# HuttleyLab/DiverseSeq

Measured on AMD Instinct MI355X. Metric: sequences scored/sec (delta-JSD, k=6), higher is better.
Workload: dtype f64 (results and every set update in f64; reject/accept decisions tiered: f32 and f32-log scores decide rows farther from the threshold than their proven error bands, f64 the rest)

## Files before the change

### diverseseq_amd/_lib.py

```python

from __future__ import annotations

import ctypes as C
import os
import pathlib
import threading

import numpy as np

_HERE = pathlib.Path(__file__).resolve().parent
LIB_PATH = pathlib.Path(os.environ["DVS_HIP_LIB"]).resolve() if os.environ.get("DVS_HIP_LIB") else _HERE / "libdvs_hip.so"

OK, ERR_VALUE, ERR_RUNTIME, ERR_NOMEM, ERR_UNSUPPORTED, ERR_ZERODIV = range(6)
CUT_HEIGHT, CUT_NCLUSTERS = 0, 1
MODE_NMOST, MODE_MAX, MODE_SET = 0, 1, 2
STAT_STDEV, STAT_COV = 0, 1
SELECT_NO_ARBITER = 1
SELECT_STEPWISE = 2
ROW_REMOTE = 0xFFFFFFFF

EXPORTS = (
    "dvs_abi_version", "dvs_ctx_create", "dvs_ctx_destroy", "dvs_last_error", "dvs_ctx_sync",
    "dvs_ctx_trim", "dvs_ctx_device_info", "dvs_ctx_set_timing", "dvs_ctx_refresh_knobs", "dvs_matrix_build", "dvs_matrix_from_freqs", "dvs_matrix_from_device_freqs", "dvs_matrix_get_source_rows", "dvs_matrix_count_bytes",
    "dvs_matrix_destroy", "dvs_matrix_nrows", "dvs_matrix_nbins", "dvs_matrix_dev_counts",
    "dvs_matrix_dev_totals", "dvs_matrix_dev_entropy", "dvs_matrix_get_counts",
    "dvs_matrix_get_totals", "dvs_matrix_get_entropy", "dvs_kmer_counts", "dvs_select_run",
    "dvs_select_destroy", "dvs_select_get_summary", "dvs_select_get_members",
    "dvs_select_gather_members",
    "dvs_select_delta_jsd", "dvs_select_step_pack",
    "dvs_select_step_apply", "dvs_select_step_poll", "dvs_select_step_peek", "dvs_select_bench_scan", "dvs_selftest_fast_log2", "dvs_selftest_log2_acc", "dvs_selftest_log2_f32", "dvs_selftest_exact_div", "dvs_selftest_handover", "dvs_mash_sketch", "dvs_mash_distances", "dvs_sketches_build", "dvs_sketches_destroy", "dvs_sketches_get", "dvs_sketches_dev", "dvs_sketches_dev_lens", "dvs_sketches_distances",
    "dvs_sketches_from_device", "dvs_sketches_copy_to_device", "dvs_sketches_distances_device",
    "dvs_default_alphabet_lut", "dvs_seqbatch_from_fasta", "dvs_seqbatch_destroy", "dvs_seqbatch_info",
    "dvs_seqbatch_offsets", "dvs_seqbatch_header_positions", "dvs_seqbatch_dev_codes", "dvs_seqbatch_get_codes",
    "dvs_matrix_build_from_seqbatch",
    "dvs_pack_sequences", "dvs_packed_destroy", "dvs_packed_info", "dvs_packed_dev_codes", "dvs_packed_dev_mask",
    "dvs_packed_get", "dvs_matrix_build_packed", "dvs_sketches_build_packed", "dvs_seqbatch_pack",
    "dvs_seqbatch_packed", "dvs_sketches_build_from_seqbatch",
    "dvs_canonical_bins", "dvs_matrix_fold_canonical", "dvs_matrix_is_canonical",
    "dvs_linkage_cut", "dvs_linkage_cophenet", "dvs_nj_patristic", "dvs_pairs_destroy", "dvs_pairs_info", "dvs_pairs_get",
    "dvs_distances", "dvs_linkage", "dvs_nj", "dvs_maxmin", "dvs_cross_distances", "dvs_nearest", "dvs_within",
    "dvs_cluster_scores", "dvs_cophenet", "dvs_threshold_clusters",
)
WITHIN_SKIP_SELF = 1
SRC_MASH, SRC_EUCLIDEAN, SRC_JSD, SRC_GIVEN = range(4)


class Source(C.Structure):
    _fields_ = [("kind", C.c_uint32), ("handle", C.c_void_p), ("rows", C.POINTER(C.c_uint32)), ("n", C.c_uint32),
                ("k", C.c_uint32), ("sketch_size", C.c_uint32), ("on_device", C.c_int)]


class SelectParams(C.Structure):
    _fields_ = [("mode", C.c_uint32), ("n_seed", C.c_uint32), ("max_size", C.c_uint32),
                ("stat", C.c_uint32), ("window", C.c_uint32), ("flags", C.c_uint32)]


class SelectSummary(C.Structure):
    _fields_ = [("size", C.c_uint32), ("lowest_index", C.c_uint32),
                ("total_jsd", C.c_double), ("mean_delta_jsd", C.c_double),
                ("std_delta_jsd", C.c_double), ("cov_delta_jsd", C.c_double),
                ("summed_entropies", C.c_double),
                ("rows_scored", C.c_uint64), ("rows_rechecked", C.c_uint64),
                ("n_windows", C.c_uint32), ("n_events", C.c_uint32),
                ("n_accepts", C.c_uint32), ("n_arbitrated", C.c_uint32),
                ("scan_ms", C.c_double), ("scan_launches", C.c_uint64),
                ("engine", C.c_uint32), ("rows_coarse_passed", C.c_uint32),
                ("scan_ms_last", C.c_double), ("rows_scored_last", C.c_uint64), ("arbiter_ms", C.c_double)]


class DvsLibraryMissing(RuntimeError):
    pass


_lib = None
_lock = threading.Lock()


def _preload_torch_hip_runtime() -> None:
    import importlib.util
    import sys

    if "torch" in sys.modules:
        return
    try:
        spec = importlib.util.find_spec("torch")
    except (ImportError, ValueError):
        spec = None
    if spec is None or not spec.submodule_search_locations:
        return
    libdir = pathlib.Path(list(spec.submodule_search_locations)[0]) / "lib"
    for name in ("libhsa-runtime64.so", "libamd_comgr.so", "libamdhip64.so"):
        p = libdir / name
        if p.exists():
            try:
                C.CDLL(str(p), mode=C.RTLD_GLOBAL)
            except OSError:
                return


def load() -> C.CDLL:
    global _lib
    with _lock:
        if _lib is not None:
            return _lib
        if not LIB_PATH.exists():
            raise DvsLibraryMissing(
                f"{LIB_PATH} not found: build it with `python -c 'import __graft_entry__ as g; "
                "g.build()'` (hipcc --offload-arch=gfx950). There is no CPU fallback.")
        _preload_torch_hip_runtime()
        L = C.CDLL(str(LIB_PATH))
        vp, u8p, u32p, u64p, f64p = (C.c_void_p, C.POINTER(C.c_uint8), C.POINTER(C.c_uint32),
                                     C.POINTER(C.c_uint64), C.POINTER(C.c_double))
        L.dvs_abi_version.restype = C.c_int
        L.dvs_ctx_create.argtypes = [C.c_int, vp, C.POINTER(vp)]
        L.dvs_ctx_destroy.argtypes = [vp]
        L.dvs_ctx_destroy.restype = None
        L.dvs_last_error.argtypes = [vp]
        L.dvs_last_error.restype = C.c_char_p
        L.dvs_ctx_sync.argtypes = [vp]
        L.dvs_ctx_trim.argtypes = [vp]
        L.dvs_ctx_set_timing.argtypes = [vp, C.c_int]
        L.dvs_ctx_refresh_knobs.argtypes = [vp]
        L.dvs_ctx_device_info.argtypes = [vp, C.c_char_p, C.c_size_t, C.POINTER(C.c_int), u64p]
        L.dvs_matrix_build.argtypes = [vp, vp, C.c_int, u64p, C.c_uint32, C.c_uint32, C.c_uint32,
                                       C.POINTER(vp)]
        L.dvs_matrix_from_freqs.argtypes = [vp, f64p, C.c_uint32, C.c_uint64, C.POINTER(vp)]
        L.dvs_matrix_from_device_freqs.argtypes = [vp, vp, vp, C.c_uint32, C.c_uint64, C.POINTER(vp)]
        L.dvs_select_gather_members.argtypes = [vp, vp, vp, vp, C.c_uint32]
        L.dvs_matrix_destroy.argtypes = [vp]
        L.dvs_matrix_destroy.restype = None
        L.dvs_matrix_nrows.argtypes = [vp]
        L.dvs_matrix_nrows.restype = C.c_uint32
        L.dvs_matrix_nbins.argtypes = [vp]
        L.dvs_matrix_nbins.restype = C.c_uint64
        for n in ("dvs_matrix_dev_counts", "dvs_matrix_dev_totals", "dvs_matrix_dev_entropy"):
            getattr(L, n).argtypes = [vp]
            getattr(L, n).restype = vp
        L.dvs_matrix_get_counts.argtypes = [vp, vp, C.c_uint32, C.c_uint32, u32p]
        L.dvs_matrix_get_totals.argtypes = [vp, vp, u32p]
        L.dvs_matrix_get_entropy.argtypes = [vp, vp, f64p]
        L.dvs_matrix_get_source_rows.argtypes = [vp, vp, u32p]
        L.dvs_matrix_count_bytes.argtypes = [vp]
        L.dvs_matrix_count_bytes.restype = C.c_uint32
        L.dvs_kmer_counts.argtypes = [vp, u8p, u64p, C.c_uint32, C.c_uint32, C.c_uint32, u32p, u32p,
                                      f64p]
        L.dvs_select_run.argtypes = [vp, vp, u32p, u32p, C.c_uint64, C.POINTER(SelectParams),
                                     C.POINTER(vp)]
        L.dvs_select_destroy.argtypes = [vp]
        L.dvs_select_destroy.restype = None
        L.dvs_select_get_summary.argtypes = [vp, vp, C.POINTER(SelectSummary)]
        L.dvs_select_get_members.argtypes = [vp, vp, u64p, u32p, f64p, f64p, f64p]
        L.dvs_select_delta_jsd.argtypes = [vp, vp, vp, u32p, f64p]
        L.dvs_select_step_pack.argtypes = [vp, vp, vp]
        L.dvs_select_step_apply.argtypes = [vp, vp, vp, C.c_uint32]
        L.dvs_select_step_poll.argtypes = [vp, vp, u32p, u64p]
        L.dvs_select_step_peek.argtypes = [vp, vp, C.c_uint32, u32p, C.POINTER(C.c_int)]
        L.dvs_select_bench_scan.argtypes = [vp, vp, C.c_int, f64p, u64p]
        L.dvs_selftest_fast_log2.argtypes = [vp, f64p]
        L.dvs_selftest_log2_acc.argtypes = [vp, f64p]
        L.dvs_selftest_log2_f32.argtypes = [vp, f64p]
        L.dvs_selftest_exact_div.argtypes = [vp, C.POINTER(C.c_uint64)]
        L.dvs_selftest_handover.argtypes = [vp, C.c_uint32, C.POINTER(C.c_uint64)]
        L.dvs_mash_sketch.argtypes = [vp, vp, C.c_int, u64p, C.c_uint32, C.c_uint32, C.c_uint32,
                                      C.c_uint32, C.c_int, u32p, u32p]
        L.dvs_mash_distances.argtypes = [vp, u32p, C.c_uint32, u32p, C.c_uint32, C.c_uint32,
                                         C.c_uint32, C.c_uint32, C.c_uint32, C.c_int, f64p]
        L.dvs_sketches_build.argtypes = [vp, vp, C.c_int, u64p, C.c_uint32, C.c_uint32, C.c_uint32, C.c_uint32,
                                         C.c_int, C.POINTER(vp)]
        L.dvs_sketches_destroy.argtypes = [vp]
        L.dvs_sketches_destroy.restype = None
        L.dvs_sketches_get.argtypes = [vp, vp, u32p, u32p]
        for n in ("dvs_sketches_dev", "dvs_sketches_dev_lens"):
            getattr(L, n).argtypes = [vp]
            getattr(L, n).restype = vp
        L.dvs_sketches_distances.argtypes = [vp, vp, C.c_uint32, C.c_uint32, C.c_uint32, C.c_uint32, C.c_int, f64p]
        L.dvs_sketches_from_device.argtypes = [vp, vp, vp, C.c_uint32, C.c_uint32, C.POINTER(vp)]
        L.dvs_sketches_copy_to_device.argtypes = [vp, vp, vp, C.c_uint32, vp]
        L.dvs_sketches_distances_device.argtypes = [vp, vp, C.c_uint32, C.c_uint32, C.c_uint32, C.c_uint32, C.c_int, vp, vp]
        L.dvs_default_alphabet_lut.argtypes = [C.c_int, u8p]
        L.dvs_default_alphabet_lut.restype = None
        L.dvs_seqbatch_from_fasta.argtypes = [vp, vp, C.c_int, C.c_uint64, u8p, C.c_int, C.POINTER(vp)]
        L.dvs_seqbatch_destroy.argtypes = [vp]
        L.dvs_seqbatch_destroy.restype = None
        L.dvs_seqbatch_info.argtypes = [vp, u32p, u64p, u32p]
        L.dvs_seqbatch_offsets.argtypes = [vp, u64p]
        L.dvs_seqbatch_header_positions.argtypes = [vp, u64p]
        L.dvs_seqbatch_dev_codes.argtypes = [vp]
        L.dvs_seqbatch_dev_codes.restype = vp
        L.dvs_seqbatch_get_codes.argtypes = [vp, vp, u8p]
        L.dvs_matrix_build_from_seqbatch.argtypes = [vp, vp, C.c_uint32, C.c_uint32, C.POINTER(vp)]
        L.dvs_pack_sequences.argtypes = [vp, vp, C.c_int, C.c_uint64, C.POINTER(vp)]
        L.dvs_packed_destroy.argtypes = [vp]
        L.dvs_packed_destroy.restype = None
        L.dvs_packed_info.argtypes = [vp, u64p, u64p]
        for n in ("dvs_packed_dev_codes", "dvs_packed_dev_mask", "dvs_seqbatch_packed"):
            getattr(L, n).argtypes = [vp]
            getattr(L, n).restype = vp
        L.dvs_packed_get.argtypes = [vp, vp, u32p, C.POINTER(C.c_uint16)]
        L.dvs_matrix_build_packed.argtypes = [vp, vp, u64p, C.c_uint32, C.c_uint32, C.POINTER(vp)]
        L.dvs_sketches_build_packed.argtypes = [vp, vp, u64p, C.c_uint32, C.c_uint32, C.c_uint32, C.c_int,
                                                C.POINTER(vp)]
        L.dvs_seqbatch_pack.argtypes = [vp, vp]
        L.dvs_sketches_build_from_seqbatch.argtypes = [vp, vp, C.c_uint32, C.c_uint32, C.c_uint32, C.c_int,
                                                       C.POINTER(vp)]
        u32, srcp = C.c_uint32, C.POINTER(Source)
        L.dvs_linkage_cut.argtypes = [vp, u32, u32p, f64p, C.c_int, C.c_double, u32p, u32p]
        L.dvs_linkage_cophenet.argtypes = [vp, u32, u32p, f64p, f64p]
        L.dvs_nj_patristic.argtypes = [vp, u32, u32p, f64p, f64p]
        L.dvs_canonical_bins.argtypes = [u32, u32p, u64p]
        L.dvs_matrix_fold_canonical.argtypes = [vp, vp, C.POINTER(vp)]
        L.dvs_matrix_is_canonical.argtypes = [vp]
        L.dvs_matrix_is_canonical.restype = C.c_uint32
        L.dvs_pairs_destroy.argtypes = [vp]
        L.dvs_pairs_destroy.restype = None
        L.dvs_pairs_info.argtypes = [vp, u32p, u64p]
        L.dvs_pairs_get.argtypes = [vp, u64p, u32p, f64p]
        L.dvs_distances.argtypes = [vp, srcp, f64p]
        L.dvs_linkage.argtypes = [vp, srcp, C.c_int, u32p, f64p, u32p]
        L.dvs_nj.argtypes = [vp, srcp, u32p, f64p]
        L.dvs_maxmin.argtypes = [vp, srcp, u32p, u32, u32, C.c_int, C.c_double, u32p, f64p, u32p, u32p, f64p, f64p]
        L.dvs_cross_distances.argtypes = [vp, srcp, srcp, f64p]
# ... 29 lines not shown
```

### diverseseq_amd/csrc/api.cpp

```cpp
#include "dvs_internal.h"

#include <algorithm>
#include <cmath>
#include <cstring>
#include <mutex>

uint64_t dvs_pow_u64(uint32_t base, uint32_t exp, bool *overflow);
void dvs_matrix_free_fields(dvs_matrix *m);
int dvs_matrix_fill_counts(dvs_ctx *ctx, dvs_matrix *m, const dvs_seq_view &sv, const uint64_t *offsets, bool no_wait);
int dvs_matrix_fill_freq_entropy(dvs_ctx *ctx, dvs_matrix *m);
int dvs_hist_prepare(dvs_ctx *ctx, const uint64_t *offsets, uint32_t nseq, uint32_t k, uint64_t nbins, uint64_t nbytes, size_t *n_long_out);
bool dvs_hist_rows_fit_u16(const dvs_ctx *ctx, uint64_t B, size_t n_long);
int dvs_matrix_fill_freq_totals(dvs_ctx *ctx, dvs_matrix *m, const double *d_meta);
int dvs_matrix_fill_compacted(dvs_ctx *ctx, dvs_matrix *m, const double *d_in, const double *d_meta);

static std::string g_create_err;

int dvs_set_error(dvs_ctx *ctx, int code, const char *fmt, ...) {
    char buf[512];
    va_list ap;
    va_start(ap, fmt);
    vsnprintf(buf, sizeof buf, fmt, ap);
    va_end(ap);
    if (ctx) ctx->err = buf;
// ... 19 lines not shown
    if (it != ctx->pool.end()) {
        *ptr = it->second;
        ctx->pool.erase(it);
        ctx->pool_bytes -= sz;
        ctx->live[*ptr] = sz;
        if (__builtin_expect(ctx->knobs.test_poison_blocks, 0)) return dev_poison(ctx, *ptr, sz, what);
        return DVS_OK;
    }
    hipError_t e = hipMalloc(ptr, sz);
    if (e != hipSuccess && !ctx->pool.empty()) {
        (void)hipGetLastError();
        dvs_dev_trim(ctx);
        e = hipMalloc(ptr, sz);
    }
    if (e != hipSuccess) {
        *ptr = nullptr;
        return dvs_hip_fail(ctx, e, what);
    }
    ctx->live[*ptr] = sz;
    if (__builtin_expect(ctx->knobs.test_poison_blocks, 0)) return dev_poison(ctx, *ptr, sz, what);
    return DVS_OK;
}

void dvs_dev_free(dvs_ctx *ctx, void *ptr) {
    if (!ptr) return;
    auto it = ctx ? ctx->live.find(ptr) : std::map<void *, size_t>::iterator();
    if (!ctx || it == ctx->live.end()) {
        (void)hipFree(ptr);
        return;
    }
    ctx->pool.emplace(it->second, ptr);
    ctx->pool_bytes += it->second;
    ctx->live.erase(it);
}

int dvs_pinned_get(dvs_ctx *ctx, void **ptr) {
    if (!ctx->pinned_pool.empty()) {
        *ptr = ctx->pinned_pool.back();
        ctx->pinned_pool.pop_back();
        if (__builtin_expect(ctx->knobs.test_poison_blocks, 0)) memset(*ptr, 0xFF, 4096);
        return DVS_OK;
    }
    hipError_t e = hipHostMalloc(ptr, 4096, hipHostMallocDefault);
    if (e != hipSuccess) return dvs_hip_fail(ctx, e, "hipHostMalloc");
    if (__builtin_expect(ctx->knobs.test_poison_blocks, 0)) memset(*ptr, 0xFF, 4096);
    return DVS_OK;
}
void dvs_pinned_put(dvs_ctx *ctx, void *ptr) {
    if (!ptr) return;
    if (ctx) ctx->pinned_pool.push_back(ptr);
    else (void)hipHostFree(ptr);
}
hipEvent_t dvs_event_get(dvs_ctx *ctx) {
    if (!ctx->event_pool.empty()) {
        hipEvent_t e = ctx->event_pool.back();
        ctx->event_pool.pop_back();
        return e;
    }
    hipEvent_t e = nullptr;
    (void)hipEventCreate(&e);
    return e;
}
void dvs_event_put(dvs_ctx *ctx, hipEvent_t e) {
    if (!e) return;
    if (ctx) ctx->event_pool.push_back(e);
    else (void)hipEventDestroy(e);
}

void dvs_dev_trim(dvs_ctx *ctx) {
    (void)hipStreamSynchronize(ctx->stream);
    for (auto &kv : ctx->pool) (void)hipFree(kv.second);
    ctx->pool.clear();
    ctx->pool_bytes = 0;
}

void dvs_knobs_from_env(dvs_knobs *k) {
    auto on = [](const char *name) { return getenv(name) != nullptr; };
    *k = dvs_knobs();
    k->no_uniform_offsets = on("DVS_NO_UNIFORM_OFFSETS");
    k->no_offsets_cache = on("DVS_NO_OFFSETS_CACHE");
    k->counts_u32 = on("DVS_COUNTS_U32");
    k->build_wait = on("DVS_BUILD_WAIT");
    k->no_packed_upload = on("DVS_NO_PACKED_UPLOAD");
    k->cu_mask_set = on("HSA_CU_MASK") || on("ROC_GLOBAL_CU_MASK");
    k->no_persist = on("DVS_NO_PERSIST");
    k->no_fast_step = on("DVS_NO_FAST_STEP");
    k->no_head_phase = on("DVS_NO_HEAD_PHASE");
    k->persist_no_seeded = on("DVS_PERSIST_NO_SEEDED");
    k->persist_no_small = on("DVS_PERSIST_NO_SMALL");
    k->persist_no_coarse = on("DVS_PERSIST_NO_COARSE");
    k->persist_no_events = on("DVS_PERSIST_NO_EVENTS");
    k->persist_debug = on("DVS_PERSIST_DEBUG");
    const char *rounds = getenv("DVS_PERSIST_WG_ROUNDS");
    k->persist_wg_rounds = rounds ? atoi(rounds) : -1;
    k->ingest_no_stream = on("DVS_INGEST_NO_STREAM");
    if (const char *sr = getenv("DVS_CROSS_STRIP_ROWS")) k->cross_strip_rows = uint32_t(strtoul(sr, nullptr, 10));
    if (const char *mb = getenv("DVS_MAXMIN_BATCH")) k->maxmin_batch = uint32_t(strtoul(mb, nullptr, 10));
    k->maxmin_jsd_cross = on("DVS_MAXMIN_JSD_CROSS");
    const char *tk = getenv("DVS_TEST_KNOBS");
    k->test_persist_fake_error = tk && strstr(tk, "fake_persist_error") != nullptr;
    if (const char *lt = tk ? strstr(tk, "long_tile_") : nullptr) k->test_long_tile = uint32_t(strtoul(lt + 10, nullptr, 10));
    k->test_rowlog_ring = 0;
    if (const char *rr = tk ? strstr(tk, "rowlog_ring_") : nullptr) k->test_rowlog_ring = uint32_t(strtoul(rr + 12, nullptr, 10));
    k->test_poison_blocks = tk && strstr(tk, "poison_blocks") != nullptr;
    if (const char *ic = tk ? strstr(tk, "ingest_chunk_") : nullptr)
        k->test_ingest_chunk = uint32_t(std::min<unsigned long>(std::max<unsigned long>(strtoul(ic + 13, nullptr, 10), 1ul), 256ul));
    if (const char *rc = tk ? strstr(tk, "ingest_reccap_") : nullptr)
        k->test_ingest_reccap = std::max<uint64_t>(strtoull(rc + 14, nullptr, 10), 1ull);
}

extern "C" {

int dvs_abi_version(void) { return DVS_ABI_VERSION; }

int dvs_ctx_refresh_knobs(dvs_ctx *ctx) {
    if (!ctx) return dvs_set_error(ctx, DVS_ERR_VALUE, "null argument");
    dvs_knobs_from_env(&ctx->knobs);
    ctx->off_cache.n_off = 0;
    return DVS_OK;
}

int dvs_ctx_create(int device, void *stream, dvs_ctx **out) {
    if (!out) return dvs_set_error(nullptr, DVS_ERR_VALUE, "null argument");
    *out = nullptr;
    int ndev = 0;
    hipError_t e = hipGetDeviceCount(&ndev);
    if (e != hipSuccess || ndev == 0)
        return dvs_set_error(nullptr, DVS_ERR_RUNTIME,
                             "no HIP device available (%s): libdvs_hip has no CPU fallback",
                             e != hipSuccess ? hipGetErrorString(e) : "device count 0");
    if (device < 0) {
        e = hipGetDevice(&device);
        if (e != hipSuccess) return dvs_hip_fail(nullptr, e, "hipGetDevice");
    }
    if (device >= ndev)
        return dvs_set_error(nullptr, DVS_ERR_VALUE, "device %d out of range (%d devices)", device, ndev);
    e = hipSetDevice(device);
    if (e != hipSuccess) return dvs_hip_fail(nullptr, e, "hipSetDevice");
    hipDeviceProp_t prop;
    e = hipGetDeviceProperties(&prop, device);
    if (e != hipSuccess) return dvs_hip_fail(nullptr, e, "hipGetDeviceProperties");
    dvs_ctx *ctx = new dvs_ctx();
    dvs_knobs_from_env(&ctx->knobs);
    ctx->device = device;
    ctx->n_cu = prop.multiProcessorCount;
    ctx->lds_per_block = prop.sharedMemPerBlockOptin ? prop.sharedMemPerBlockOptin
                                                     : prop.sharedMemPerBlock;
    if (ctx->lds_per_block < prop.sharedMemPerBlock) ctx->lds_per_block = prop.sharedMemPerBlock;
    if (stream) {
        ctx->stream = static_cast<hipStream_t>(stream);
    } else {
        e = hipStreamCreateWithFlags(&ctx->stream, hipStreamNonBlocking);
        if (e != hipSuccess) {
            delete ctx;
            return dvs_hip_fail(nullptr, e, "hipStreamCreate");
        }
        ctx->own_stream = true;
    }
    *out = ctx;
    return DVS_OK;
}

void dvs_ctx_destroy(dvs_ctx *ctx) {
    if (!ctx || ctx->owner_gone) return;
    ctx->owner_gone = true;
    dvs_ctx_release(ctx);
// ... 76 lines not shown
    dvs_dev_trim(ctx);
    return DVS_OK;
}

int dvs_ctx_sync(dvs_ctx *ctx) {
    if (!ctx) return DVS_ERR_VALUE;
    DVS_HIP(ctx, hipStreamSynchronize(ctx->stream));
    return DVS_OK;
}

int dvs_ctx_set_timing(dvs_ctx *ctx, int on) {
    if (!ctx) return DVS_ERR_VALUE;
    ctx->timing = on != 0;
    return DVS_OK;
}

int dvs_ctx_device_info(dvs_ctx *ctx, char *name, size_t name_len, int *n_cu, uint64_t *hbm_bytes) {
    if (!ctx) return DVS_ERR_VALUE;
    hipDeviceProp_t prop;
    DVS_HIP(ctx, hipGetDeviceProperties(&prop, ctx->device));
    if (name && name_len) {
        snprintf(name, name_len, "%s (%s)", prop.name, prop.gcnArchName);
    }
    if (n_cu) *n_cu = prop.multiProcessorCount;
    if (hbm_bytes) *hbm_bytes = prop.totalGlobalMem;
    return DVS_OK;
}

static int matrix_alloc(dvs_ctx *ctx, dvs_matrix *m) {
    const size_t cells = size_t(m->nrows) * m->nbins;
    const size_t bytes = cells * (m->kind == 0 ? 4 : m->kind == 2 ? 2 : 8);
    size_t free_b = 0, total_b = 0;
    const bool cached = ctx->pool.count(((bytes ? bytes : 4) + 4095) & ~size_t(4095)) > 0;
    if (!cached) DVS_HIP(ctx, hipMemGetInfo(&free_b, &total_b));
    if (!cached && bytes + size_t(m->nrows) * 12 + (64u << 20) > free_b + ctx->pool_bytes)
        return dvs_set_error(ctx, DVS_ERR_NOMEM,
                             "%u x %llu matrix needs %zu bytes of HBM, %zu free", m->nrows,
                             (unsigned long long)m->nbins, bytes, free_b);
    const size_t nr = m->nrows ? m->nrows : 1;
    m->ctx = ctx;
    dvs_ctx_retain(ctx);
    int rc;
    if (m->kind == 0) rc = dvs_dev_alloc(ctx, (void **)&m->d_counts, bytes ? bytes : 4, "matrix counts");
    else if (m->kind == 2) rc = dvs_dev_alloc(ctx, (void **)&m->d_counts16, bytes ? bytes : 4, "matrix counts (16-bit)");
    else rc = dvs_dev_alloc(ctx, (void **)&m->d_freqs, bytes ? bytes : 8, "matrix freqs");
    if (!rc) rc = dvs_dev_alloc(ctx, (void **)&m->d_totals, nr * 4, "matrix totals");
    if (!rc) rc = dvs_dev_alloc(ctx, (void **)&m->d_entropy, nr * 8, "matrix entropy");
    return rc;
}

static int build_shape(dvs_ctx *ctx, uint32_t k, uint32_t num_states, uint64_t *B_out) {
    if (k == 0) return dvs_set_error(ctx, DVS_ERR_VALUE, "k cannot be 0");
    if (num_states < 1 || num_states > 255)
        return dvs_set_error(ctx, DVS_ERR_VALUE, "num_states %u outside 1..255", num_states);
    if (k > 17) return dvs_set_error(ctx, DVS_ERR_UNSUPPORTED, "k = %u > 17 is not supported", k);
    bool ovf = false;
    const uint64_t B = dvs_pow_u64(num_states, k, &ovf);
    if (ovf || B > (1ull << 32))
        return dvs_set_error(ctx, DVS_ERR_UNSUPPORTED, "%u^%u bins do not fit a dense count row",
                             num_states, k);
    *B_out = B;
    return DVS_OK;
}

static int matrix_build_view(dvs_ctx *ctx, const dvs_seq_view &sv, const uint64_t *offsets, uint32_t nseq, uint32_t k,
                             uint32_t num_states, bool no_wait, dvs_matrix **out) {
    *out = nullptr;
    uint64_t B = 0;
    const int arc = build_shape(ctx, k, num_states, &B);
    if (arc) return arc;
    size_t n_long = 0;
    if (nseq) {
        const int prc = dvs_hist_prepare(ctx, offsets, nseq, k, B, sv.nbytes, &n_long);
        if (prc) return prc;
    }
    dvs_matrix *m = new dvs_matrix();
    m->kind = (nseq && dvs_hist_rows_fit_u16(ctx, B, n_long)) ? 2 : 0;
    m->nrows = nseq;
    m->nbins = B;
    m->k = k;
    m->num_states = num_states;
    m->device = ctx->device;
    int rc = matrix_alloc(ctx, m);
    if (!rc && nseq) rc = dvs_matrix_fill_counts(ctx, m, sv, offsets, no_wait);
    if (rc) {
        dvs_matrix_free_fields(m);
        delete m;
        return rc;
    }
    *out = m;
    return DVS_OK;
}

int dvs_matrix_build(dvs_ctx *ctx, const uint8_t *seqs, int seqs_on_device, const uint64_t *offsets,
                     uint32_t nseq, uint32_t k, uint32_t num_states, dvs_matrix **out) {
    if (!ctx || !offsets || !out || (!seqs && nseq && offsets[nseq] > 0))
        return dvs_set_error(ctx, DVS_ERR_VALUE, "null argument");
    *out = nullptr;
    {
        uint64_t B_ = 0;
        const int arc = build_shape(ctx, k, num_states, &B_);
        if (arc) return arc;
    }
    DVS_HIP(ctx, hipSetDevice(ctx->device));
    const uint64_t nbytes = nseq ? offsets[nseq] : 0;
    dvs_seq_view sv;
    if (seqs_on_device) {
        if (reinterpret_cast<uintptr_t>(seqs) & 15)
            return dvs_set_error(ctx, DVS_ERR_VALUE, "device sequence buffer must be 16-byte aligned");
        sv.seqs = seqs;
        sv.nbytes = nbytes;
        return matrix_build_view(ctx, sv, offsets, nseq, k, num_states, !ctx->knobs.build_wait, out);
    }
    if (nbytes && dvs_packed_upload_wanted(ctx, num_states, nbytes)) {
        dvs_packed *p = nullptr;
        int rc = dvs_packed_alloc(ctx, nbytes, &p);
        if (!rc) rc = dvs_packed_fill_from_host(ctx, p, seqs);
        if (!rc) {
            sv.codes = p->d_codes;
            sv.mask = p->d_mask;
            sv.nbytes = nbytes;
            rc = matrix_build_view(ctx, sv, offsets, nseq, k, num_states, false, out);
        }
        if (p) {
            (void)hipStreamSynchronize(ctx->stream);
            dvs_packed_destroy(p);
        }
        return rc;
    }
    const uint64_t padded = ((nbytes + 15) & ~15ull) + 16;
    uint8_t *d_tmp = nullptr;
    int rc = dvs_dev_alloc(ctx, (void **)&d_tmp, padded, "sequence upload buffer");
    if (rc) return rc;
    hipError_t ue = hipMemsetAsync(d_tmp + (nbytes & ~15ull), 0xFF, padded - (nbytes & ~15ull), ctx->stream);
    if (ue == hipSuccess && nbytes) ue = hipMemcpyAsync(d_tmp, seqs, nbytes, hipMemcpyHostToDevice, ctx->stream);
    if (ue != hipSuccess) {
        (void)hipStreamSynchronize(ctx->stream);
        dvs_dev_free(ctx, d_tmp);
        return dvs_hip_fail(ctx, ue, "sequence upload");
    }
    sv.seqs = d_tmp;
    sv.nbytes = padded;
    rc = matrix_build_view(ctx, sv, offsets, nseq, k, num_states, false, out);
    (void)hipStreamSynchronize(ctx->stream);
    dvs_dev_free(ctx, d_tmp);
    return rc;
}

int dvs_matrix_build_packed(dvs_ctx *ctx, const dvs_packed *p, const uint64_t *offsets, uint32_t nseq, uint32_t k,
                            dvs_matrix **out) {
    if (!ctx || !p || !offsets || !out) return dvs_set_error(ctx, DVS_ERR_VALUE, "null argument");
    *out = nullptr;
    DVS_HIP(ctx, hipSetDevice(ctx->device));
    dvs_seq_view sv;
    sv.codes = p->d_codes;
    sv.mask = p->d_mask;
    sv.nbytes = p->nbases;
    p->async_readers = true;
    return matrix_build_view(ctx, sv, offsets, nseq, k, 4, !ctx->knobs.build_wait, out);
}

int dvs_matrix_from_freqs(dvs_ctx *ctx, const double *freqs, uint32_t nrows, uint64_t nbins,
                          dvs_matrix **out) {
    if (!ctx || !out || (!freqs && nrows)) return dvs_set_error(ctx, DVS_ERR_VALUE, "null argument");
    *out = nullptr;
    if (nbins == 0)
// ... 36 lines not shown
    return DVS_OK;
}

int dvs_matrix_from_device_freqs(dvs_ctx *ctx, const double *d_freqs, const double *d_meta, uint32_t nrows,
                                 uint64_t nbins, dvs_matrix **out) {
    if (!ctx || !out || (!d_freqs && nrows)) return dvs_set_error(ctx, DVS_ERR_VALUE, "null argument");
    *out = nullptr;
    if (nbins == 0)
        return dvs_set_error(ctx, DVS_ERR_VALUE, "cannot calculate entropy as frequency vector empty");
    DVS_HIP(ctx, hipSetDevice(ctx->device));
    dvs_matrix *m = new dvs_matrix();
    m->kind = 1;
    m->nrows = nrows;
    m->nbins = nbins;
    m->device = ctx->device;
    int rc = matrix_alloc(ctx, m);
    if (!rc && nrows && d_meta) {
        rc = dvs_dev_alloc(ctx, (void **)&m->d_src_row, size_t(nrows) * 4, "source rows");
        if (!rc) rc = dvs_matrix_fill_compacted(ctx, m, d_freqs, d_meta);
        if (!rc) rc = dvs_matrix_fill_freq_entropy(ctx, m);
    } else if (!rc && nrows) {
        hipError_t e = hipMemcpyAsync(m->d_freqs, d_freqs, size_t(nrows) * nbins * 8, hipMemcpyDeviceToDevice,
                                      ctx->stream);
        if (e != hipSuccess) rc = dvs_hip_fail(ctx, e, "hipMemcpyAsync(freqs)");
        if (!rc) rc = dvs_matrix_fill_freq_totals(ctx, m, nullptr);
        if (!rc) rc = dvs_matrix_fill_freq_entropy(ctx, m);
    }
    if (rc) {
        dvs_matrix_free_fields(m);
        delete m;
        return rc;
    }
    *out = m;
    return DVS_OK;
}

int dvs_matrix_get_source_rows(dvs_ctx *ctx, const dvs_matrix *m, uint32_t *out) {
    if (!ctx || !m || !out) return dvs_set_error(ctx, DVS_ERR_VALUE, "null argument");
    if (!m->d_src_row) {
        for (uint32_t r = 0; r < m->nrows; r++) out[r] = r;
        return DVS_OK;
    }
    DVS_HIP(ctx, hipMemcpyAsync(out, m->d_src_row, size_t(m->nrows) * 4, hipMemcpyDeviceToHost, ctx->stream));
    DVS_HIP(ctx, hipStreamSynchronize(ctx->stream));
    return DVS_OK;
}

void dvs_matrix_destroy(dvs_matrix *m) {
    if (!m) return;
    dvs_matrix_free_fields(m);
    delete m;
}

uint32_t dvs_matrix_nrows(const dvs_matrix *m) { return m ? m->nrows : 0; }
uint64_t dvs_matrix_nbins(const dvs_matrix *m) { return m ? m->nbins : 0; }
const void *dvs_matrix_dev_counts(const dvs_matrix *m) {
    return !m ? nullptr : m->kind == 2 ? static_cast<const void *>(m->d_counts16) : static_cast<const void *>(m->d_counts);
}
uint32_t dvs_matrix_count_bytes(const dvs_matrix *m) { return !m ? 0u : m->kind == 0 ? 4u : m->kind == 2 ? 2u : 0u; }
const void *dvs_matrix_dev_totals(const dvs_matrix *m) { return m ? m->d_totals : nullptr; }
const void *dvs_matrix_dev_entropy(const dvs_matrix *m) { return m ? m->d_entropy : nullptr; }

int dvs_matrix_get_counts(dvs_ctx *ctx, const dvs_matrix *m, uint32_t row0, uint32_t nrows,
                          uint32_t *out) {
    if (!ctx || !m || !out) return dvs_set_error(ctx, DVS_ERR_VALUE, "null argument");
    if (m->kind == 1) return dvs_set_error(ctx, DVS_ERR_VALUE, "not a count matrix");
    if (uint64_t(row0) + nrows > m->nrows) return dvs_set_error(ctx, DVS_ERR_VALUE, "row range out of bounds");
    if (!nrows) return DVS_OK;
    if (m->kind == 2) {
        const size_t cells = size_t(nrows) * m->nbins;
        std::vector<uint16_t> tmp(cells);
        DVS_HIP(ctx, hipMemcpyAsync(tmp.data(), m->d_counts16 + uint64_t(row0) * m->nbins, cells * 2,
                                    hipMemcpyDeviceToHost, ctx->stream));
        DVS_HIP(ctx, hipStreamSynchronize(ctx->stream));
        for (size_t i = 0; i < cells; i++) out[i] = tmp[i];
        return DVS_OK;
    }
    DVS_HIP(ctx, hipMemcpyAsync(out, m->d_counts + uint64_t(row0) * m->nbins,
                                size_t(nrows) * m->nbins * 4, hipMemcpyDeviceToHost, ctx->stream));
    DVS_HIP(ctx, hipStreamSynchronize(ctx->stream));
    return DVS_OK;
}

int dvs_matrix_get_totals(dvs_ctx *ctx, const dvs_matrix *m, uint32_t *out) {
    if (!ctx || !m || !out) return dvs_set_error(ctx, DVS_ERR_VALUE, "null argument");
    if (!m->nrows) return DVS_OK;
    DVS_HIP(ctx, hipMemcpyAsync(out, m->d_totals, size_t(m->nrows) * 4, hipMemcpyDeviceToHost,
                                ctx->stream));
    DVS_HIP(ctx, hipStreamSynchronize(ctx->stream));
    return DVS_OK;
}

int dvs_matrix_get_entropy(dvs_ctx *ctx, const dvs_matrix *m, double *out) {
    if (!ctx || !m || !out) return dvs_set_error(ctx, DVS_ERR_VALUE, "null argument");
    if (!m->nrows) return DVS_OK;
    DVS_HIP(ctx, hipMemcpyAsync(out, m->d_entropy, size_t(m->nrows) * 8, hipMemcpyDeviceToHost,
                                ctx->stream));
    DVS_HIP(ctx, hipStreamSynchronize(ctx->stream));
    return DVS_OK;
}

int dvs_kmer_counts(dvs_ctx *ctx, const uint8_t *seqs, const uint64_t *offsets, uint32_t nseq,
                    uint32_t k, uint32_t num_states, uint32_t *counts_out, uint32_t *totals_out,
                    double *entropy_out) {
    dvs_matrix *m = nullptr;
    int rc = dvs_matrix_build(ctx, seqs, 0, offsets, nseq, k, num_states, &m);
    if (rc) return rc;
    if (counts_out) rc = dvs_matrix_get_counts(ctx, m, 0, nseq, counts_out);
    if (!rc && totals_out) rc = dvs_matrix_get_totals(ctx, m, totals_out);
    if (!rc && entropy_out) rc = dvs_matrix_get_entropy(ctx, m, entropy_out);
    dvs_matrix_destroy(m);
    return rc;
}

}

int dvs_matrix_alloc_fields(dvs_ctx *ctx, dvs_matrix *m) { return matrix_alloc(ctx, m); }
```

### diverseseq_amd/csrc/dvs_internal.h

```cpp
#pragma once

#include <hip/hip_runtime.h>

#include <cstdarg>
#include <cstdint>
#include <cstdio>
#include <functional>
#include <map>
#include <string>
#include <vector>

#include "../../include/dvs_hip.h"

#define DVS_EPS 2.220446049250313e-16
#define DVS_HEAD_ROWS 1024u

struct dvs_knobs {
    bool no_uniform_offsets = false;
    bool no_offsets_cache = false;
    bool counts_u32 = false;
    bool build_wait = false;
    bool no_packed_upload = false;
    bool cu_mask_set = false;
    bool no_fast_step = false;
    bool no_persist = false;
    bool no_head_phase = false;
    bool persist_no_seeded = false;
    bool persist_no_small = false;
    bool persist_no_coarse = false;
    bool persist_no_events = false;
    bool persist_debug = false;
    int persist_wg_rounds = -1;
    uint32_t cross_strip_rows = 0;
    uint32_t maxmin_batch = 0;
    bool maxmin_jsd_cross = false;
    bool ingest_no_stream = false;
    bool test_persist_fake_error = false;
    uint32_t test_long_tile = 0;
    uint32_t test_rowlog_ring = 0;
    bool test_poison_blocks = false;
    uint32_t test_ingest_chunk = 0;
    uint64_t test_ingest_reccap = 0;
};
void dvs_knobs_from_env(dvs_knobs *k);

struct dvs_ctx {
    dvs_knobs knobs;
    int device = 0;
    hipStream_t stream = nullptr;
    bool own_stream = false;
    hipStream_t stream2 = nullptr;
    hipStream_t stream_head = nullptr, stream_rest = nullptr;
    int head_cus = 0;
    bool cu_split_tried = false;
    int persist_timeouts = 0;
    int n_cu = 0;
    size_t lds_per_block = 0;
    double *d_clog_tbl = nullptr;
    bool timing = false;
    std::string err;
    std::multimap<size_t, void *> pool;
    std::vector<void *> pinned_pool;
    std::vector<hipEvent_t> event_pool;
    std::map<void *, size_t> live;
    size_t pool_bytes = 0;
    int refs = 1;
    bool owner_gone = false;
    std::map<const void *, size_t> lds_raised;
    std::map<std::pair<const void *, size_t>, bool> persist_fits;
    struct OffsetsCache {
        uint64_t *h_off = nullptr;
        size_t h_cap = 0, n_off = 0;
        hipEvent_t ev_up = nullptr;
        std::vector<uint32_t> h_long_rows;
        std::vector<unsigned char> h_tiles;
        uint64_t nbytes = 0;
        uint32_t k = 0;
        void *d_off = nullptr, *d_rows = nullptr, *d_tiles = nullptr;
        size_t d_off_cap = 0;
        size_t n_long = 0, n_tiles = 0;
        bool uniform = false;
        uint64_t uni_base = 0, uni_stride = 0;
        bool lists_in_flight = false;
    } off_cache;
    void *h_pack = nullptr;
    size_t h_pack_cap = 0;
    hipEvent_t pack_ev = nullptr;
    std::map<uint32_t, uint32_t *> canon_reps;
};
int dvs_raise_dyn_lds(dvs_ctx *ctx, const void *fn, size_t bytes);
void dvs_ctx_retain(dvs_ctx *ctx);
hipStream_t dvs_ctx_stream2(dvs_ctx *ctx);
bool dvs_ctx_cu_split(dvs_ctx *ctx);
void dvs_ctx_release(dvs_ctx *ctx);

struct dvs_matrix;
int dvs_matrix_settle(dvs_ctx *ctx, const dvs_matrix *m);
int dvs_dev_alloc(dvs_ctx *ctx, void **ptr, size_t bytes, const char *what);
void dvs_dev_free(dvs_ctx *ctx, void *ptr);
void dvs_dev_trim(dvs_ctx *ctx);
struct PooledBuf {
    dvs_ctx *ctx;
    void *p = nullptr;
    ~PooledBuf() { dvs_dev_free(ctx, p); }
    template <typename T>
    T *as() { return static_cast<T *>(p); }
};
int dvs_pinned_get(dvs_ctx *ctx, void **ptr);
void dvs_pinned_put(dvs_ctx *ctx, void *ptr);
hipEvent_t dvs_event_get(dvs_ctx *ctx);
void dvs_event_put(dvs_ctx *ctx, hipEvent_t e);

int dvs_set_error(dvs_ctx *ctx, int code, const char *fmt, ...);
int dvs_hip_fail(dvs_ctx *ctx, hipError_t e, const char *what);

#define DVS_HIP(ctx, call)                                        \
    do {                                                          \
        hipError_t e__ = (call);                                  \
        if (e__ != hipSuccess) return dvs_hip_fail(ctx, e__, #call); \
    } while (0)

struct dvs_matrix {
    int kind = 0;
    uint16_t *d_counts16 = nullptr;
    uint32_t nrows = 0;
    uint64_t nbins = 0;
    uint32_t k = 0, num_states = 0;
    uint32_t *d_counts = nullptr;
    double *d_freqs = nullptr;
    uint32_t *d_totals = nullptr;
    double *d_entropy = nullptr;
    uint32_t *d_src_row = nullptr;
    std::vector<uint32_t> h_head_totals;
    uint32_t *h_head_pinned = nullptr;
    hipEvent_t ev_built = nullptr;
    hipEvent_t ev_join = nullptr;
    uint32_t head_count = 0;
    uint32_t head_rows_built = 0;
    bool rest_beside_head = false;
    bool in_flight = false;
    bool canonical = false;
    int device = 0;
    dvs_ctx *ctx = nullptr;
};

struct dvs_packed {
    dvs_ctx *ctx = nullptr;
    uint32_t *d_codes = nullptr;
    uint16_t *d_mask = nullptr;
    uint64_t nbases = 0, nwords = 0;
    mutable bool async_readers = false;
};
struct dvs_seq_view {
    const uint8_t *seqs = nullptr;
    const uint32_t *codes = nullptr;
    const uint16_t *mask = nullptr;
    uint64_t nbytes = 0;
};
int dvs_packed_alloc(dvs_ctx *ctx, uint64_t nbases, dvs_packed **out);
int dvs_packed_fill_from_device(dvs_ctx *ctx, dvs_packed *p, const uint8_t *d_seqs);
int dvs_packed_fill_from_host(dvs_ctx *ctx, dvs_packed *p, const uint8_t *seqs);
bool dvs_packed_upload_wanted(const dvs_ctx *ctx, uint32_t num_states, uint64_t nbytes);

int dvs_linkage_check_size(dvs_ctx *ctx, uint32_t n);
int dvs_linkage_check_method(dvs_ctx *ctx, int method);
int dvs_linkage_device(dvs_ctx *ctx, double *d_dist, uint32_t n, const uint32_t *d_zerodiv, int method, uint32_t *pairs,
                       double *heights, uint32_t *sizes);
constexpr uint32_t DVS_LNK_NONFINITE = 1, DVS_LNK_NEGATIVE = 4;
hipError_t dvs_linkage_enqueue_prepare(dvs_ctx *ctx, double *d_dist, uint32_t n, bool sign, uint32_t *d_status);

int dvs_nj_device(dvs_ctx *ctx, double *d_dist, uint32_t n, const uint32_t *d_zerodiv, uint32_t *joins, double *lengths);

int dvs_cophenet_walk(dvs_ctx *ctx, uint32_t n, const uint32_t *pairs, const double *heights, uint32_t *order,
                      uint32_t *pos, uint32_t *gap, double *c_bar);

struct dvs_dist_stage {
    const char *label;
    uint32_t n;
    std::function<int()> check;
    size_t scratch_bytes;
    const char *scratch_what;
    bool scratch_is_zerodiv;
    bool zero_diagonal;
    std::function<hipError_t(double *d_dist, void *d_scratch)> enqueue;
};
dvs_dist_stage dvs_mash_stage(dvs_ctx *ctx, const dvs_sketches *sk, uint32_t k, uint32_t sketch_size);

struct dvs_cross_stage {
    const char *label;
    uint32_t m, n;
    std::function<int()> check;
    size_t scratch_bytes;
    const char *scratch_what;
    bool scratch_is_zerodiv;
    std::function<hipError_t(void *d_scratch)> prepare;
    std::function<hipError_t(uint32_t q0, uint32_t mq, double *d_strip, void *d_scratch)> enqueue;
};
dvs_cross_stage dvs_mash_cross_stage(dvs_ctx *ctx, const dvs_sketches *q, const uint32_t *q_rows, uint32_t nq,
                                     const dvs_sketches *r, const uint32_t *r_rows, uint32_t nr, uint32_t k,
                                     uint32_t sketch_size, const uint32_t *d_q_rows = nullptr);
dvs_cross_stage dvs_euclid_cross_stage(dvs_ctx *ctx, const dvs_matrix *q, const uint32_t *q_rows, uint32_t nq,
                                       const dvs_matrix *r, const uint32_t *r_rows, uint32_t nr,
                                       const uint32_t *d_q_rows = nullptr);
hipError_t dvs_jsd_entropies_enqueue(dvs_ctx *ctx, const dvs_matrix *m, const uint32_t *d_rows, uint32_t count, double *d_h);
hipError_t dvs_jsd_cross_row_enqueue(dvs_ctx *ctx, const dvs_matrix *m, const uint32_t *d_q_rows, uint32_t q0, uint32_t n,
                                     const double *d_hq, const double *d_hr, double *d_row);
int dvs_rows_check(dvs_ctx *ctx, uint32_t n);
// ... 134 lines not shown
```

### diverseseq_amd/csrc/kmer_hist.hip

```cpp
#include "dvs_internal.h"

#include <algorithm>
#include <cstring>
#include <cmath>
#include <cstdlib>

namespace {

constexpr int HIST_THREADS = 256;
constexpr int HIST_MAX_THREADS = 512;
constexpr uint32_t TILE_LEN = 32768;
static_assert(TILE_LEN < 65536, "a whole-sequence tile's counts must fit the packed 16-bit LDS counters");
constexpr int CLOG_TBL = 256;

struct KTile {
    uint64_t begin;
    uint64_t end;
    uint64_t seq_begin;
    uint32_t row;
    uint32_t single;
};

__device__ __forceinline__ uint4 load16(const uint8_t *base, uint64_t off, uint64_t nbytes) {
    if (off + 16 <= nbytes) return *reinterpret_cast<const uint4 *>(base + off);
    uint32_t w[4] = {0xFFFFFFFFu, 0xFFFFFFFFu, 0xFFFFFFFFu, 0xFFFFFFFFu};
    for (int i = 0; i < 16; i++) {
        if (off + i < nbytes) {
            w[i >> 2] &= ~(0xFFu << (8 * (i & 3)));
            w[i >> 2] |= uint32_t(base[off + i]) << (8 * (i & 3));
        }
    }
    return make_uint4(w[0], w[1], w[2], w[3]);
}

template <bool LDS_HIST, bool PK16 = false>
__device__ __forceinline__ void bump(uint32_t *hist, uint32_t idx) {
    if (PK16) atomicAdd(&hist[idx >> 1], (idx & 1u) ? 0x10000u : 1u);
    else atomicAdd(&hist[idx], 1u);
}

__device__ __forceinline__ double clog2c(uint32_t c, const double *tbl) {
    if (c < CLOG_TBL) return tbl[c];
    const double d = double(c);
    return d * log2(d);
}

template <bool NS4, bool LDS_HIST, bool PK16 = false, bool OUT16 = false, bool PACKED = false>
__global__ __launch_bounds__(HIST_MAX_THREADS) void kmer_hist_kernel(
    const uint8_t *__restrict__ seqs, const uint16_t *__restrict__ pmask, uint64_t nbytes,
    const uint64_t *__restrict__ offsets,
    const KTile *__restrict__ tiles, uint32_t *__restrict__ counts, uint32_t *__restrict__ totals,
    double *__restrict__ entropy, const double *__restrict__ clog_tbl, uint32_t k, uint32_t ns,
    uint64_t B, uint32_t hot_rows, uint32_t row0, uint64_t uni_base, uint64_t uni_stride) {
    extern __shared__ __attribute__((aligned(16))) unsigned char smem[];
    KTile t;
    if (tiles) {
        t = tiles[blockIdx.x];
    } else {
        const uint32_t r = row0 + (hot_rows ? gridDim.x - 1 - blockIdx.x : blockIdx.x);
        const uint64_t s0 = offsets ? offsets[r] : uni_base + uint64_t(r) * uni_stride;
        const uint64_t s1 = offsets ? offsets[r + 1] : s0 + uni_stride;
        t.row = r;
        t.single = 1;
        t.seq_begin = s0;
        t.begin = s0 + k - 1;
        t.end = s1;
        if (s1 - s0 >= k && s1 - t.begin > TILE_LEN) return;
        if (s1 - s0 < k) t.begin = t.end = s1;
    }
    static_assert(!OUT16 || PK16, "16-bit rows come from the packed histogram");
    static_assert(!PACKED || NS4, "only four-state sequences have a packed form");
    uint32_t *row = OUT16 ? counts + uint64_t(t.row) * (B / 2) : counts + uint64_t(t.row) * B;
    uint32_t *hist = LDS_HIST ? reinterpret_cast<uint32_t *>(smem) : row;
    double *tbl = reinterpret_cast<double *>(smem + (LDS_HIST ? ((B * (PK16 ? 2 : 4) + 15) & ~15ull) : 0));
    double *scratch = tbl + CLOG_TBL;
    const int tid = threadIdx.x;
    const int nthreads = blockDim.x;

    if (LDS_HIST) {
        if ((B & 3) == 0) {
            uint4 *h4 = reinterpret_cast<uint4 *>(hist);
            for (uint64_t i = tid; i < B / (PK16 ? 8 : 4); i += nthreads) h4[i] = make_uint4(0, 0, 0, 0);
            if (PK16 && (B & 7) && tid == 0) reinterpret_cast<uint2 *>(hist)[B / 4 - 1] = make_uint2(0, 0);
        } else {
            for (uint64_t i = tid; i < B; i += nthreads) hist[i] = 0;
        }
    }
    for (int i = tid; i < CLOG_TBL; i += nthreads) tbl[i] = clog_tbl[i];
    __syncthreads();

    uint32_t nvalid = 0;
    const uint64_t abase = t.begin & ~15ull;
    const uint64_t nchunks = t.end > t.begin ? (t.end - abase + 15) >> 4 : 0;
    const uint32_t bmask = uint32_t(B - 1);

    if (NS4) {
        const uint32_t lane = tid & 63, wave = tid >> 6, nwaves = (nthreads + 63) >> 6;
        const uint64_t per_wave = ((nchunks + nwaves - 1) / nwaves + 63) & ~63ull;
        const uint64_t c_lo = uint64_t(wave) * per_wave;
        const uint64_t c_hi = c_lo + per_wave < nchunks ? c_lo + per_wave : nchunks;
        uint32_t carryP = 0, carryI = 0xFFFFu;
        if (c_lo < c_hi) {
            const uint64_t A0 = abase + (c_lo << 4);
            if (A0 >= 16) {
                if constexpr (PACKED) {
                    carryP = reinterpret_cast<const uint32_t *>(seqs)[(A0 >> 4) - 1];
                    carryI = pmask[(A0 >> 4) - 1];
                } else {
                    const uint4 pv = load16(seqs, A0 - 16, nbytes);
                    carryP = dvs_pack16(pv);
                    carryI = dvs_inv16(pv);
                }
            }
        }
        for (uint64_t c0 = c_lo; c0 < c_hi; c0 += 64) {
            const uint64_t c = c0 + lane;
            const bool live = c < c_hi;
            const uint64_t A = abase + ((live ? c : c_hi - 1) << 4);
            uint32_t Pc, Ic = 0;
            if constexpr (PACKED) {
                Pc = reinterpret_cast<const uint32_t *>(seqs)[A >> 4];
                Ic = pmask[A >> 4];
            } else {
                const uint4 cur = load16(seqs, A, nbytes);
                Pc = dvs_pack16(cur);
                const uint32_t hib = (cur.x | cur.y | cur.z | cur.w) & 0xFCFCFCFCu;
                if (__ballot(hib != 0)) Ic = dvs_inv16(cur);
            }
            const uint32_t Pp = uint32_t(__builtin_amdgcn_update_dpp(int(carryP), int(Pc), 0x138, 0xF, 0xF, false));
            const uint32_t Ip = uint32_t(__builtin_amdgcn_update_dpp(int(carryI), int(Ic), 0x138, 0xF, 0xF, false));
            carryP = uint32_t(__builtin_amdgcn_readlane(int(Pc), 63));
            carryI = uint32_t(__builtin_amdgcn_readlane(int(Ic), 63));
            const uint64_t P = (uint64_t(Pp) << 32) | Pc;
            uint32_t I = (Ip << 16) | Ic;
            const int64_t lead = int64_t(t.seq_begin) - (int64_t(A) - 16);
            if (lead > 0) I |= (lead >= 32) ? 0xFFFFFFFFu : ~(0xFFFFFFFFu >> lead);
// ... 5 lines not shown
                    cover *= 2;
                }
                if (cover < k) W |= W >> (k - cover);
            }
            const uint32_t lo = t.begin > A ? uint32_t(t.begin - A < 16 ? t.begin - A : 16) : 0u;
            const uint32_t hi = t.end > A ? uint32_t(t.end - A < 16 ? t.end - A : 16) : 0u;
            const uint32_t R = (live && hi > lo) ? ((0xFFFFu >> lo) & ~(0xFFFFu >> hi)) : 0u;
            const uint32_t ok = R & ~W & 0xFFFFu;
            nvalid += __popc(ok);
            if (__ballot(ok != 0xFFFFu) == 0) {
                if constexpr (PK16) {
                    const uint64_t P2 = P << 1;
                    const uint32_t p2lo = uint32_t(P2), p2hi = uint32_t(P2 >> 32);
                    const uint32_t amask = (bmask << 1) & ~3u;
                    unsigned char *hb = smem;
#pragma unroll
                    for (int j = 0; j < 16; j++) {
                        const uint32_t tq = __builtin_amdgcn_alignbit(p2hi, p2lo, 2 * (15 - j));
                        uint32_t half = __builtin_amdgcn_ubfe(tq, 1, 1);
                        asm volatile("" : "+v"(half));
                        atomicAdd(reinterpret_cast<uint32_t *>(hb + (tq & amask)), __umul24(half, 0xFFFFu) + 1u);
                    }
                } else {
#pragma unroll
                    for (int j = 0; j < 16; j++) bump<LDS_HIST, PK16>(hist, uint32_t(P >> (2 * (15 - j))) & bmask);
                }
            } else {
#pragma unroll
                for (int j = 0; j < 16; j++) {
                    const uint32_t idx = uint32_t(P >> (2 * (15 - j))) & bmask;
                    if ((ok >> (15 - j)) & 1u) bump<LDS_HIST, PK16>(hist, idx);
                }
            }
        }
    } else {
        for (uint64_t c = tid; c < nchunks; c += nthreads) {
            const uint64_t A = abase + (c << 4);
            const uint4 cur = load16(seqs, A, nbytes);
            const uint4 prev = (A >= 16) ? load16(seqs, A - 16, nbytes)
                                         : make_uint4(0xFFFFFFFFu, 0xFFFFFFFFu, 0xFFFFFFFFu, 0xFFFFFFFFu);
            const int64_t lead = int64_t(t.seq_begin) - (int64_t(A) - 16);
            const uint32_t w[8] = {prev.x, prev.y, prev.z, prev.w, cur.x, cur.y, cur.z, cur.w};
            uint32_t idx = 0, run = 0;
            const uint32_t Bd = uint32_t(B / ns);
#pragma unroll
            for (int q = 0; q < 32; q++) {
                const uint32_t b = (w[q >> 2] >> (8 * (q & 3))) & 0xFFu;
                const bool ok = (b < ns) && (int64_t(q) >= lead);
                idx = ok ? (idx % Bd) * ns + b : 0u;
                run = ok ? run + 1 : 0u;
                if (q >= 16) {
                    const uint64_t p = A + (q - 16);
                    if (p >= t.begin && p < t.end && run >= k) {
                        bump<LDS_HIST, PK16>(hist, idx);
                        nvalid++;
                    }
                }
            }
        }
    }
    if (!LDS_HIST) __threadfence();
    __syncthreads();

    if constexpr (PK16) {
        const uint2 *h2 = reinterpret_cast<const uint2 *>(hist);
        uint4 *r4 = reinterpret_cast<uint4 *>(row);
        typedef uint32_t u32x4 __attribute__((ext_vector_type(4)));
        double sv[2] = {0.0, 0.0}, tv[2] = {0.0, 0.0};
#pragma unroll
        for (int half = 0; half < 2; half++)
            for (uint64_t u = uint64_t(tid) + 128u * half; u < B / 4; u += HIST_THREADS) {
                const uint2 w = h2[u];
                const uint4 v = make_uint4(w.x & 0xFFFFu, w.x >> 16, w.y & 0xFFFFu, w.y >> 16);
                if constexpr (OUT16) {
                    typedef uint32_t u32x2 __attribute__((ext_vector_type(2)));
                    uint2 *r2 = reinterpret_cast<uint2 *>(row);
                    if (t.row < hot_rows) r2[u] = w;
                    else __builtin_nontemporal_store((u32x2){w.x, w.y}, reinterpret_cast<u32x2 *>(r2 + u));
                } else if (t.row < hot_rows) r4[u] = v;
                else __builtin_nontemporal_store((u32x4){v.x, v.y, v.z, v.w}, reinterpret_cast<u32x4 *>(r4 + u));
                if (((w.x | w.y) & 0xFF00FF00u) == 0) sv[half] += ((tbl[v.x] + tbl[v.y]) + tbl[v.z]) + tbl[v.w];
                else sv[half] += clog2c(v.x, tbl) + clog2c(v.y, tbl) + clog2c(v.z, tbl) + clog2c(v.w, tbl);
            }
        tv[0] = double(nvalid);
        const int lane = tid & 63, wave = tid >> 6;
        double sums[2];
#pragma unroll
        for (int q = 0; q < 2; q++) {
            const double a = dvs_wave_sum(q ? tv[0] : sv[0]), b = dvs_wave_sum(q ? tv[1] : sv[1]);
            __syncthreads();
            if (lane == 0) {
                scratch[wave] = a;
                scratch[wave + 2] = b;
            }
            __syncthreads();
            double acc = 0.0;
            for (int i = 0; i < 4; i++) acc += scratch[i];
            sums[q] = acc;
        }
        if (tid == 0) {
            totals[t.row] = uint32_t(sums[1]);
            entropy[t.row] = sums[1] > 0.0 ? log2(sums[1]) - sums[0] / sums[1] : 0.0;
        }
    } else if (t.single) {
        double s = 0.0, tot = 0.0;
        if (tid >= HIST_THREADS) {
        } else if (LDS_HIST) {
            if ((B & 3) == 0) {
                const uint4 *h4 = reinterpret_cast<const uint4 *>(hist);
                uint4 *r4 = reinterpret_cast<uint4 *>(row);
                for (uint64_t i = tid; i < B / 4; i += HIST_THREADS) {
                    const uint4 v = h4[i];
                    typedef uint32_t u32x4 __attribute__((ext_vector_type(4)));
                    if (t.row < hot_rows) r4[i] = v;
                    else __builtin_nontemporal_store((u32x4){v.x, v.y, v.z, v.w}, reinterpret_cast<u32x4 *>(r4 + i));
                    s += clog2c(v.x, tbl) + clog2c(v.y, tbl) + clog2c(v.z, tbl) + clog2c(v.w, tbl);
                    tot += double(v.x) + double(v.y) + double(v.z) + double(v.w);
                }
            } else {
                for (uint64_t i = tid; i < B; i += HIST_THREADS) {
                    const uint32_t v = hist[i];
                    row[i] = v;
                    s += clog2c(v, tbl);
                    tot += double(v);
                }
            }
        } else {
            for (uint64_t i = tid; i < B; i += HIST_THREADS) {
                const uint32_t v = __hip_atomic_load(&row[i], __ATOMIC_RELAXED, __HIP_MEMORY_SCOPE_AGENT);
                s += clog2c(v, tbl);
                tot += double(v);
            }
        }
        s = dvs_block_sum(s, scratch);
        tot = dvs_block_sum(tot, scratch);
        if (tid == 0) {
            totals[t.row] = uint32_t(tot);
            entropy[t.row] = tot > 0.0 ? log2(tot) - s / tot : 0.0;
        }
    } else if (LDS_HIST) {
        for (uint64_t i = tid; i < B; i += nthreads) {
            const uint32_t v = hist[i];
            if (v) atomicAdd(&row[i], v);
        }
    }
}

__global__ void clog_tbl_kernel(double *tbl) {
    const int c = threadIdx.x;
    tbl[c] = c ? double(c) * log2(double(c)) : 0.0;
}

__global__ __launch_bounds__(HIST_THREADS) void row_stats_kernel(
    const uint32_t *__restrict__ counts, const uint32_t *__restrict__ rows,
    uint32_t *__restrict__ totals, double *__restrict__ entropy, uint64_t B) {
    __shared__ double tbl[CLOG_TBL];
    __shared__ double scratch[32];
    const int tid = threadIdx.x;
    if (tid < CLOG_TBL) tbl[tid] = tid ? double(tid) * log2(double(tid)) : 0.0;
    __syncthreads();
    const uint32_t r = rows[blockIdx.x];
    const uint32_t *row = counts + uint64_t(r) * B;
    double s = 0.0, tot = 0.0;
    for (uint64_t i = tid; i < B; i += HIST_THREADS) {
        const uint32_t v = row[i];
        s += clog2c(v, tbl);
        tot += double(v);
    }
    s = dvs_block_sum(s, scratch);
    tot = dvs_block_sum(tot, scratch);
    if (tid == 0) {
        totals[r] = uint32_t(tot);
        entropy[r] = tot > 0.0 ? log2(tot) - s / tot : 0.0;
    }
}

__global__ __launch_bounds__(HIST_THREADS) void zero_rows_kernel(uint32_t *__restrict__ counts,
                                                                const uint32_t *__restrict__ rows,
                                                                uint64_t B) {
    uint32_t *row = counts + uint64_t(rows[blockIdx.x]) * B;
    for (uint64_t i = threadIdx.x; i < B; i += HIST_THREADS) row[i] = 0;
}

__global__ __launch_bounds__(HIST_THREADS) void freq_entropy_kernel(
    const double *__restrict__ freqs, double *__restrict__ entropy, uint64_t B) {
// ... 2 lines not shown
    double h = 0.0;
    for (uint64_t i = threadIdx.x; i < B; i += HIST_THREADS) {
        const double f = row[i];
        if (f != 0.0) h += -f * log2(f);
    }
    h = dvs_block_sum(h, scratch);
    if (threadIdx.x == 0) entropy[blockIdx.x] = h;
}

__global__ __launch_bounds__(HIST_THREADS) void compact_freq_rows_kernel(
    const double *__restrict__ in, const double *__restrict__ meta, double *__restrict__ out,
    uint32_t *__restrict__ totals, uint32_t *__restrict__ src, uint32_t nrows, uint64_t B) {
    __shared__ uint32_t s_cnt[2];
    const uint32_t r = blockIdx.x;
    if (threadIdx.x < 2) s_cnt[threadIdx.x] = 0;
    __syncthreads();
    uint32_t before = 0, all = 0;
    for (uint32_t q = threadIdx.x; q < nrows; q += HIST_THREADS) {
        const uint32_t v = meta[2 * q + 1] != 0.0 ? 1u : 0u;
        all += v;
        if (q < r) before += v;
    }
    atomicAdd(&s_cnt[0], before);
    atomicAdd(&s_cnt[1], all);
    __syncthreads();
    const bool real = meta[2 * r + 1] != 0.0;
    const uint32_t dest = real ? s_cnt[0] : s_cnt[1] + (r - s_cnt[0]);
    const double *a = in + uint64_t(r) * B;
    double *o = out + uint64_t(dest) * B;
    for (uint64_t i = threadIdx.x; i < B; i += HIST_THREADS) o[i] = a[i];
    if (threadIdx.x == 0) {
        totals[dest] = real ? 1u : 0u;
        src[dest] = r;
    }
}

__global__ void freq_totals_kernel(uint32_t *__restrict__ totals, const double *__restrict__ meta,
                                   uint32_t nrows) {
    const uint32_t r = blockIdx.x * blockDim.x + threadIdx.x;
    if (r < nrows) totals[r] = (!meta || meta[2 * r + 1] != 0.0) ? 1u : 0u;
}

template <typename K>
int set_dyn_lds(dvs_ctx *ctx, K kernel, size_t bytes) {
    return dvs_raise_dyn_lds(ctx, reinterpret_cast<const void *>(kernel), bytes);
}

}

uint64_t dvs_pow_u64(uint32_t base, uint32_t exp, bool *overflow) {
    uint64_t r = 1;
    *overflow = false;
    for (uint32_t i = 0; i < exp; i++) {
        if (r > UINT64_MAX / (base ? base : 1)) *overflow = true;
        r *= base;
    }
    return r;
}

int dvs_matrix_settle(dvs_ctx *ctx, const dvs_matrix *cm) {
    dvs_matrix *m = const_cast<dvs_matrix *>(cm);
    if (!m || !m->ev_built) return DVS_OK;
    const hipError_t e = hipEventSynchronize(m->ev_built);
    if (e == hipSuccess) m->h_head_totals.assign(m->h_head_pinned, m->h_head_pinned + m->head_count);
    else m->h_head_totals.clear();
    dvs_event_put(m->ctx, m->ev_built);
    dvs_pinned_put(m->ctx, m->h_head_pinned);
    m->ev_built = nullptr;
    m->h_head_pinned = nullptr;
    if (e != hipSuccess) return dvs_hip_fail(ctx ? ctx : m->ctx, e, "histogram kernels");
    return DVS_OK;
}

void dvs_matrix_free_fields(dvs_matrix *m) {
    if (!m) return;
    (void)dvs_matrix_settle(m->ctx, m);
    if (m->in_flight && m->ctx) (void)hipStreamSynchronize(m->ctx->stream);
    m->in_flight = false;
    if (m->ev_join) dvs_event_put(m->ctx, m->ev_join);
    m->ev_join = nullptr;
    dvs_dev_free(m->ctx, m->d_counts);
    dvs_dev_free(m->ctx, m->d_counts16);
    m->d_counts16 = nullptr;
    dvs_dev_free(m->ctx, m->d_freqs);
    dvs_dev_free(m->ctx, m->d_totals);
    dvs_dev_free(m->ctx, m->d_entropy);
    dvs_dev_free(m->ctx, m->d_src_row);
    m->d_src_row = nullptr;
    m->d_counts = nullptr;
    m->d_freqs = nullptr;
    m->d_totals = nullptr;
    m->d_entropy = nullptr;
    dvs_ctx_release(m->ctx);
    m->ctx = nullptr;
}

int dvs_hist_prepare(dvs_ctx *ctx, const uint64_t *offsets, uint32_t nseq, uint32_t k, uint64_t nbins, uint64_t nbytes,
                     size_t *n_long_out) {
    dvs_ctx::OffsetsCache &oc = ctx->off_cache;
    const size_t n_off = size_t(nseq) + 1;
    oc.uniform = false;
    if (nseq >= 1 && !ctx->knobs.no_uniform_offsets) {
        const uint64_t base = offsets[0], stride = offsets[1] - offsets[0];
        bool uni = offsets[1] >= offsets[0] && stride < uint64_t(TILE_LEN) + k;
        uint64_t diff = 0;
        for (uint32_t r = 0; r < nseq && uni; r += 4096) {
            const uint32_t e = std::min<uint32_t>(nseq, r + 4096);
            for (uint32_t q = r; q < e; q++) diff |= (offsets[q + 1] - offsets[q]) ^ stride;
            uni = diff == 0;
        }
        if (uni && base + uint64_t(nseq) * stride <= nbytes) {
            if (oc.lists_in_flight && (oc.d_rows || oc.d_tiles)) {
                (void)hipStreamSynchronize(ctx->stream);
                oc.lists_in_flight = false;
            }
            dvs_dev_free(ctx, oc.d_rows);
            dvs_dev_free(ctx, oc.d_tiles);
            oc.d_rows = oc.d_tiles = nullptr;
            oc.n_long = oc.n_tiles = 0;
            oc.n_off = 0;
            oc.uniform = true;
            oc.uni_base = base;
            oc.uni_stride = stride;
            *n_long_out = 0;
            return DVS_OK;
        }
    }
    const bool hit = oc.d_off && oc.h_off && oc.k == k && oc.nbytes == nbytes && oc.n_off == n_off &&
                     !ctx->knobs.no_offsets_cache && std::memcmp(oc.h_off, offsets, n_off * 8) == 0;
    if (!hit) {
        if (oc.ev_up) (void)hipEventSynchronize(oc.ev_up);
        if (oc.h_cap < n_off) {
            if (oc.h_off) (void)hipHostFree(oc.h_off);
            oc.h_off = nullptr;
            oc.h_cap = 0;
            const size_t cap = std::max<size_t>(n_off + n_off / 4, 1024);
            const hipError_t he = hipHostMalloc((void **)&oc.h_off, cap * 8, hipHostMallocDefault);
            if (he != hipSuccess) {
                oc.h_off = nullptr;
                return dvs_hip_fail(ctx, he, "pinned offsets block");
            }
            oc.h_cap = cap;
        }
        oc.n_off = 0;
        std::vector<KTile> tiles;
        std::vector<uint32_t> long_rows;
        uint64_t *dst = oc.h_off;
        uint64_t bad = 0, longest = 0;
        dst[0] = offsets[0];
        for (uint32_t r = 0; r < nseq; r++) {
            const uint64_t s0 = offsets[r], s1 = offsets[r + 1];
            dst[r + 1] = s1;
            bad |= uint64_t(s1 < s0) | uint64_t(s1 > nbytes);
            const uint64_t len = s1 - s0;
            longest = len > longest ? len : longest;
        }
        if (bad || longest >= uint64_t(TILE_LEN) + k) {
            uint64_t long_windows = 0;
            for (uint32_t r = 0; r < nseq; r++) {
                const uint64_t s0 = offsets[r], s1 = offsets[r + 1];
                if (s1 < s0 || s1 > nbytes)
                    return dvs_set_error(ctx, DVS_ERR_VALUE, "offsets[%u..%u] = %llu..%llu out of range", r,
                                         r + 1, (unsigned long long)s0, (unsigned long long)s1);
                if (s1 - s0 >= k && s1 - (s0 + k - 1) > TILE_LEN) long_windows += s1 - (s0 + k - 1);
            }
            uint64_t tile_long = TILE_LEN;
// ... 10 lines not shown
                long_rows.push_back(r);
                for (uint64_t b = first; b < s1; b += tile_long) {
                    KTile t;
                    t.begin = b;
                    t.end = std::min<uint64_t>(b + tile_long, s1);
                    t.seq_begin = s0;
                    t.row = r;
                    t.single = 0;
                    tiles.push_back(t);
                }
            }
        }
        if (oc.lists_in_flight && (oc.d_rows || oc.d_tiles || oc.d_off_cap < n_off)) {
            (void)hipStreamSynchronize(ctx->stream);
            oc.lists_in_flight = false;
        }
        dvs_dev_free(ctx, oc.d_rows);
        dvs_dev_free(ctx, oc.d_tiles);
        oc.d_rows = oc.d_tiles = nullptr;
        oc.n_long = oc.n_tiles = 0;
        int arc = DVS_OK;
        if (oc.d_off_cap < n_off) {
            dvs_dev_free(ctx, oc.d_off);
            oc.d_off = nullptr;
            oc.d_off_cap = 0;
            arc = dvs_dev_alloc(ctx, &oc.d_off, (n_off + n_off / 4) * 8, "offsets");
            if (!arc) oc.d_off_cap = n_off + n_off / 4;
        }
        if (!arc && !long_rows.empty()) arc = dvs_dev_alloc(ctx, &oc.d_rows, long_rows.size() * 4, "row list");
        if (!arc && !tiles.empty()) arc = dvs_dev_alloc(ctx, &oc.d_tiles, tiles.size() * sizeof(KTile), "tile list");
        hipError_t ue = hipSuccess;
        oc.h_tiles.assign(reinterpret_cast<const unsigned char *>(tiles.data()),
                          reinterpret_cast<const unsigned char *>(tiles.data()) + tiles.size() * sizeof(KTile));
        oc.h_long_rows = long_rows;
        if (!arc) ue = hipMemcpyAsync(oc.d_off, oc.h_off, n_off * 8, hipMemcpyHostToDevice, ctx->stream);
        if (!arc && ue == hipSuccess) {
            if (!oc.ev_up) oc.ev_up = dvs_event_get(ctx);
            if (oc.ev_up) ue = hipEventRecord(oc.ev_up, ctx->stream);
        }
        if (!arc && ue == hipSuccess && !long_rows.empty()) {
            ue = hipMemcpyAsync(oc.d_rows, oc.h_long_rows.data(), long_rows.size() * 4, hipMemcpyHostToDevice, ctx->stream);
            if (ue == hipSuccess)
                ue = hipMemcpyAsync(oc.d_tiles, oc.h_tiles.data(), oc.h_tiles.size(), hipMemcpyHostToDevice,
                                    ctx->stream);
        }
        if (arc || ue != hipSuccess) {
            dvs_dev_free(ctx, oc.d_rows);
            dvs_dev_free(ctx, oc.d_tiles);
            oc.d_rows = oc.d_tiles = nullptr;
            return arc ? arc : dvs_hip_fail(ctx, ue, "histogram setup");
        }
        oc.n_off = n_off;
        oc.nbytes = nbytes;
        oc.k = k;
        oc.n_long = long_rows.size();
        oc.n_tiles = tiles.size();
    }
    *n_long_out = oc.n_long;
    return DVS_OK;
}

bool dvs_hist_rows_fit_u16(const dvs_ctx *ctx, uint64_t B, size_t n_long) {
    return n_long == 0 && B <= 4096 && (B & 3) == 0 && !ctx->knobs.counts_u32;
}

int dvs_matrix_fill_counts(dvs_ctx *ctx, dvs_matrix *m, const dvs_seq_view &sv, const uint64_t *offsets,
                           bool no_wait) {
    const bool packed = sv.codes != nullptr;
    const uint8_t *d_seqs = packed ? reinterpret_cast<const uint8_t *>(sv.codes) : sv.seqs;
    const uint16_t *d_pmask = sv.mask;
    const uint64_t nbytes = sv.nbytes;
    const uint32_t nseq = m->nrows, k = m->k, ns = m->num_states;
    if (packed && ns != 4) return dvs_set_error(ctx, DVS_ERR_VALUE, "packed sequences have four states, not %u", ns);
    const uint64_t B = m->nbins;
    const bool lds_hist = B * 4 <= 64 * 1024;
    const bool ns4 = ns == 4;
    (void)offsets;
    dvs_ctx::OffsetsCache &oc = ctx->off_cache;
    uint64_t *d_off = oc.uniform ? nullptr : static_cast<uint64_t *>(oc.d_off);
    const uint64_t uni_base = oc.uni_base, uni_stride = oc.uni_stride;
    uint32_t *d_rows = static_cast<uint32_t *>(oc.d_rows);
    KTile *d_tiles = static_cast<KTile *>(oc.d_tiles);
    const size_t n_long = oc.n_long, n_tiles = oc.n_tiles;
    auto cleanup = [&]() {};
    int rc = DVS_OK;
    hipError_t e = hipSuccess;
    if (!lds_hist)
        e = hipMemsetAsync(m->d_counts, 0, size_t(nseq) * B * 4, ctx->stream);
    if (e == hipSuccess && n_long && lds_hist)
        hipLaunchKernelGGL(zero_rows_kernel, dim3(uint32_t(n_long)), dim3(HIST_THREADS), 0, ctx->stream,
                           m->d_counts, d_rows, B);
    if (e != hipSuccess) return dvs_hip_fail(ctx, e, "histogram setup");
    if (!ctx->d_clog_tbl) {
        rc = dvs_dev_alloc(ctx, (void **)&ctx->d_clog_tbl, CLOG_TBL * sizeof(double), "c log2 c table");
        if (rc) {
            cleanup();
            return rc;
        }
        hipLaunchKernelGGL(clog_tbl_kernel, dim3(1), dim3(CLOG_TBL), 0, ctx->stream, ctx->d_clog_tbl);
    }
    int nthreads = HIST_THREADS;
    const int tile_threads = (lds_hist && B * 4 > 32768) ? HIST_MAX_THREADS : HIST_THREADS;
    const size_t lds = (lds_hist ? ((B * 4 + 15) & ~15ull) : 0) + (CLOG_TBL + 32) * sizeof(double);
#define DVS_LAUNCH_HIST(NS4, LH, PKD, GRID, TILES, NTHR, HOT)                                             \
    do {                                                                                         \
        rc = set_dyn_lds(ctx, kmer_hist_kernel<NS4, LH, false, false, PKD>, lds);                \
        if (!rc)                                                                                 \
            hipLaunchKernelGGL((kmer_hist_kernel<NS4, LH, false, false, PKD>), dim3(GRID), dim3(NTHR), lds,  \
                               ctx->stream, d_seqs, d_pmask, nbytes, d_off, TILES, m->d_counts,  \
                               m->d_totals, m->d_entropy, ctx->d_clog_tbl, k, ns, B, HOT, 0u, uni_base, uni_stride);   \
    } while (0)
#define DVS_LAUNCH_HIST_ANY(GRID, TILES, NTHR, HOT)                            \
    do {                                                                  \
        if (packed && lds_hist) DVS_LAUNCH_HIST(true, true, true, GRID, TILES, NTHR, HOT);   \
        else if (packed) DVS_LAUNCH_HIST(true, false, true, GRID, TILES, NTHR, HOT);         \
        else if (ns4 && lds_hist) DVS_LAUNCH_HIST(true, true, false, GRID, TILES, NTHR, HOT);   \
        else if (ns4) DVS_LAUNCH_HIST(true, false, false, GRID, TILES, NTHR, HOT);         \
        else if (lds_hist) DVS_LAUNCH_HIST(false, true, false, GRID, TILES, NTHR, HOT);    \
        else DVS_LAUNCH_HIST(false, false, false, GRID, TILES, NTHR, HOT);                 \
    } while (0)
    uint32_t hot_rows = uint32_t(std::min<uint64_t>(nseq, (192ull << 20) / (B * (m->kind == 2 ? 2 : 4))));
    const bool pk16 = lds_hist && (B & 3) == 0;
    uint32_t head_rows = 0;
    if (m->kind == 2 && no_wait) {
        uint32_t want = DVS_HEAD_ROWS;
        head_rows = std::min<uint32_t>(nseq, want);
    }
    if (head_rows == nseq) head_rows = 0;
    bool head_event_done = false;
    if (m->kind == 2) {
        const size_t lds16 = ((B * 2 + 15) & ~15ull) + (CLOG_TBL + 32) * sizeof(double);
        uint32_t *out16 = reinterpret_cast<uint32_t *>(m->d_counts16);
        auto launch16 = [&](uint32_t row0, uint32_t count, uint32_t hot_end, hipStream_t on) {
            if (packed) {
                rc = set_dyn_lds(ctx, kmer_hist_kernel<true, true, true, true, true>, lds16);
                if (!rc)
                    hipLaunchKernelGGL((kmer_hist_kernel<true, true, true, true, true>), dim3(count), dim3(128), lds16, on,
                                       d_seqs, d_pmask, nbytes, d_off, static_cast<const KTile *>(nullptr), out16,
                                       m->d_totals, m->d_entropy, ctx->d_clog_tbl, k, ns, B, hot_end, row0, uni_base, uni_stride);
            } else if (ns4) {
                rc = set_dyn_lds(ctx, kmer_hist_kernel<true, true, true, true>, lds16);
                if (!rc)
                    hipLaunchKernelGGL((kmer_hist_kernel<true, true, true, true>), dim3(count), dim3(128), lds16, on,
                                       d_seqs, d_pmask, nbytes, d_off, static_cast<const KTile *>(nullptr), out16,
                                       m->d_totals, m->d_entropy, ctx->d_clog_tbl, k, ns, B, hot_end, row0, uni_base, uni_stride);
            } else {
                rc = set_dyn_lds(ctx, kmer_hist_kernel<false, true, true, true>, lds16);
                if (!rc)
                    hipLaunchKernelGGL((kmer_hist_kernel<false, true, true, true>), dim3(count), dim3(128), lds16, on,
                                       d_seqs, d_pmask, nbytes, d_off, static_cast<const KTile *>(nullptr), out16,
                                       m->d_totals, m->d_entropy, ctx->d_clog_tbl, k, ns, B, hot_end, row0, uni_base, uni_stride);
            }
        };
        if (head_rows) {
            const bool split = nseq - head_rows >= 16u * head_rows && dvs_ctx_cu_split(ctx);
            hipEvent_t ev_fork = split ? dvs_event_get(ctx) : nullptr;
            bool forked = ev_fork && hipEventRecord(ev_fork, ctx->stream) == hipSuccess &&
                          hipStreamWaitEvent(ctx->stream_rest, ev_fork, 0) == hipSuccess;
            launch16(0, head_rows, head_rows, ctx->stream);
            void *pin = nullptr;
            if (!rc && dvs_pinned_get(ctx, &pin) == DVS_OK) {
                m->head_count = uint32_t(std::min<size_t>(head_rows, 4096 / sizeof(uint32_t)));
                m->h_head_pinned = static_cast<uint32_t *>(pin);
                m->ev_built = dvs_event_get(ctx);
                if (m->ev_built &&
                    hipMemcpyAsync(m->h_head_pinned, m->d_totals, size_t(m->head_count) * 4, hipMemcpyDeviceToHost,
                                   ctx->stream) == hipSuccess &&
                    hipEventRecord(m->ev_built, ctx->stream) == hipSuccess) {
                    head_event_done = true;
                    m->head_rows_built = head_rows;
                } else {
                    if (m->ev_built) dvs_event_put(ctx, m->ev_built);
                    dvs_pinned_put(ctx, pin);
                    m->ev_built = nullptr;
                    m->h_head_pinned = nullptr;
                }
            }
            if (!rc) {
                const uint32_t hot_end = uint32_t(std::min<uint64_t>(nseq, uint64_t(head_rows) + hot_rows));
                forked = forked && head_event_done;
                launch16(head_rows, nseq - head_rows, hot_end, forked ? ctx->stream_rest : ctx->stream);
                if (forked) {
                    hipEvent_t ev_join = dvs_event_get(ctx);
                    if (!ev_join || hipEventRecord(ev_join, ctx->stream_rest) != hipSuccess ||
                        hipStreamWaitEvent(ctx->stream, ev_join, 0) != hipSuccess) {
                        (void)hipGetLastError();
                        (void)hipStreamSynchronize(ctx->stream_rest);
                    } else {
                        m->rest_beside_head = true;
                    }
                    m->ev_join = ev_join;
                }
            }
            if (ev_fork) dvs_event_put(ctx, ev_fork);
        } else {
            launch16(0, nseq, hot_rows, ctx->stream);
        }
    } else if (pk16) {
        const size_t lds16 = ((B * 2 + 15) & ~15ull) + (CLOG_TBL + 32) * sizeof(double);
        if (packed) {
            rc = set_dyn_lds(ctx, kmer_hist_kernel<true, true, true, false, true>, lds16);
            if (!rc)
                hipLaunchKernelGGL((kmer_hist_kernel<true, true, true, false, true>), dim3(nseq), dim3(128), lds16, ctx->stream,
                                   d_seqs, d_pmask, nbytes, d_off, static_cast<const KTile *>(nullptr), m->d_counts,
                                   m->d_totals, m->d_entropy, ctx->d_clog_tbl, k, ns, B, hot_rows, 0u, uni_base, uni_stride);
        } else if (ns4) {
            rc = set_dyn_lds(ctx, kmer_hist_kernel<true, true, true>, lds16);
            if (!rc)
                hipLaunchKernelGGL((kmer_hist_kernel<true, true, true>), dim3(nseq), dim3(128), lds16, ctx->stream,
                                   d_seqs, d_pmask, nbytes, d_off, static_cast<const KTile *>(nullptr), m->d_counts,
                                   m->d_totals, m->d_entropy, ctx->d_clog_tbl, k, ns, B, hot_rows, 0u, uni_base, uni_stride);
        } else {
            rc = set_dyn_lds(ctx, kmer_hist_kernel<false, true, true>, lds16);
            if (!rc)
                hipLaunchKernelGGL((kmer_hist_kernel<false, true, true>), dim3(nseq), dim3(128), lds16, ctx->stream,
                                   d_seqs, d_pmask, nbytes, d_off, static_cast<const KTile *>(nullptr), m->d_counts,
                                   m->d_totals, m->d_entropy, ctx->d_clog_tbl, k, ns, B, hot_rows, 0u, uni_base, uni_stride);
        }
    } else
        DVS_LAUNCH_HIST_ANY(nseq, static_cast<const KTile *>(nullptr), nthreads, hot_rows);
    if (!rc && n_tiles) {
        DVS_LAUNCH_HIST_ANY(uint32_t(n_tiles), d_tiles, tile_threads, 0u);
        if (!rc)
            hipLaunchKernelGGL(row_stats_kernel, dim3(uint32_t(n_long)), dim3(HIST_THREADS), 0,
                               ctx->stream, m->d_counts, d_rows, m->d_totals, m->d_entropy, B);
    }
#undef DVS_LAUNCH_HIST_ANY
#undef DVS_LAUNCH_HIST
    if (!rc && (e = hipGetLastError()) != hipSuccess) rc = dvs_hip_fail(ctx, e, "histogram launch");
    if (!rc && no_wait && head_event_done) {
        m->in_flight = oc.lists_in_flight = true;
        return DVS_OK;
    }
    if (!rc && no_wait) {
        void *pin = nullptr;
        if (dvs_pinned_get(ctx, &pin) == DVS_OK) {
            m->head_count = uint32_t(std::min<size_t>(nseq, 4096 / sizeof(uint32_t)));
            m->h_head_pinned = static_cast<uint32_t *>(pin);
            m->ev_built = dvs_event_get(ctx);
            if (m->ev_built &&
                hipMemcpyAsync(m->h_head_pinned, m->d_totals, size_t(m->head_count) * 4, hipMemcpyDeviceToHost,
                               ctx->stream) == hipSuccess &&
                hipEventRecord(m->ev_built, ctx->stream) == hipSuccess) {
                m->in_flight = oc.lists_in_flight = true;
                return DVS_OK;
            }
            if (m->ev_built) dvs_event_put(ctx, m->ev_built);
            dvs_pinned_put(ctx, pin);
            m->ev_built = nullptr;
            m->h_head_pinned = nullptr;
        }
    }
    m->h_head_totals.assign(std::min<size_t>(nseq, 4096), 0u);
    if (!rc && !m->h_head_totals.empty() &&
        hipMemcpyAsync(m->h_head_totals.data(), m->d_totals, m->h_head_totals.size() * 4, hipMemcpyDeviceToHost,
                       ctx->stream) != hipSuccess)
        m->h_head_totals.clear();
    if (hipStreamSynchronize(ctx->stream) != hipSuccess && !rc)
        rc = dvs_set_error(ctx, DVS_ERR_RUNTIME, "histogram kernels failed");
    cleanup();
    return rc;
}

int dvs_matrix_fill_freq_entropy(dvs_ctx *ctx, dvs_matrix *m) {
    hipLaunchKernelGGL(freq_entropy_kernel, dim3(m->nrows), dim3(HIST_THREADS), 0, ctx->stream,
                       m->d_freqs, m->d_entropy, m->nbins);
    DVS_HIP(ctx, hipGetLastError());
    return DVS_OK;
}

int dvs_matrix_fill_compacted(dvs_ctx *ctx, dvs_matrix *m, const double *d_in, const double *d_meta) {
    hipLaunchKernelGGL(compact_freq_rows_kernel, dim3(m->nrows), dim3(HIST_THREADS), 0, ctx->stream, d_in, d_meta,
                       m->d_freqs, m->d_totals, m->d_src_row, m->nrows, m->nbins);
    DVS_HIP(ctx, hipGetLastError());
    return DVS_OK;
}

int dvs_matrix_fill_freq_totals(dvs_ctx *ctx, dvs_matrix *m, const double *d_meta) {
    hipLaunchKernelGGL(freq_totals_kernel, dim3((m->nrows + 255) / 256), dim3(256), 0, ctx->stream,
                       m->d_totals, d_meta, m->nrows);
    DVS_HIP(ctx, hipGetLastError());
    return DVS_OK;
}
```

### diverseseq_amd/csrc/persist.hip

```cpp
#include "select_dev.h"

#include <algorithm>
#include <type_traits>
#include <cstddef>
#include <cstdlib>
#include <cstring>

namespace {

constexpr int P_THREADS = 512;
constexpr int P_J = 8;
constexpr int P_CH = 16;
constexpr uint32_t P_MAXN = 512;
constexpr uint32_t P_MAXN_BIG = 256;
constexpr uint32_t P_MAXN_MAX = 896;
constexpr uint32_t p_maxn(bool cached, bool maxm = false) { return cached ? (maxm ? P_MAXN_MAX : P_MAXN) : P_MAXN_BIG; }
constexpr uint32_t P_SMALLN = 16;
constexpr uint32_t P_SMALL_ROWS = 13;
constexpr uint32_t p_maxjobs(bool cached, bool maxm = false) { return p_maxn(cached, maxm) + 1; }
constexpr size_t p_acc_bytes(uint32_t maxn) { return size_t(8) * (maxn + 1) * 2 * sizeof(unsigned long long); }
__device__ __forceinline__ unsigned long long p_acc_word(double v) {
    return ((unsigned long long)__double2ll_rn(v * 0x1p50) << 6) + 1ull;
}
__device__ __forceinline__ double p_acc_value(unsigned long long w) { return double((long long)w >> 6) * 0x1p-50; }
// ... 157 lines not shown
    if (idx < P_LIST) __hip_atomic_store(w.mysoft + idx, p_word(w.epoch, p, false), RLX_AGENT);
    else p_post_event_thread(w, p, false);
}
template <int CTRL>
__device__ __forceinline__ unsigned long long p_dpp_mov_u64(unsigned long long v) {
    int lo = int(uint32_t(v)), hi = int(uint32_t(v >> 32));
    lo = __builtin_amdgcn_update_dpp(0, lo, CTRL, 0xF, 0xF, true);
    hi = __builtin_amdgcn_update_dpp(0, hi, CTRL, 0xF, 0xF, true);
    return ((unsigned long long)uint32_t(hi) << 32) | uint32_t(lo);
}
__device__ __forceinline__ unsigned long long p_wave_min_u64(unsigned long long v) {
    auto mn = [](unsigned long long a, unsigned long long b) { return b < a ? b : a; };
    v = mn(v, p_dpp_mov_u64<0xB1>(v));
    v = mn(v, p_dpp_mov_u64<0x4E>(v));
    v = mn(v, p_dpp_mov_u64<0x141>(v));
    v = mn(v, p_dpp_mov_u64<0x140>(v));
    const int lo = int(uint32_t(v)), hi = int(uint32_t(v >> 32));
    auto row = [&](int l) {
        return ((unsigned long long)uint32_t(__builtin_amdgcn_readlane(hi, l)) << 32) | uint32_t(__builtin_amdgcn_readlane(lo, l));
    };
    return mn(mn(row(0), row(16)), mn(row(32), row(48)));
}

__device__ __forceinline__ unsigned long long p_gather(PSync *sync, uint32_t G, uint32_t epoch, unsigned long long own,
                                                       uint32_t lane, bool &ok, unsigned long long *seen_all = nullptr,
                                                       unsigned long long *stored = nullptr) {
    constexpr uint32_t Q = P_MAXG / 64;
    unsigned long long w[Q];
    bool have[Q];
#pragma unroll
    for (uint32_t q = 0; q < Q; q++) {
        w[q] = ~0ull;
        have[q] = lane + 64 * q >= G - 1;
    }
    uint32_t spins = 0;
    ok = true;
    for (;;) {
        unsigned long long got[Q];
#pragma unroll
        for (uint32_t q = 0; q < Q; q++)
            got[q] = have[q] ? 0ull : __hip_atomic_load(&sync->wrec[epoch & 1u][lane + 64 * q], RLX_AGENT);
        bool all = true;
#pragma unroll
        for (uint32_t q = 0; q < Q; q++) {
            if (!have[q] && p_word_is(got[q], epoch)) {
                w[q] = got[q];
                have[q] = true;
            }
            all = all && have[q];
        }
        if (__ballot(!all) == 0ull) break;
        if ((++spins & 255u) == 0 && (spins > P_SPIN_LIMIT || __hip_atomic_load(&sync->timeout, RLX_AGENT))) {
            ok = false;
            break;
        }
        __builtin_amdgcn_s_sleep(1);
    }
    if (seen_all) *seen_all = __builtin_amdgcn_s_memrealtime();
    unsigned long long m = own & ~6ull, fl = own & 6ull;
#pragma unroll
    for (uint32_t q = 0; q < Q; q++)
        if (lane + 64 * q < G - 1 && have[q]) {
            m = (w[q] & ~6ull) < m ? (w[q] & ~6ull) : m;
            fl |= w[q] & 6ull;
        }
    m = p_wave_min_u64(m);
    const bool anyl = __ballot(fl != 0ull) != 0ull;
    const unsigned long long relw = m | (anyl ? 2ull : 0ull);
    if (ok && lane < 8) __hip_atomic_store(&sync->rel[lane].rel, relw, RLX_AGENT);
    if (!ok && lane == 0) __hip_atomic_store(&sync->timeout, 1u, RLX_AGENT);
    if (stored) *stored = __builtin_amdgcn_s_memrealtime();
    return relw;
}

template <typename T, bool COARSE>
__device__ __forceinline__ void p_scan_rows(const T *__restrict__ mat,
                                            const uint32_t *__restrict__ totals,
                                            const double *__restrict__ rowH, const double *sl,
                                            const float *slf, uint64_t B, const PState &st, double he_base,
                                            const PWin &win,
                                            uint64_t first, uint64_t stride, uint64_t nrows,
                                            uint32_t lane, uint32_t &nread,
                                            uint32_t &nprecise, uint32_t &nmid, bool coarse_on,
                                            bool burst_drop = true) {
    const double dn = double(st.n), rn = 1.0 / dn;
    const double thr_lo = st.thr - st.band;
    const double thr_fast = thr_lo - FAST_BAND, thr_sure = st.thr + st.band + FAST_BAND;
    (void)thr_lo;
    const bool vec = (B & 255) == 0;
    const double cband = coarse_band(B);
    const double thr_c_lo = st.thr - st.band - cband, thr_c_hi = st.thr + st.band + cband;
    for (uint64_t r = first; r < nrows; r += stride) {
        const uint64_t p = st.cursor + r;
        const T *rp = mat + p * B;
        const uint64_t ev = p_hint_pos(win);
        const uint32_t tot = totals[p];
        const double hrow = rowH[p];
        if (ev < p) break;
        if (tot == 0) continue;
        const double rt = 1.0 / double(tot);
        const double mean_entropy = (he_base + hrow) / dn;
        nread++;
        if constexpr (COARSE) {
            if (vec && coarse_on) {
                const float rtn = float(rt * rn);
                const dvs_f2 r2 = {rtn, rtn};
                double c0 = 0.0, c1 = 0.0;
                bool done16 = false;
                if constexpr (sizeof(T) == 2) {
                    if (B == 4096) {
                        uint4 raw8[8];
#pragma unroll
                        for (int j = 0; j < 8; j++) raw8[j] = *reinterpret_cast<const uint4 *>(rp + j * 512 + lane * 8);
                        __builtin_amdgcn_sched_barrier(0);
#pragma unroll
                        for (int j = 0; j < 8; j++) {
                            asm volatile("" : "+v"(raw8[j].x), "+v"(raw8[j].y), "+v"(raw8[j].z), "+v"(raw8[j].w));
                            coarse8(raw8[j], slf + j * 512 + lane * 8, r2, c0, c1);
                        }
                        done16 = true;
                    }
                }
                if (!done16) {
                constexpr int C_CH = sizeof(T) == 2 ? 16 : 8;
                const uint64_t full = B - B % (256 * C_CH);
                uint64_t i0 = 0;
                bool dropped = false;
                for (; i0 < full; i0 += 256 * C_CH) {
                    if (i0 && burst_drop && p_hint_pos(win) < p) {
                        dropped = true;
                        break;
                    }
                    Raw4<T> raw[C_CH];
#pragma unroll
                    for (int j = 0; j < C_CH; j++) raw[j].load(rp + i0 + uint64_t(j) * 256 + lane * 4);
                    __builtin_amdgcn_sched_barrier(0);
#pragma unroll
                    for (int j = 0; j < C_CH; j += 2) {
                        const uint64_t i = i0 + uint64_t(j) * 256 + lane * 4;
                        raw[j].pin();
                        raw[j + 1].pin();
                        c0 += double(coarse4(raw[j].c, *reinterpret_cast<const float4 *>(slf + i), r2));
                        c1 += double(coarse4(raw[j + 1].c, *reinterpret_cast<const float4 *>(slf + i + 256), r2));
                    }
                }
                if (dropped) {
                    nread--;
                    break;
                }
                for (; i0 < B; i0 += 256) {
                    const uint64_t i = i0 + lane * 4;
                    Raw4<T> raw;
                    raw.load(rp + i);
                    c0 += double(coarse4(raw.c, *reinterpret_cast<const float4 *>(slf + i), r2));
                }
                }
                const double jf0 = -dvs_wave_sum_dpp(c0 + c1) - mean_entropy;
                if (!(jf0 > thr_c_lo)) continue;
                if (jf0 > thr_c_hi) {
                    p_post_event_wave(win, p, true, lane);
                    continue;
                }
                nmid++;
            }
        }
        double a0 = 0.0, a1 = 0.0, a2 = 0.0, a3 = 0.0, xmin = 0.0;
        if (vec) {
            constexpr int F_CH = COARSE ? P_CH / 2 : P_CH;
            const uint64_t full = B - B % (256 * F_CH);
            uint64_t i0 = 0;
            for (; i0 < full; i0 += 256 * F_CH) {
                Raw4<T> raw[F_CH];
#pragma unroll
                for (int j = 0; j < F_CH; j++) raw[j].load(rp + i0 + uint64_t(j) * 256 + lane * 4);
#pragma unroll
                for (int j = 0; j < F_CH; j++) {
                    const uint64_t i = i0 + uint64_t(j) * 256 + lane * 4;
                    const double2 b01 = *reinterpret_cast<const double2 *>(sl + i);
                    const double2 b23 = *reinterpret_cast<const double2 *>(sl + i + 2);
                    double v0, v1, v2, v3;
                    raw[j].get(v0, v1, v2, v3);
                    const double x0 = fma(v0, rt, b01.x) * rn, x1 = fma(v1, rt, b01.y) * rn;
                    const double x2 = fma(v2, rt, b23.x) * rn, x3 = fma(v3, rt, b23.y) * rn;
                    a0 += fast_neg_xlog2x(x0);
                    a1 += fast_neg_xlog2x(x1);
                    a2 += fast_neg_xlog2x(x2);
                    a3 += fast_neg_xlog2x(x3);
                    xmin = fmin(fmin(xmin, fmin(x0, x1)), fmin(x2, x3));
                }
            }
            for (; i0 < B; i0 += 256) {
                const uint64_t i = i0 + lane * 4;
                double v0, v1, v2, v3;
// ... 268 lines not shown
            return uint32_t(w);
        }
    }
    wgmode = false;
    return sel_next_window(st.cursor, st.n, st.wmin, st.wmax, st.wscale);
}

template <uint32_t Q>
__device__ __forceinline__ void p_argmin(const double *s_dl, const double *s_ds, uint32_t n, uint64_t B,
                                         uint32_t lane, double *scratch) {
    const double v0 = lane < n ? s_dl[lane] : 1e6;
    auto val = [&](uint32_t q) { return (Q == 1 || q == 0) ? v0 : s_dl[lane + 64 * q]; };
    double best = 1e6, acc = 0.0;
    bool rk = false;
#pragma unroll
    for (uint32_t q = 0; q < Q; q++) {
        const uint32_t r = lane + 64 * q;
        if (r < n) {
            const double v = val(q);
            rk |= sum_risky(s_ds[r], B);
            acc += v;
            if (v < best) best = v;
        }
    }
    const double dn = double(n);
    const double mnv = dvs_wave_min(best);
    double fi = 4294967295.0;
#pragma unroll
    for (uint32_t q = 0; q < Q; q++)
        if (mnv < 1e6 && lane + 64 * q < n && val(q) == mnv) fi = fmin(fi, double(lane + 64 * q));
    const double first = dvs_wave_min(fi);
    const uint32_t lw = (first < 4294967295.0) ? uint32_t(first) : 0u;
    const double mu = dvs_wave_sum(acc) / dn;
    double sec = 1e6, tv = 0.0;
#pragma unroll
    for (uint32_t q = 0; q < Q; q++) {
        const uint32_t r = lane + 64 * q;
        if (r < n) {
            const double v = val(q);
            if (r != lw && v < sec) sec = v;
            const double t = v - mu;
            tv += t * t;
        }
    }
    sec = dvs_wave_min(sec);
    const double var = dvs_wave_sum(tv);
    const unsigned long long anyr = __ballot(rk);
    if (lane == 0) {
        scratch[100] = mnv;
        scratch[101] = double(lw);
        scratch[102] = sec;
        scratch[103] = mu;
        scratch[104] = sqrt(var / (dn - 1.0));
        scratch[105] = anyr ? 1.0 : 0.0;
    }
}

template <typename T, bool CACHED, bool MAXM = false, bool SMALL = false>
__global__ __launch_bounds__(P_THREADS, 2) void persist_nmost_kernel(SelDev d, const T *__restrict__ mat,
                                                                    PSync *sync, unsigned long long *part, uint32_t G) {
    static_assert(!SMALL || (CACHED && !MAXM && sizeof(T) == 2), "SMALL: nmost, 16-bit rows, state in the register cache");
    constexpr uint32_t maxn = SMALL ? P_SMALLN : p_maxn(CACHED, MAXM);
    constexpr bool SPEC = CACHED && !MAXM && sizeof(T) <= 4;
    constexpr bool SPEC_BIG = !CACHED && !MAXM && sizeof(T) <= 4;
    constexpr bool OWN = SPEC && !SMALL;
    extern __shared__ __attribute__((aligned(16))) unsigned char smem[];
    const uint64_t B0 = d.B;
    const uint64_t B = B0;
    double *sl = reinterpret_cast<double *>(smem);
    constexpr bool COARSE = CACHED && sizeof(T) <= 4;
    float *slf = reinterpret_cast<float *>(sl + ((B + 1) & ~1ull));
    static_assert(!MAXM || CACHED, "the growth phase keeps the candidate's frequencies in registers");
    double *Sl = sl + ((B + 1) & ~1ull) + (COARSE ? ((B + 3) & ~3ull) / 2 : 0);
    double *scratch = Sl + (MAXM ? ((B + 1) & ~1ull) : 0);
    double *s_mH = scratch + 128;
    double *s_tot = s_mH + maxn;
    double *s_rt = s_tot + maxn;
    double *s_dl = s_rt + maxn;
    double *s_ds = s_dl + maxn;
    uint64_t *s_pos = reinterpret_cast<uint64_t *>(s_ds + maxn);
    uint32_t *s_slot = reinterpret_cast<uint32_t *>(s_pos + maxn);
    unsigned long long *s_win = reinterpret_cast<unsigned long long *>(s_slot + maxn + (maxn & 1));
    int *s_flag = reinterpret_cast<int *>(s_win + P_WINWORDS);
    static_assert(maxn % 4 == 0 && P_WINWORDS % 2 == 0, "s_ltab below must sit on a 16-byte boundary");
    double2 *s_ltab = reinterpret_cast<double2 *>(s_win + P_WINWORDS + 2);
    unsigned long long *s_prev = reinterpret_cast<unsigned long long *>(s_ltab + 128);
    unsigned char *s_tail = reinterpret_cast<unsigned char *>(s_prev + uint64_t(maxn + 1) * 2);
    [[maybe_unused]] uint16_t *s_rows = reinterpret_cast<uint16_t *>(s_tail);
    [[maybe_unused]] uint32_t *s_inv = reinterpret_cast<uint32_t *>(s_tail);
    [[maybe_unused]] T *s_own = reinterpret_cast<T *>(s_inv + maxn);
    [[maybe_unused]] double *s_bt = reinterpret_cast<double *>(s_tail);
    [[maybe_unused]] double *s_bH = s_bt + P_BATCH;
    [[maybe_unused]] double *s_bev = s_bH + P_BATCH;
    [[maybe_unused]] double *s_bpart = s_bev + 12 * P_BATCH;
    if (threadIdx.x < 128) log2_tab_fill(s_ltab, threadIdx.x);
    for (uint32_t i = threadIdx.x; i < (maxn + 1) * 2; i += P_THREADS) s_prev[i] = 0ull;
    SelCtl *ctl = d.ctl;
    const int tid0 = threadIdx.x;
    const int tid = tid0;
    [[maybe_unused]] const uint32_t lane = tid & 63, wave = tid >> 6;
    const bool two_roles = G >= 3;
    const bool gath = blockIdx.x == G - 1;
    const bool lead = blockIdx.x == (two_roles ? G - 2 : G - 1);
    const uint32_t n_work = G > 1 ? G - (two_roles ? 2u : 1u) : 1u;

    PState st;
    st.cursor = ctl->cursor;
    st.npos = ctl->npos;
    const bool head_phase = sync->stop_at != 0u && uint64_t(sync->stop_at) < st.npos;
    if (head_phase) st.npos = sync->stop_at;
    st.window = ctl->window;
    st.wmin = ctl->window_min;
    st.wmax = sync->wmax > ctl->window_max ? sync->wmax : ctl->window_max;
    st.n = ctl->size;
    st.li = ctl->lowest;
    st.sumH = ctl->sum_entropy;
    st.total_jsd = ctl->total_jsd;
    st.thr = ctl->thr;
    st.band = ctl->band;
    st.wscale = ctl->wscale;
    st.n_windows = st.n_events = st.n_accepts = 0;
    st.max_size = MAXM ? ctl->max_size : st.n;
    st.stat = ctl->stat;
    st.mean_d = ctl->mean_delta;
    st.std_d = ctl->std_delta;
    st.cov_d = ctl->cov_delta;
    if (lead && tid == 0) ctl->rows_before_launch = ctl->rows_scored;
    if (ctl->status != SEL_RUN || ctl->ev_kind != 0 || st.n > maxn || st.n < 2) {
        if (lead && tid == 0 && ctl->status == SEL_RUN) ctl->why[7]++;
        return;
    }
    if (MAXM && st.n < st.max_size && (ctl->s_is_resum == 0 || st.n + 2 > maxn)) {
        if (lead && tid == 0) ctl->why[6]++;
        return;
    }
    const bool seeded = !MAXM && CACHED && sync->seeded != 0u;
    for (uint32_t r = tid; r < st.n; r += P_THREADS) {
        const uint32_t slot = seeded ? r : d.ord[r];
        const uint64_t mp = seeded ? sync->seed_list[r] : d.mPos[slot];
        const double t = double(d.totals[mp]);
        s_slot[r] = slot;
        s_mH[r] = seeded ? d.rowH[mp] : d.mH[slot];
        s_pos[r] = mp;
        s_tot[r] = t;
        s_rt[r] = 1.0 / t;
    }
    __syncthreads();
    if (!seeded) {
        const double *low = d.M + uint64_t(s_slot[st.li]) * B;
        const double rn0 = 1.0 / double(st.n);
        for (uint64_t i = tid; i < B; i += P_THREADS) {
            const double v = d.S[i] - low[i];
            sl[i] = v;
            if (COARSE) slf[i] = coarse_sl(v, rn0);
            if (MAXM) Sl[i] = d.S[i];
        }
    }
    __syncthreads();

    uint32_t gen = 0, epoch = 0;
    uint32_t nread = 0, nprecise = 0, nmid = 0;
    uint32_t exit_status = SEL_RUN;
    uint32_t arb_stage = 0;
    uint64_t arb_pos = 0;
    uint32_t pend_kind = 0;
    bool bail = false;
    [[maybe_unused]] uint32_t mx_batch = 1;
    [[maybe_unused]] uint32_t n_batches = 0;
    uint32_t early_rec = 0xFFFFFFFFu;
    auto announce_early = [&](uint32_t next_epoch) {
        if (lead && two_roles && !MAXM) {
            if (threadIdx.x == 0)
                __hip_atomic_store(&sync->wrec[next_epoch & 1u][blockIdx.x], p_word(next_epoch, SEL_NONE, false), RLX_AGENT);
            early_rec = next_epoch;
        }
    };
    const uint64_t wpb = P_THREADS / 64;
    const uint32_t nwg = n_work;
    const uint64_t nwaves = uint64_t(nwg) * wpb;
// ... 280 lines not shown
            const unsigned long long t_now = __builtin_amdgcn_s_memrealtime(); \
            s_dbg[k] += t_now - t_prev;                                    \
            t_prev = t_now;                                                \
        }                                                                  \
    } while (0)
#define P_TRACE(which)                                                                             \
    do {                                                                                           \
        if (tid == 0 && (epoch == 12 || epoch == 24 || epoch == 36 || epoch == 48))               \
            sync->trace[epoch / 12 - 1][which][blockIdx.x] = __builtin_amdgcn_s_memrealtime();     \
    } while (0)
#define P_TRACE_G(slot)                                                                            \
    do {                                                                                           \
        if (tid == 0 && (epoch == 12 || epoch == 24 || epoch == 36 || epoch == 48))               \
            sync->trace[epoch / 12 - 1][3][slot] = __builtin_amdgcn_s_memrealtime();               \
    } while (0)
#endif
#else
#define P_STAMP(k) do { } while (0)
#define P_STAMP_B0(k) do { } while (0)
#define P_TRACE(which) do { } while (0)
#define P_TRACE_G(slot) do { } while (0)
#define P_PROBE_BEGIN(id) do { } while (0)
#define P_PROBE_END(id) do { } while (0)
#endif
#ifdef DVS_PERSIST_CHAOS
#define P_CHAOS(k)                                                                                         \
    do {                                                                                                   \
        uint32_t h_ = (epoch * 0x9E3779B1u) ^ ((blockIdx.x + 1u) * 0x85EBCA77u) ^ (uint32_t(k) * 0xC2B2AE3Du); \
        h_ ^= h_ >> 15;                                                                                    \
        h_ *= 0x27D4EB2Fu;                                                                                 \
        h_ ^= h_ >> 13;                                                                                    \
        if ((h_ & 15u) == 0u)                                                                              \
            for (uint32_t z_ = (h_ >> 8) & 31u; z_ > 0; z_--) __builtin_amdgcn_s_sleep(12);               \
        if ((h_ & 0xFFF0u) == 0x1230u)       \
            for (uint32_t z_ = 0; z_ < 160; z_++) __builtin_amdgcn_s_sleep(14);                            \
    } while (0)
#else
#define P_CHAOS(k) do { } while (0)
#endif
    for (;;) {
        uint64_t B = B0;
        int tid = tid0;
        asm volatile("" : "+s"(B));
        asm volatile("" : "+v"(tid));
        const uint32_t lane = uint32_t(tid) & 63u, wave = uint32_t(tid) >> 6;
        if (epoch >= P_EPOCH_MAX) {
            bail = true;
            break;
        }
        PRel *myrel = &sync->rel[blockIdx.x & 7u];
        PWin win;
        win.epoch = epoch;
        win.hintp = &myrel->hint;
        win.rel = sync->rel;
        win.wgev = s_win;
        win.nlist = reinterpret_cast<uint32_t *>(s_win + 1);
        win.mysoft = &sync->soft[epoch & 1u][blockIdx.x][0];
        if (tid == 0) {
            s_win[0] = p_word(epoch, SEL_NONE, false);
            *win.nlist = 0u;
        }
        __syncthreads();
        P_PROBE_END(6);
        P_PROBE_BEGIN(1);
        P_CHAOS(1);
        P_STAMP_B0(9);
        P_TRACE(0);
#ifdef DVS_PERSIST_STAMPS
        const unsigned long long t_window = __builtin_amdgcn_s_memrealtime();
#endif
        const uint64_t end = umin64(st.cursor + uint64_t(st.window), st.npos);
        const uint64_t nrows = end - st.cursor;
        if ((!lead && !gath) || G == 1) {
            if (wgmode && COARSE && B == 4096 && coarse_on) {
                if constexpr (COARSE)
                    p_scan_rows_wg_stream<T>(mat, d.totals, d.rowH, sl, slf, st, st.sumH - s_mH[st.li], win,
                                             blockIdx.x, nwg, nrows, scratch + 32, nread, nprecise, nmid);
            } else if (wgmode)
                p_scan_rows_wg<T, COARSE>(mat, d.totals, d.rowH, sl, slf, B, st, st.sumH - s_mH[st.li], win,
                                          blockIdx.x, nwg, nrows, scratch + 32, nread, nprecise, nmid, coarse_on);
            else
                p_scan_rows<T, COARSE>(mat, d.totals, d.rowH, sl, slf, B, st, st.sumH - s_mH[st.li], win,
                                       uint64_t(blockIdx.x) * wpb + wave, nwaves, nrows, lane, nread, nprecise, nmid, coarse_on,
                                       true);
        }
        double fr[P_J];
        [[maybe_unused]] T craw[P_J];
        [[maybe_unused]] uint64_t craw_pos = SEL_NONE;
        [[maybe_unused]] uint32_t craw_tot = 1;
        [[maybe_unused]] double craw_H = 0.0;
        [[maybe_unused]] uint64_t fr_pos = SEL_NONE;
        [[maybe_unused]] uint64_t spec_job_pos = SEL_NONE;
        [[maybe_unused]] double spec_th = 0.0, spec_ts = 0.0;
        [[maybe_unused]] auto fetch_raw = [&](uint64_t q) {
            if (craw_pos != q) {
                const T *gp = mat + q * B;
#pragma unroll
                for (int j = 0; j < P_J; j++) {
                    const uint64_t i = uint64_t(j) * P_THREADS + tid;
                    craw[j] = i < B ? gp[i] : T(0);
                }
                craw_tot = d.totals[q];
                craw_H = d.rowH[q];
                craw_pos = q;
            }
        };
        [[maybe_unused]] auto small_job = [&](uint32_t r, uint32_t part_i, uint32_t at, uint32_t n_, double &th, double &ts) {
            const double dn_ = double(n_), rn_ = 1.0 / dn_, rdiv_ = 1.0 / (dn_ - 1.0);
            const bool is_new = r == n_ - 1;
            uint32_t mcv[P_J];
#pragma unroll
            for (int j = 0; j < P_J; j++) mcv[j] = 0u;
            double mtot = 1.0, mrt = 1.0;
            if (r < n_ && !is_new) {
                if constexpr (SMALL) {
                    const uint4 q = *reinterpret_cast<const uint4 *>(s_rows + uint64_t(s_slot[at]) * 4096 + uint32_t(tid) * 8);
                    const uint32_t qw[4] = {q.x, q.y, q.z, q.w};
#pragma unroll
                    for (int j = 0; j < P_J; j++) mcv[j] = (qw[j >> 1] >> ((j & 1) * 16)) & 0xFFFFu;
                } else if (use_own) {
#pragma unroll
                    for (int j = 0; j < P_J; j++) mcv[j] = uint32_t(s_own[uint32_t(tid) * P_J + j]);
                } else {
                    const T *mrow = mat + s_pos[at] * B;
#pragma unroll
                    for (int j = 0; j < P_J; j++) {
                        const uint64_t i = uint64_t(j) * P_THREADS + tid;
                        if ((uint32_t(j) & (K - 1)) == part_i && i < B) mcv[j] = uint32_t(mrow[i]);
                    }
                }
                mtot = s_tot[at];
                mrt = s_rt[at];
            }
            double h = 0.0, sv = 0.0;
#pragma unroll
            for (int j = 0; j < P_J; j++) {
                if ((uint32_t(j) & (K - 1)) == part_i && uint64_t(j) * P_THREADS + tid < B) {
                    double v = sl[uint64_t(j) * P_THREADS + tid];
                    if (v <= DVS_EPS) v = 0.0;
                    const double sn = v + fr[j];
                    double u;
                    if (r == n_) {
                        u = sn * rn_;
                    } else {
                        u = (sn - (is_new ? fr[j] : exact_div_u32(double(mcv[j]), mtot, mrt))) * rdiv_;
                        if (u <= DVS_EPS) u = 0.0;
                    }
                    if (u > 0.0) h -= u * log2_tab(u, s_ltab);
                    sv += u;
                }
            }
            h = dvs_wave_sum_dpp(h);
            sv = dvs_wave_sum_dpp(sv);
            __syncthreads();
            if (lane == 0) {
                scratch[64 + wave] = h;
                scratch[80 + wave] = sv;
            }
            __syncthreads();
            th = ts = 0.0;
            if (tid < 8) {
                for (uint32_t w = 0; w < P_THREADS / 64; w++) {
                    th += scratch[64 + w];
                    ts += scratch[80 + w];
                }
            }
        };
// ... 1333 lines not shown
        {
            const bool low_is_new = lowest == n - 1;
            const T *lrow = mat + s_pos[lowest] * B;
            const double ltot = s_tot[lowest], lrt = s_rt[lowest];
            constexpr int RB = (!CACHED && sizeof(T) <= 4) ? 2 * P_J : P_J;
            for (uint64_t b0 = 0; b0 < B; b0 += uint64_t(RB) * P_THREADS) {
                T cv[RB], lv[RB];
                if constexpr (SMALL) {
                    const uint4 q = *reinterpret_cast<const uint4 *>(s_rows + uint64_t(s_slot[lowest]) * 4096 + uint32_t(tid) * 8);
                    lv[0] = T(q.x & 0xFFFFu); lv[1] = T(q.x >> 16);
                    lv[2] = T(q.y & 0xFFFFu); lv[3] = T(q.y >> 16);
                    lv[4] = T(q.z & 0xFFFFu); lv[5] = T(q.z >> 16);
                    lv[6] = T(q.w & 0xFFFFu); lv[7] = T(q.w >> 16);
                } else {
#pragma unroll
                for (int j = 0; j < RB; j++) {
                    const uint64_t i = b0 + uint64_t(j) * P_THREADS + tid;
                    if (i < B) {
                        if (!CACHED) cv[j] = rp[i];
                        if (!low_is_new) lv[j] = lrow[i];
                    }
                }
                }
#ifdef DVS_PERSIST_STAMPS
                asm volatile("s_waitcnt vmcnt(0)" ::: "memory");
                P_STAMP(8);
#endif
#pragma unroll
                for (int j = 0; j < RB; j++) {
                    const uint64_t i = b0 + uint64_t(j) * P_THREADS + tid;
                    if (i < B) {
                        double v = sl[i];
                        if (v <= DVS_EPS) v = 0.0;
                        const double f = CACHED ? fr[j % P_J] : count_freq_x(cv[j], tot, rtot);
                        const double sn = v + f;
                        const double nv = sn - (low_is_new ? f : count_freq_x(lv[j], ltot, lrt));
                        sl[i] = nv;
                        if (MAXM) Sl[i] = sn;
                        if (COARSE) slf[i] = coarse_sl(nv, rn);
                        (void)dn;
                    }
                }
            }
        }
        P_PROBE_END(8);
        P_PROBE_BEGIN(9);
        if (lead && tid == 0) {
            ctl->lowest = lowest;
            ctl->band = band;
            ctl->he_base = st.sumH - s_mH[lowest];
            ctl->thr = st.thr;
            ctl->ev_risky = 0;
        }
        __syncthreads();
        P_STAMP(5);
        P_PROBE_END(9);
        P_PROBE_END(5);
        P_PROBE_BEGIN(6);
        P_TRACE(6);
        P_STAMP_B0(12);
        if (st.cursor >= st.npos) { exit_status = SEL_DONE; break; }
        st.window = p_next_window(st, nwg, wg_thresh, wg_scale, wgmode);
        epoch++;
    }

#ifdef DVS_PERSIST_STAMPS
#ifdef DVS_PROBE
    if ((blockIdx.x == n_work - 1 || blockIdx.x == 0) && tid == 0)
        for (int k_ = 0; k_ < 16; k_++) (blockIdx.x == 0 ? sync->dbg2 : sync->dbg)[k_] += s_dbg[k_];
#else
    if ((lead || blockIdx.x == 0) && tid == 0)
        for (int k_ = 0; k_ < 16; k_++) (lead ? sync->dbg : sync->dbg2)[k_] += s_dbg[k_];
#endif
#endif
    if (lead && exit_status != SEL_ERROR && !(exit_status == SEL_ARBITER && arb_stage == ARB_FINALIZE)) {
        const double dn_x = double(st.n);
        for (uint64_t i = tid; i < B; i += P_THREADS) d.base[i] = sl[i] / dn_x;
    }
    if (lane == 0 && nread) {
        atomicAdd(&ctl->rows_scored, (unsigned long long)nread);
        if (nprecise) atomicAdd(&ctl->rows_rechecked, (unsigned long long)nprecise);
        if (nmid) atomicAdd(&ctl->rows_coarse_passed, (unsigned long long)nmid);
    }
    if (lead && tid == 0) {
        ctl->cursor = st.cursor;
        ctl->window = st.window < ctl->window_max ? st.window : ctl->window_max;
        ctl->n_windows += st.n_windows;
        ctl->n_events += st.n_events;
        ctl->n_accepts += st.n_accepts;
        ctl->ev_kind = pend_kind;
        if (exit_status == SEL_ARBITER) {
            ctl->arb_stage = arb_stage;
            ctl->arb_pos = arb_pos;
            if (arb_stage == ARB_RESOLVE) ctl->event_pos = arb_pos;
        }
        ctl->status = (bail || (head_phase && exit_status == SEL_DONE)) ? SEL_RUN
                      : (exit_status == SEL_RUN ? SEL_ERROR : exit_status);
    }
}

__device__ __forceinline__ uint32_t ho_hash(uint32_t round, uint32_t b) {
    uint32_t h = round * 0x9E3779B1u ^ (b + 1u) * 0x85EBCA77u;
    h ^= h >> 15;
    h *= 0xC2B2AE3Du;
    h ^= h >> 13;
    return h;
}
__device__ __forceinline__ uint64_t ho_event(uint32_t round, uint32_t b, bool &sure, bool &lists) {
    const uint32_t h = ho_hash(round, b);
    sure = (h >> 2) & 1u;
    lists = ((h >> 3) & 15u) == 0u;
    return (h & 3u) == 0u ? uint64_t(round) * 4096u + ((h >> 8) % 4000u) : SEL_NONE;
}
constexpr uint32_t HO_MEMBERS = 24, HO_K = 8;

__global__ __launch_bounds__(P_THREADS) void handover_selftest_kernel(PSync *sync, unsigned long long *acc_all, uint32_t G,
                                                                      uint32_t rounds, unsigned long long *bad) {
    __shared__ unsigned long long s_win[8];
    __shared__ unsigned long long s_prev[(HO_MEMBERS + 1) * 2];
    __shared__ int s_flag[2];
    const uint32_t tid = threadIdx.x, lane = tid & 63u, wave = tid >> 6, b = blockIdx.x;
    const bool gath = b == G - 1;
    const bool mirror = b == G - 2;
    const uint32_t n_work = G - 2;
    uint32_t early_rec = 0xFFFFFFFFu;
    for (uint32_t i = tid; i < (HO_MEMBERS + 1) * 2; i += P_THREADS) s_prev[i] = 0ull;
    unsigned long long fails = 0;
    PRel *myrel = &sync->rel[b & 7u];
    const unsigned long long *acc = acc_all + uint64_t(b & 7u) * (HO_MEMBERS + 1) * 2;
    for (uint32_t epoch = 0; epoch < rounds; epoch++) {
        PWin win;
        win.epoch = epoch;
        win.hintp = &myrel->hint;
        win.rel = sync->rel;
        win.wgev = s_win;
        win.nlist = reinterpret_cast<uint32_t *>(s_win + 1);
        win.mysoft = &sync->soft[epoch & 1u][b][0];
        if (tid == 0) {
            s_win[0] = p_word(epoch, SEL_NONE, false);
            *win.nlist = 0u;
        }
        __syncthreads();
        const uint32_t h = ho_hash(epoch, b);
        for (uint32_t z = (h >> 24) & 15u; z > 0; z--) __builtin_amdgcn_s_sleep(3);
        bool sure, lists;
        const uint64_t mine = (gath || mirror) ? SEL_NONE : ho_event(epoch, b, sure, lists);
        if (mirror) lists = false;
        if (!gath && !mirror && tid == 0) {
            if (mine != SEL_NONE) p_post_event_thread(win, mine, sure);
            if (lists) p_list_candidate(win, uint64_t(epoch) * 4096u + 4001u + b);
        }
        __syncthreads();
        const uint32_t nl = *win.nlist;
        const unsigned long long own = s_win[0] | ((unsigned long long)(nl < P_LIST ? nl : P_LIST) << 1);
        if (tid == 0 && early_rec != epoch) __hip_atomic_store(&sync->wrec[epoch & 1u][b], own, RLX_AGENT);
        unsigned long long rel_w = 0ull;
        bool ok = true;
        if (gath) {
            if (wave == 0) {
                const unsigned long long relw = p_gather(sync, G, epoch, own, lane, ok);
                if (lane == 0) {
                    s_win[4] = relw;
                    s_flag[0] = ok ? 1 : 0;
                }
            }
        } else if (tid == 0) {
// ... 379 lines not shown
```

### diverseseq_amd/csrc/select.h

```cpp
#pragma once

#include "dvs_internal.h"

#define SEL_NONE 0xFFFFFFFFFFFFFFFFull
#define SEL_SEEDS_AT 512

enum : uint32_t { SEL_RUN = 0, SEL_DONE = 1, SEL_ARBITER = 2, SEL_ERROR = 3,
                  SEL_NEED_SETUP = 4 };
enum : uint32_t { ARB_RESOLVE = 1, ARB_FINALIZE = 2 };
enum : uint32_t { FORCE_NONE = 0, FORCE_ACCEPT = 1, FORCE_REJECT = 2, FORCE_COMMIT = 3, FORCE_ROLLBACK = 4 };

struct SelCtl {
    unsigned long long cursor;
    unsigned long long npos;
    unsigned long long event_pos;
    unsigned long long arb_pos;
    unsigned long long rows_scored, rows_rechecked;
    unsigned long long rows_coarse_passed;
    unsigned long long rows_before_launch;
    uint32_t window, window_min, window_max;
    uint32_t status, arb_stage, forced, forced_lowest;
    uint32_t size, lowest, mode, max_size, stat;
    uint32_t ev_kind;
    uint32_t ev_n;
    uint32_t ev_risky;
    uint32_t s_is_resum;
    uint32_t mb_rows;
    uint32_t mb_stuck;
    uint32_t n_windows, n_events, n_accepts;
    uint32_t n_logged;
    double total_jsd, sum_entropy;
    double thr, band;
    double he_base;
    double mean_delta, std_delta, cov_delta;
    double t_total_jsd, t_sum_entropy;
    double last_jsd;
    double arb_H;
    double wscale;
    uint32_t why[8];
};

struct SelDev {
    SelCtl *ctl = nullptr;
    uint64_t B = 0;
    uint32_t nlabels = 0;
    const uint32_t *order = nullptr;
    const uint32_t *labels = nullptr;
    const uint32_t *totals = nullptr;
    const double *rowH = nullptr;
    double *S = nullptr;
    double *Stmp = nullptr;
    double *base = nullptr;
    double *cand = nullptr;
    double *M = nullptr;
    double *mH = nullptr;
    double *mDelta = nullptr;
    double *dtmp = nullptr;
    double *dsum = nullptr;
    uint32_t *mLabel = nullptr;
    unsigned long long *mPos = nullptr;
    uint32_t *ord = nullptr;
    uint8_t *inset = nullptr;
    uint32_t *wg_rows = nullptr;
    unsigned long long *evlog_pos = nullptr;
    uint32_t *evlog_kind = nullptr;
    const double *gather_all = nullptr;
    uint32_t gather_world = 0;
    double *rowlog = nullptr;
    uint32_t rowlog_cap = 0;
};

struct dvs_select {
    dvs_ctx *ctx = nullptr;
    dvs_select_params params{};
    const dvs_matrix *mat = nullptr;
    int mat_kind = 0;
    uint64_t npos = 0;
    uint32_t cap = 0;
    SelDev dev;
    SelCtl *h_ctl = nullptr;
    SelCtl ctl0{};
    std::vector<uint32_t> h_order, h_labels;
    std::vector<uint32_t> h_out_labels;
    std::vector<uint64_t> seed_positions;
    uint32_t scan_grid = 0, loo_grid = 0;
    size_t scan_lds = 0;
    bool base_in_lds = true;
    bool scan_hot = false;
    bool persist = false;
    uint32_t persist_grid = 0, persist_maxn = 0, persist_maxjobs = 0;
    bool persist_small = false;
    uint32_t persist_small_rows = 0;
    size_t persist_lds = 0;
    void *psync = nullptr;
    std::vector<unsigned char> h_psync;
    std::vector<unsigned char> h_psync_head;
    void *ppart = nullptr;
    double *d_mbres = nullptr;
    uint32_t mb_jw = 0;
    uint32_t mb_launched = 0;
    void *psync_head = nullptr, *ppart_head = nullptr;
    bool persist_seeded = false;
    bool seeded_start = false;
    bool head_prepared = false;
    bool persist_prepared = false;
    bool used_side_streams = false;
    hipEvent_t ev_side_done = nullptr;
    void *d_seed_list = nullptr;
    bool seed_list_in_ctl = false;
    bool inset_clean = false;
    hipStream_t setup_side = nullptr;
    bool head_phase = false;
    int batch = 16;
    bool time_scan = false;
    std::vector<hipEvent_t> ev_pool;
    size_t ev_used = 0;
    double scan_ms = 0.0;
    double scan_ms_last = 0.0;
    uint64_t scan_launches = 0;
    uint32_t n_arbitrated = 0;
    double arbiter_ms = 0.0;
    bool fast_step = false;
    bool fs_need_scan = false;
    unsigned long long *h_fshist = nullptr;
    unsigned long long fs_launches = 0;
    unsigned long long fs_peek_floor = 0;
    double *fs_slot = nullptr;
    double *fs_packed = nullptr;
    double *d_jobres = nullptr;
    void *d_fsync = nullptr;
    uint32_t fs_K = 1, fs_jobs = 0, fs_grid = 0;
    size_t fs_lds = 0;
    std::vector<double> h_rowlog;
    uint64_t rowlog_have = 0;
    uint32_t steps_since_poll = 0;
    void *arbiter = nullptr;
};

int dvs_select_arbitrate(dvs_ctx *ctx, dvs_select *s);
void dvs_select_arbiter_free(dvs_select *s);

int dvs_persist_setup(dvs_ctx *ctx, dvs_select *s);
int dvs_persist_launch(dvs_ctx *ctx, dvs_select *s);
int dvs_persist_launch_head(dvs_ctx *ctx, dvs_select *s, uint32_t grid, uint32_t stop_at, hipStream_t on);
int dvs_persist_prepare_main(dvs_ctx *ctx, dvs_select *s);
int dvs_persist_prepare_head(dvs_ctx *ctx, dvs_select *s, uint32_t stop_at, hipStream_t on);
// ... 5 lines not shown
```

### diverseseq_amd/csrc/select.hip

```cpp
#include "dvs_internal.h"
#include "select.h"
#include "select_dev.h"

#include <algorithm>
#include <chrono>
#include <type_traits>
#include <cmath>
#include <cstring>
#include <cstdlib>
#include <memory>

namespace {

constexpr int SCAN_THREADS = 512;
constexpr int WIDE_THREADS = 1024;
constexpr int LOO_THREADS = 256;

template <typename T>
__device__ __forceinline__ void scan_rows_hot(SelCtl *ctl, const T *__restrict__ mat,
                                              const uint32_t *__restrict__ totals,
                                              const double *__restrict__ rowH, const double *bvec,
                                              uint64_t B, const ScanState &st, uint64_t first,
                                              uint64_t stride, uint32_t lane, uint32_t &nread,
                                              uint32_t &nprecise) {
// ... 2088 lines not shown
    }
    a.labels = labels;
    if (npos < n_seed)
        return dvs_set_error(ctx, DVS_ERR_VALUE, "The number of sequences %llu is < n %u",
                             (unsigned long long)npos, n_seed);
    if (params->mode == DVS_MODE_MAX && npos <= max_size) max_size = uint32_t(npos);
    if (params->mode != DVS_MODE_MAX) max_size = n_seed;

    uint32_t nlabels = 0;
    if (order || labels) {
        for (uint64_t p = 0; p < npos; p++) {
            const uint32_t row = order ? order[p] : uint32_t(p);
            if (row == DVS_ROW_REMOTE) continue;
            if (row >= m->nrows)
                return dvs_set_error(ctx, DVS_ERR_VALUE, "order[%llu] = %u out of range",
                                     (unsigned long long)p, row);
            const uint32_t lab = labels ? labels[p] : row;
            if (lab != 0xFFFFFFFFu) nlabels = std::max(nlabels, lab + 1);
        }
    } else {
        nlabels = uint32_t(npos);
    }
    if (order)
        for (uint64_t p = 0; p < n_seed; p++)
            if (order[p] == DVS_ROW_REMOTE)
                return dvs_set_error(ctx, DVS_ERR_VALUE,
                                     "seed position %llu is not local: the first n rows must be replicated",
                                     (unsigned long long)p);
    const uint32_t cap = std::max<uint32_t>(std::max<uint32_t>(max_size, n_seed) + 1, 2);
    const size_t need = size_t(cap) * B * 8 + 5 * B * 8 + size_t(npos) * 8 + nlabels + (1 << 20);
    size_t free_b = 0, total_b = 0;
    if (need > (size_t(1) << 30)) DVS_HIP(ctx, hipMemGetInfo(&free_b, &total_b));
    if (need > (size_t(1) << 30) && need > free_b + ctx->pool_bytes)
        return dvs_set_error(ctx, DVS_ERR_NOMEM, "selection state needs %zu bytes, %zu free", need,
                             free_b);
    a.n_seed = n_seed;
    a.max_size = max_size;
    a.nlabels = nlabels;
    a.cap = cap;
    return DVS_OK;
}

static int sel_geometry(dvs_ctx *ctx, dvs_select *s, const uint32_t *order, const uint32_t *labels) {
    const uint64_t B = s->dev.B;
    s->base_in_lds = B * 8 <= 128 * 1024 && B * 8 + 1024 <= ctx->lds_per_block;
    s->scan_lds = 16 + (s->base_in_lds ? B * 8 : 0);
    const uint32_t wg_fit = s->base_in_lds ? std::max<uint32_t>(1, uint32_t((160 * 1024) / (B * 8 + 512))) : 4;
    uint32_t wg_per_cu = std::min<uint32_t>(wg_fit, 2);
    s->scan_grid = std::max<uint32_t>(1, uint32_t(ctx->n_cu) * wg_per_cu);
    s->loo_grid = s->cap;
    s->batch = 16;
    s->time_scan = ctx->timing;
    s->scan_hot = B % (256 * SCAN_CH) == 0 && !order && !labels && s->base_in_lds;
    if (s->scan_lds <= 48 * 1024) return DVS_OK;
    const void *fn = dvs_mat_dispatch(s->mat, [&](auto *mp) -> const void * {
        using T = std::remove_cv_t<std::remove_pointer_t<decltype(mp)>>;
        return s->scan_hot ? reinterpret_cast<const void *>(scan_kernel<T, true>)
                           : reinterpret_cast<const void *>(scan_kernel<T, false>);
    });
    return dvs_raise_dyn_lds(ctx, fn, s->scan_lds);
}

static int sel_alloc(dvs_ctx *ctx, dvs_select *s, const uint32_t *order, const uint32_t *labels) {
    SelDev &d = s->dev;
    const uint64_t B = d.B, npos = s->npos;
    const uint32_t cap = s->cap, nlabels = d.nlabels;
    const size_t nlog = size_t(npos - s->params.n_seed + 2);
    static_assert(sizeof(SelCtl) <= SEL_SEEDS_AT, "the seed list starts behind the control block");
    const struct { void **ptr; size_t bytes; const char *what; } blocks[] = {
        {(void **)&d.ctl, 4096, "d.ctl"},
        {(void **)&d.S, B * 8, "d.S"},
        {(void **)&d.Stmp, B * 8, "d.Stmp"},
        {(void **)&d.base, B * 8, "d.base"},
        {(void **)&d.cand, B * 8, "d.cand"},
        {(void **)&d.M, size_t(cap) * B * 8, "d.M"},
        {(void **)&d.mH, size_t(cap) * 8, "d.mH"},
        {(void **)&d.mDelta, size_t(cap) * 8, "d.mDelta"},
        {(void **)&d.dtmp, size_t(cap) * 8, "d.dtmp"},
        {(void **)&d.dsum, size_t(cap) * 8, "d.dsum"},
        {(void **)&d.mLabel, size_t(cap) * 4, "d.mLabel"},
        {(void **)&d.mPos, size_t(cap) * 8, "d.mPos"},
        {(void **)&d.ord, size_t(cap) * 4, "d.ord"},
        {(void **)&d.inset, std::max<size_t>(nlabels, 1), "d.inset"},
        {(void **)&d.wg_rows, size_t(s->scan_grid) * 8, "d.wg_rows"},
        {(void **)&d.evlog_pos, nlog * 8, "d.evlog_pos"},
        {(void **)&d.evlog_kind, nlog * 4, "d.evlog_kind"},
    };
    for (const auto &b : blocks)
        if (int rc = dvs_dev_alloc(ctx, b.ptr, b.bytes, b.what)) return rc;
    if (s->params.flags & DVS_SELECT_STEPWISE) {
        uint64_t ring = std::min<uint64_t>(256, std::max<uint64_t>(32, (uint64_t(256) << 20) / (B * 8)));
        if (ctx->knobs.test_rowlog_ring >= 4) ring = ctx->knobs.test_rowlog_ring;
        d.rowlog_cap = uint32_t(ring);
        if (int rc = dvs_dev_alloc(ctx, (void **)&d.rowlog, size_t(ring) * B * 8, "d.rowlog")) return rc;
        uint32_t fsK = 1;
        while (uint64_t(cap + 1) * fsK * 2 <= 96 && uint64_t(fsK) * 2 * FS_JOB_THREADS <= B) fsK *= 2;
        const size_t fs_lds = ((B + 1) & ~1ull) * 16 + size_t(cap + 1) * 3 * 8 + size_t(cap + 1) * fsK * 7 * 8 + 64;
        if (s->params.mode == DVS_MODE_NMOST && s->params.n_seed >= 2 && !labels && !ctx->knobs.no_fast_step &&
            fs_lds <= ctx->lds_per_block && uint64_t(cap + 1) <= FS_MAXJOBS) {
            s->fs_K = fsK;
            s->fs_lds = fs_lds;
            s->fs_grid = uint32_t(ctx->n_cu);
            if (int rc = dvs_dev_alloc(ctx, (void **)&s->d_jobres, size_t(FS_MAXJOBS) * FS_RES * 8 + 8 * 8 * 1024, "s->d_jobres")) return rc;
            DVS_HIP(ctx, hipMemsetAsync(s->d_jobres, 0, size_t(FS_MAXJOBS) * FS_RES * 8 + 8 * 8 * 1024, ctx->stream));
            if (int rc = dvs_dev_alloc(ctx, (void **)&s->d_fsync, sizeof(FsSync), "s->d_fsync")) return rc;
            DVS_HIP(ctx, hipMemsetAsync(s->d_fsync, 0, sizeof(FsSync), ctx->stream));
            void *hh = nullptr;
            if (int rc = dvs_pinned_get(ctx, &hh)) return rc;
            memset(hh, 0, 4096);
            s->h_fshist = static_cast<unsigned long long *>(hh);
            s->fast_step = true;
            s->fs_need_scan = true;
        }
    }
    if (order) {
        if (int rc = dvs_dev_alloc(ctx, (void **)&d.order, size_t(npos) * 4, "d.order")) return rc;
        DVS_HIP(ctx, hipMemcpyAsync((void *)d.order, order, size_t(npos) * 4, hipMemcpyHostToDevice, ctx->stream));
    }
    if (labels) {
        if (int rc = dvs_dev_alloc(ctx, (void **)&d.labels, size_t(npos) * 4, "d.labels")) return rc;
        DVS_HIP(ctx, hipMemcpyAsync((void *)d.labels, labels, size_t(npos) * 4, hipMemcpyHostToDevice, ctx->stream));
    }
    static_assert(sizeof(SelCtl) <= 4096, "control block must fit a cached pinned block");
    return dvs_pinned_get(ctx, (void **)&s->h_ctl);
}

static int sel_prepare_engine(dvs_ctx *ctx, dvs_select *s, const uint32_t *order, const uint32_t *labels) {
    SelDev &d = s->dev;
    const dvs_matrix *m = s->mat;
    const uint32_t n_seed = s->params.n_seed, nlabels = d.nlabels;
    int rc = dvs_persist_setup(ctx, s);
    if (rc) return rc;
    sel_plan_setup_stream(ctx, s);
    if (s->setup_side) s->used_side_streams = true;
    DVS_HIP(ctx, hipMemsetAsync(d.inset, 0, std::max<size_t>(nlabels, 1), s->setup_side ? s->setup_side : ctx->stream));
    s->inset_clean = true;
    DVS_HIP(ctx, hipMemsetAsync(d.wg_rows, 0, size_t(s->scan_grid) * 8, s->setup_side ? s->setup_side : ctx->stream));
    s->seeded_start = s->persist && s->params.mode == DVS_MODE_NMOST && d.B <= 4096 && !order && !labels &&
                      !(s->params.flags & DVS_SELECT_STEPWISE) && n_seed >= 2 && n_seed <= 32 && !ctx->knobs.persist_no_seeded;
    s->persist_seeded = s->seeded_start;
    if (size_t(n_seed) * sizeof(uint64_t) <= 4096 - SEL_SEEDS_AT) {
        s->d_seed_list = reinterpret_cast<unsigned char *>(d.ctl) + SEL_SEEDS_AT;
        s->seed_list_in_ctl = true;
    } else if (s->seeded_start) {
        if ((rc = dvs_dev_alloc(ctx, &s->d_seed_list, size_t(n_seed) * sizeof(uint64_t), "seed list"))) return rc;
    }
    if (s->persist && m->rest_beside_head && ctx->stream_head && m->head_rows_built && s->params.mode == DVS_MODE_NMOST &&
        !order && !labels) {
        s->used_side_streams = true;
        return dvs_persist_prepare_head(ctx, s, m->head_rows_built, ctx->stream_head);
    }
    return DVS_OK;
}

static int sel_read_seeds(dvs_ctx *ctx, dvs_select *s, const uint32_t *order) {
    const dvs_matrix *m = s->mat;
    const uint32_t n_seed = s->params.n_seed;
    std::vector<uint32_t> h_tot(n_seed);
    int rc = dvs_matrix_settle(ctx, m);
    if (rc) return rc;
    hipError_t ce = hipSuccess;
    if (!order && n_seed && n_seed <= m->h_head_totals.size()) {
        std::copy(m->h_head_totals.begin(), m->h_head_totals.begin() + n_seed, h_tot.begin());
    } else if (!order && n_seed) {
        ce = hipMemcpyAsync(h_tot.data(), m->d_totals, size_t(n_seed) * 4, hipMemcpyDeviceToHost, ctx->stream);
    } else {
        for (uint64_t p = 0; p < n_seed && ce == hipSuccess; p++)
            ce = hipMemcpyAsync(&h_tot[p], m->d_totals + order[p], 4, hipMemcpyDeviceToHost, ctx->stream);
    }
    if ((order || n_seed > m->h_head_totals.size()) &&
        (hipStreamSynchronize(ctx->stream) != hipSuccess || ce != hipSuccess))
        return dvs_set_error(ctx, DVS_ERR_RUNTIME, "reading the seed rows' totals failed");
    std::vector<uint64_t> &seeds = s->seed_positions;
    for (uint64_t p = 0; p < n_seed; p++)
        if (h_tot[p] > 0) seeds.push_back(p);
    if (seeds.size() < 2)
        return seeds.empty() ? dvs_set_error(ctx, DVS_ERR_VALUE, "records cannot be empty")
                             : dvs_set_error(ctx, DVS_ERR_VALUE, "must have > 1 KmerSeq");
    return DVS_OK;
}

static void sel_init_ctl(dvs_ctx *ctx, dvs_select *s) {
    SelCtl c;
    std::memset(&c, 0, sizeof c);
    c.cursor = s->params.n_seed;
    c.npos = s->npos;
    c.event_pos = SEL_NONE;
    c.status = SEL_RUN;
    c.size = uint32_t(s->seed_positions.size());
    c.mode = s->params.mode;
    c.max_size = s->params.max_size;
    c.stat = s->params.stat;
    c.forced = FORCE_NONE;
    c.forced_lowest = 0xFFFFFFFFu;
    c.band = 0.0;
    c.wscale = 4.0;
    if (ctx->knobs.persist_no_events) c.wscale = 1e5;
    s->ctl0 = c;
}

extern "C" int dvs_select_run(dvs_ctx *ctx, const dvs_matrix *m, const uint32_t *order,
                              const uint32_t *labels, uint64_t npos,
                              const dvs_select_params *params, dvs_select **out) {
    if (!ctx || !m || !params || !out) return dvs_set_error(ctx, DVS_ERR_VALUE, "null argument");
    *out = nullptr;
    DVS_HIP(ctx, hipSetDevice(ctx->device));
    SelArgs a;
    int rc = sel_check_args(ctx, m, order, labels, npos, params, a);
    if (rc) return rc;
    labels = a.labels;
    std::unique_ptr<dvs_select, void (*)(dvs_select *)> s(new dvs_select(), sel_free);
    s->ctx = ctx;
    dvs_ctx_retain(ctx);
    s->params = *params;
    s->params.n_seed = a.n_seed;
    s->params.max_size = a.max_size;
    s->mat = m;
    s->mat_kind = m->kind;
    s->npos = npos;
    s->h_order.assign(order ? order : nullptr, order ? order + npos : nullptr);
    s->h_labels.assign(labels ? labels : nullptr, labels ? labels + npos : nullptr);
    if (a.caller_labels) s->h_out_labels.assign(a.caller_labels, a.caller_labels + npos);
    s->cap = a.cap;
    s->dev.B = m->nbins;
    s->dev.nlabels = a.nlabels;
    s->dev.totals = m->d_totals;
    s->dev.rowH = m->d_entropy;
    if ((rc = sel_geometry(ctx, s.get(), order, labels)) || (rc = sel_alloc(ctx, s.get(), order, labels)) ||
        (rc = sel_prepare_engine(ctx, s.get(), order, labels)) || (rc = sel_read_seeds(ctx, s.get(), order)))
        return rc;
    sel_init_ctl(ctx, s.get());
    if ((rc = dvs_mat_dispatch(m, [&](auto *mp) { return sel_start(ctx, s.get(), mp); }))) return rc;
    *out = s.release();
    return DVS_OK;
}

extern "C" void dvs_select_destroy(dvs_select *s) { sel_free(s); }

extern "C" int dvs_select_get_summary(dvs_ctx *ctx, const dvs_select *s, dvs_select_summary *out) {
    if (!s || !out) return dvs_set_error(ctx, DVS_ERR_VALUE, "null argument");
    const SelCtl &c = *s->h_ctl;
    std::memset(out, 0, sizeof *out);
    out->size = c.size;
    out->lowest_index = c.lowest;
    out->total_jsd = c.total_jsd;
    out->mean_delta_jsd = c.mean_delta;
    out->std_delta_jsd = c.std_delta;
    out->cov_delta_jsd = c.cov_delta;
    out->summed_entropies = c.sum_entropy;
    out->rows_scored = c.rows_scored;
    out->rows_rechecked = c.rows_rechecked;
    out->n_windows = c.n_windows;
    out->n_events = c.n_events;
    out->n_accepts = c.n_accepts;
    out->n_arbitrated = s->n_arbitrated;
    out->scan_ms = s->scan_ms;
    out->scan_launches = s->scan_launches;
    out->engine = s->persist ? 1u : 0u;
    out->rows_coarse_passed = uint32_t(std::min<unsigned long long>(c.rows_coarse_passed, 0xFFFFFFFFull));
    out->scan_ms_last = s->scan_ms_last;
    out->rows_scored_last = s->persist ? c.rows_scored - std::min(c.rows_before_launch, c.rows_scored) : 0;
    out->arbiter_ms = s->arbiter_ms;
    return DVS_OK;
}

extern "C" int dvs_select_get_members(dvs_ctx *ctx, const dvs_select *s, uint64_t *positions,
                                      uint32_t *labels, double *delta_jsd, double *entropy,
                                      double *freqs) {
    if (!s) return dvs_set_error(ctx, DVS_ERR_VALUE, "null argument");
    const uint32_t n = s->h_ctl->size;
    const uint64_t B = s->dev.B;
    std::vector<uint32_t> ord(n), lab(s->cap);
    std::vector<uint64_t> pos(s->cap);
    std::vector<double> mh(s->cap);
    DVS_HIP(ctx, hipMemcpy(ord.data(), s->dev.ord, size_t(n) * 4, hipMemcpyDeviceToHost));
    DVS_HIP(ctx, hipMemcpy(lab.data(), s->dev.mLabel, size_t(s->cap) * 4, hipMemcpyDeviceToHost));
    DVS_HIP(ctx, hipMemcpy(pos.data(), s->dev.mPos, size_t(s->cap) * 8, hipMemcpyDeviceToHost));
    DVS_HIP(ctx, hipMemcpy(mh.data(), s->dev.mH, size_t(s->cap) * 8, hipMemcpyDeviceToHost));
    if (delta_jsd)
        DVS_HIP(ctx, hipMemcpy(delta_jsd, s->dev.mDelta, size_t(n) * 8, hipMemcpyDeviceToHost));
    for (uint32_t i = 0; i < n; i++) {
        const uint32_t sl = ord[i];
        if (positions) positions[i] = pos[sl];
        if (labels) labels[i] = s->h_out_labels.empty() ? lab[sl] : s->h_out_labels[pos[sl]];
        if (entropy) entropy[i] = mh[sl];
        if (freqs)
            DVS_HIP(ctx, hipMemcpy(freqs + uint64_t(i) * B, s->dev.M + uint64_t(sl) * B, B * 8,
                                   hipMemcpyDeviceToHost));
    }
    return DVS_OK;
}

extern "C" int dvs_select_delta_jsd(dvs_ctx *ctx, const dvs_select *s, const dvs_matrix *q,
                                    const uint32_t *qlabels, double *out) {
    if (!s || !q || !out) return dvs_set_error(ctx, DVS_ERR_VALUE, "null argument");
    if (q->nbins != s->dev.B)
        return dvs_set_error(ctx, DVS_ERR_VALUE, "query matrix has %llu bins, the set %llu",
                             (unsigned long long)q->nbins, (unsigned long long)s->dev.B);
    if (q->nrows == 0) return DVS_OK;
    DVS_HIP(ctx, hipSetDevice(ctx->device));
    double *d_out = nullptr;
    uint32_t *d_lab = nullptr;
    std::vector<uint32_t> qtrans;
    if (qlabels && !s->h_out_labels.empty()) {
        const uint32_t n = s->h_ctl->size;
        std::vector<uint64_t> pos(s->cap);
        std::vector<uint32_t> ord(n);
        DVS_HIP(ctx, hipMemcpy(ord.data(), s->dev.ord, size_t(n) * 4, hipMemcpyDeviceToHost));
        DVS_HIP(ctx, hipMemcpy(pos.data(), s->dev.mPos, size_t(s->cap) * 8, hipMemcpyDeviceToHost));
        std::map<uint32_t, uint32_t> member_of;
        for (uint32_t i = 0; i < n; i++) {
            const uint64_t p = pos[ord[i]];
            if (s->h_out_labels[p] != 0xFFFFFFFFu) member_of[s->h_out_labels[p]] = uint32_t(p);
        }
        qtrans.resize(q->nrows);
        for (uint32_t i = 0; i < q->nrows; i++) {
            auto it = member_of.find(qlabels[i]);
            qtrans[i] = it == member_of.end() ? 0xFFFFFFFFu : it->second;
        }
        qlabels = qtrans.data();
    }
    DVS_HIP(ctx, hipMalloc(&d_out, size_t(q->nrows) * 8));
    if (qlabels) {
        DVS_HIP(ctx, hipMalloc(&d_lab, size_t(q->nrows) * 4));
        DVS_HIP(ctx, hipMemcpyAsync(d_lab, qlabels, size_t(q->nrows) * 4, hipMemcpyHostToDevice,
                                    ctx->stream));
    }
    dvs_mat_dispatch(q, [&](auto *qp) {
        using T = std::remove_cv_t<std::remove_pointer_t<decltype(qp)>>;
        hipLaunchKernelGGL((score_kernel<T>), dim3(q->nrows), dim3(LOO_THREADS), 0, ctx->stream, s->dev, qp,
                           q->d_totals, q->d_entropy, d_lab, d_out);
        return 0;
    });
    DVS_HIP(ctx, hipGetLastError());
    DVS_HIP(ctx, hipMemcpyAsync(out, d_out, size_t(q->nrows) * 8, hipMemcpyDeviceToHost, ctx->stream));
    DVS_HIP(ctx, hipStreamSynchronize(ctx->stream));
    (void)hipFree(d_out);
    if (d_lab) (void)hipFree(d_lab);
    return DVS_OK;
}

__global__ void log2_acc_selftest_kernel(double *out) {
    __shared__ double2 tab[128];
    if (threadIdx.x < 128) log2_tab_fill(tab, threadIdx.x);
    __syncthreads();
    const uint32_t t = blockIdx.x * blockDim.x + threadIdx.x;
    double worst = 0.0;
    for (int e = -78; e <= 1; e++) {
// ... 297 lines not shown
```

### diverseseq_amd/csrc/select_dev.h

```cpp
#pragma once

#include "select.h"

namespace {

__device__ __forceinline__ double log2_acc(double x) {
    double m = __builtin_amdgcn_frexp_mant(x);
    int e = __builtin_amdgcn_frexp_exp(x);
    if (m < 0.70710678118654752) {
        m *= 2.0;
        e -= 1;
    }
    const double f = m - 1.0;
    const double s = f / (2.0 + f);
    const double z = s * s;
    double p = 1.0 / 19.0;
    p = fma(p, z, 1.0 / 17.0);
    p = fma(p, z, 1.0 / 15.0);
    p = fma(p, z, 1.0 / 13.0);
    p = fma(p, z, 1.0 / 11.0);
    p = fma(p, z, 1.0 / 9.0);
    p = fma(p, z, 1.0 / 7.0);
    p = fma(p, z, 1.0 / 5.0);
    p = fma(p, z, 1.0 / 3.0);
// ... 4 lines not shown
__device__ __forceinline__ void log2_tab_fill(double2 *tab, int i) {
    const double c = 0.5 + (double(i) + 0.5) / 256.0;
    tab[i] = make_double2(log2_acc(c), 1.0 / c);
}
__device__ __forceinline__ double log2_tab(double x, const double2 *tab) {
    const double m = __builtin_amdgcn_frexp_mant(x);
    const int e = __builtin_amdgcn_frexp_exp(x);
    const uint32_t i = (uint32_t(__double2hiint(m)) >> 13) & 127u;
    const double2 t = tab[i];
    const double r = fma(m, t.y, -1.0);
    double p = 1.0 / 7.0;
    p = fma(p, r, -1.0 / 6.0);
    p = fma(p, r, 1.0 / 5.0);
    p = fma(p, r, -1.0 / 4.0);
    p = fma(p, r, 1.0 / 3.0);
    p = fma(p, r, -1.0 / 2.0);
    p = fma(p, r, 1.0);
    return fma(p * r, 1.4426950408889634, double(e) + t.x);
}

struct Ent {
    double h = 0.0, sum = 0.0, mn = 0.0;
    __device__ __forceinline__ void add(double x) {
        if (x > 0.0) h -= x * log2_acc(x);
        sum += x;
        mn = fmin(mn, x);
    }
    __device__ __forceinline__ void add(double x, const double2 *tab) {
        if (x > 0.0) h -= x * log2_tab(x, tab);
        sum += x;
        mn = fmin(mn, x);
    }
};

__device__ __forceinline__ uint64_t umin64(uint64_t a, uint64_t b) { return a < b ? a : b; }

__device__ __forceinline__ double sel_band(double hmean, uint64_t B) {
    return 4.0 * double(B) * DVS_EPS * fmax(1.0, fabs(hmean));
}

__device__ __forceinline__ double row_value(const uint32_t *row, uint64_t i) { return double(row[i]); }
__device__ __forceinline__ double row_value(const uint16_t *row, uint64_t i) { return double(row[i]); }
__device__ __forceinline__ double row_value(const double *row, uint64_t i) { return row[i]; }

constexpr double FAST_BAND = 4e-7;
constexpr int SCAN_CH = 16;

__device__ __forceinline__ double fast_neg_xlog2x(double x) {
    const double xm = fmax(x, 1e-300);
    const double m = __builtin_amdgcn_frexp_mant(xm);
    const int e = __builtin_amdgcn_frexp_exp(xm);
    const float l = __builtin_amdgcn_logf(float(m));
    return -xm * (double(e) + double(l));
}

typedef float dvs_f2 __attribute__((ext_vector_type(2)));
__device__ __forceinline__ double coarse_band(uint64_t B) {
    return 1.25 * 0x1p-24 * (9.0 * log2(double(B)) + 7.4);
}
__device__ __forceinline__ float coarse_sl(double v, double rn) { return v == 0.0 ? 1e-30f : float(v * rn); }
__device__ __forceinline__ float coarse4(const uint4 c, const float4 b, const dvs_f2 r2) {
    const dvs_f2 c01 = {float(c.x), float(c.y)}, c23 = {float(c.z), float(c.w)};
    const dvs_f2 y01 = __builtin_elementwise_fma(c01, r2, (dvs_f2){b.x, b.y});
    const dvs_f2 y23 = __builtin_elementwise_fma(c23, r2, (dvs_f2){b.z, b.w});
    const dvs_f2 l01 = {__builtin_amdgcn_logf(y01.x), __builtin_amdgcn_logf(y01.y)};
    const dvs_f2 l23 = {__builtin_amdgcn_logf(y23.x), __builtin_amdgcn_logf(y23.y)};
    const dvs_f2 s = y01 * l01 + y23 * l23;
    return s.x + s.y;
}

__device__ __forceinline__ float coarse4(const uint2 c, const float4 b, const dvs_f2 r2) {
    const dvs_f2 c01 = {float(c.x & 0xFFFFu), float(c.x >> 16)}, c23 = {float(c.y & 0xFFFFu), float(c.y >> 16)};
    const dvs_f2 y01 = __builtin_elementwise_fma(c01, r2, (dvs_f2){b.x, b.y});
    const dvs_f2 y23 = __builtin_elementwise_fma(c23, r2, (dvs_f2){b.z, b.w});
    const dvs_f2 l01 = {__builtin_amdgcn_logf(y01.x), __builtin_amdgcn_logf(y01.y)};
    const dvs_f2 l23 = {__builtin_amdgcn_logf(y23.x), __builtin_amdgcn_logf(y23.y)};
    const dvs_f2 s = y01 * l01 + y23 * l23;
    return s.x + s.y;
}

__device__ __forceinline__ void coarse8(const uint4 c, const float *b, const dvs_f2 r2, double &a0, double &a1) {
    a0 += double(coarse4(make_uint2(c.x, c.y), *reinterpret_cast<const float4 *>(b), r2));
    a1 += double(coarse4(make_uint2(c.z, c.w), *reinterpret_cast<const float4 *>(b + 4), r2));
}

template <typename T> struct Raw4;
template <> struct Raw4<uint32_t> {
    uint4 c;
    __device__ __forceinline__ void load(const uint32_t *p) { c = *reinterpret_cast<const uint4 *>(p); }
    __device__ __forceinline__ void pin() { asm volatile("" : "+v"(c.x), "+v"(c.y), "+v"(c.z), "+v"(c.w)); }
    __device__ __forceinline__ void get(double &v0, double &v1, double &v2, double &v3) const {
        v0 = double(c.x); v1 = double(c.y); v2 = double(c.z); v3 = double(c.w);
    }
};
template <> struct Raw4<uint16_t> {
    uint2 c;
    __device__ __forceinline__ void load(const uint16_t *p) { c = *reinterpret_cast<const uint2 *>(p); }
    __device__ __forceinline__ void pin() { asm volatile("" : "+v"(c.x), "+v"(c.y)); }
    __device__ __forceinline__ void get(double &v0, double &v1, double &v2, double &v3) const {
        v0 = double(c.x & 0xFFFFu); v1 = double(c.x >> 16); v2 = double(c.y & 0xFFFFu); v3 = double(c.y >> 16);
    }
};
template <> struct Raw4<double> {
    double2 a, b;
    __device__ __forceinline__ void load(const double *p) {
        a = *reinterpret_cast<const double2 *>(p);
        b = *reinterpret_cast<const double2 *>(p + 2);
    }
    __device__ __forceinline__ void pin() {}
    __device__ __forceinline__ void get(double &v0, double &v1, double &v2, double &v3) const {
        v0 = a.x; v1 = a.y; v2 = b.x; v3 = b.y;
    }
};

template <typename T>
__device__ __forceinline__ void load4(const T *rp, uint64_t i, double &v0, double &v1, double &v2,
                                      double &v3) {
    if constexpr (sizeof(T) == 4) {
        const uint4 c = *reinterpret_cast<const uint4 *>(rp + i);
        v0 = double(c.x); v1 = double(c.y); v2 = double(c.z); v3 = double(c.w);
    } else if constexpr (sizeof(T) == 2) {
        const uint2 c = *reinterpret_cast<const uint2 *>(rp + i);
        v0 = double(c.x & 0xFFFFu); v1 = double(c.x >> 16); v2 = double(c.y & 0xFFFFu); v3 = double(c.y >> 16);
    } else {
        const double2 a = *reinterpret_cast<const double2 *>(rp + i);
        const double2 b = *reinterpret_cast<const double2 *>(rp + i + 2);
        v0 = a.x; v1 = a.y; v2 = b.x; v3 = b.y;
    }
}

struct ScanState {
    uint64_t cursor, nrows;
    double thr_lo, thr_fast, thr_sure, he_base, dsize;
};

__device__ __forceinline__ void fast4(const double2 b01, const double2 b23, double v0, double v1,
                                      double v2, double v3, double rinv, double &a0, double &a1,
                                      double &a2, double &a3, double &xmin) {
    const double x0 = fma(v0, rinv, b01.x), x1 = fma(v1, rinv, b01.y);
    const double x2 = fma(v2, rinv, b23.x), x3 = fma(v3, rinv, b23.y);
    a0 += fast_neg_xlog2x(x0);
    a1 += fast_neg_xlog2x(x1);
    a2 += fast_neg_xlog2x(x2);
    a3 += fast_neg_xlog2x(x3);
    xmin = fmin(fmin(xmin, fmin(x0, x1)), fmin(x2, x3));
}

template <typename T>
__device__ __forceinline__ bool precise_row(const T *rp, const double *bvec, uint64_t B, double rinv,
                                            double mean_entropy, double thr_lo, uint32_t lane) {
    Ent e;
    if ((B & 255) == 0) {
        for (uint64_t i0 = 0; i0 < B; i0 += 256) {
            const uint64_t i = i0 + lane * 4;
            double v0, v1, v2, v3;
            load4(rp, i, v0, v1, v2, v3);
            e.add(fma(v0, rinv, bvec[i]));
            e.add(fma(v1, rinv, bvec[i + 1]));
            e.add(fma(v2, rinv, bvec[i + 2]));
            e.add(fma(v3, rinv, bvec[i + 3]));
        }
    } else {
        for (uint64_t i = lane; i < B; i += 64) e.add(fma(row_value(rp, i), rinv, bvec[i]));
    }
    const double h = dvs_wave_sum(e.h);
    return h - mean_entropy > thr_lo;
// ... 108 lines not shown
```

### diverseseq_amd/engine.py

```python

from __future__ import annotations

import ctypes as C
import weakref
from dataclasses import dataclass

import numpy as np

from . import _lib


def concat(seqs) -> tuple[np.ndarray, np.ndarray]:
    if seqs and all(type(s) is bytes for s in seqs):
        offsets = np.zeros(len(seqs) + 1, dtype=np.uint64)
        offsets[1:] = np.cumsum(np.fromiter(map(len, seqs), dtype=np.int64, count=len(seqs)), dtype=np.uint64)
        total = int(offsets[-1])
        data = np.frombuffer(b"".join(seqs), dtype=np.uint8) if total else np.zeros(16, dtype=np.uint8)
        return data, offsets
    arrs = []
    for s in seqs:
        if isinstance(s, (bytes, bytearray, memoryview)):
            arrs.append(np.frombuffer(s, dtype=np.uint8))
        else:
            arrs.append(np.ascontiguousarray(s, dtype=np.uint8).reshape(-1))
# ... 250 lines not shown
                while True:
                    line = raw_host[p + 1: p + 1 + width]
                    nl = np.flatnonzero(line == 10)
                    if nl.size or p + 1 + width >= raw_host.size:
                        break
                    width *= 16
                end = int(nl[0]) if nl.size else line.size
                self.labels_.append(line[:end].tobytes().decode("utf8", "replace").strip())
            self._labels = self.labels_
        return self._labels

    @property
    def dev_ptr(self) -> int:
        return int(self.ctx._L.dvs_seqbatch_dev_codes(self._h) or 0)

    def codes(self) -> np.ndarray:
        out = np.zeros(self.total, dtype=np.uint8)
        self.ctx.check(self.ctx._L.dvs_seqbatch_get_codes(self.ctx._h, self._h, _lib.ptr(out, C.c_uint8)))
        return out

    def sequences(self) -> list:
        c = self.codes()
        return [c[int(a): int(b)] for a, b in zip(self.offsets[:-1], self.offsets[1:])]

    def pack(self) -> "SeqBatch":
        self.ctx.check(self.ctx._L.dvs_seqbatch_pack(self.ctx._h, self._h))
        return self

    @property
    def packed(self) -> "Packed | None":
        h = self.ctx._L.dvs_seqbatch_packed(self._h)
        if not h:
            return None
        view = Packed(self.ctx, C.c_void_p(h), owned=False)
        view._batch = self
        return view

    def build_matrix(self, k: int, num_states: int = 4, *, canonical: bool = False) -> "CountMatrix":
        h = C.c_void_p()
        self.ctx.check(self.ctx._L.dvs_matrix_build_from_seqbatch(self.ctx._h, self._h, k, num_states, C.byref(h)))
        m = CountMatrix(self.ctx, h, k, num_states)
        m._source = self
        return _folded(m, canonical)

    def close(self):
        if getattr(self, "_h", None):
            self.ctx._L.dvs_seqbatch_destroy(self._h)
            self._h = None

    def __del__(self):
        try:
            self.close()
        except Exception:
            pass


class CountMatrix:

    def __init__(self, ctx: Context, handle, k: int, num_states: int):
        self.ctx, self._h, self.k, self.num_states = ctx, handle, k, num_states
        self._source = None
        L = ctx._L
        self.nrows = int(L.dvs_matrix_nrows(handle))
        self.nbins = int(L.dvs_matrix_nbins(handle))

    def close(self):
        if getattr(self, "_h", None):
            self.ctx._L.dvs_matrix_destroy(self._h)
            self._h = None

    def __del__(self):
        try:
            self.close()
        except Exception:
            pass

    def counts(self, row0: int = 0, nrows: int | None = None) -> np.ndarray:
        nrows = self.nrows - row0 if nrows is None else nrows
        out = np.zeros((nrows, self.nbins), dtype=np.uint32)
        self.ctx.check(self.ctx._L.dvs_matrix_get_counts(self.ctx._h, self._h, row0, nrows,
                                                         _lib.ptr(out, C.c_uint32)))
        return out

    def totals(self) -> np.ndarray:
        out = np.zeros(self.nrows, dtype=np.uint32)
        self.ctx.check(self.ctx._L.dvs_matrix_get_totals(self.ctx._h, self._h,
                                                         _lib.ptr(out, C.c_uint32)))
        return out

    def entropy(self) -> np.ndarray:
        out = np.zeros(self.nrows, dtype=np.float64)
        self.ctx.check(self.ctx._L.dvs_matrix_get_entropy(self.ctx._h, self._h,
                                                          _lib.ptr(out, C.c_double)))
        return out

    def source_rows(self) -> np.ndarray:
        out = np.zeros(self.nrows, dtype=np.uint32)
        self.ctx.check(self.ctx._L.dvs_matrix_get_source_rows(self.ctx._h, self._h, _lib.ptr(out, C.c_uint32)))
        return out

    def dev_counts(self) -> int:
        return int(self.ctx._L.dvs_matrix_dev_counts(self._h) or 0)

    @property
    def is_canonical(self) -> bool:
        return bool(self.ctx._L.dvs_matrix_is_canonical(self._h))

    def canonical(self) -> "CountMatrix":
        h = C.c_void_p()
        self.ctx.check(self.ctx._L.dvs_matrix_fold_canonical(self.ctx._h, self._h, C.byref(h)))
        return CountMatrix(self.ctx, h, self.k, self.num_states)

    @property
    def count_bytes(self) -> int:
        return int(self.ctx._L.dvs_matrix_count_bytes(self._h))

    def select(self, mode: int, n_seed: int, *, max_size: int = 0, stat: int = _lib.STAT_STDEV,
               order=None, labels=None, npos: int | None = None, window: int = 0,
               flags: int = 0) -> "Selection":
        order_a = None if order is None else np.ascontiguousarray(order, dtype=np.uint32)
        labels_a = None if labels is None else np.ascontiguousarray(labels, dtype=np.uint32)
        if npos is None:
            npos = order_a.size if order_a is not None else self.nrows
        p = _lib.SelectParams(mode, n_seed, max_size, stat, window, flags)
        h = C.c_void_p()
        self.ctx.check(self.ctx._L.dvs_select_run(self.ctx._h, self._h,
                                                  _lib.ptr(order_a, C.c_uint32),
                                                  _lib.ptr(labels_a, C.c_uint32), npos,
                                                  C.byref(p), C.byref(h)))
        sel = Selection(self, h)
        sel._order = order_a
        return sel

    def nmost(self, n: int, **kw) -> "Selection":
        return self.select(_lib.MODE_NMOST, n, **kw)

    def max_divergent(self, min_size: int, max_size: int, stat: str = "stdev", **kw) -> "Selection":
        st = _lib.STAT_STDEV if stat == "stdev" else _lib.STAT_COV
        return self.select(_lib.MODE_MAX, min_size, max_size=max_size, stat=st, **kw)

    def as_set(self, **kw) -> "Selection":
        return self.select(_lib.MODE_SET, 0, **kw)


@dataclass
class Members:
    positions: np.ndarray
    labels: np.ndarray
    delta_jsd: np.ndarray
    entropy: np.ndarray
    kfreqs: np.ndarray | None


class Selection:

    def __init__(self, matrix: CountMatrix, handle):
        self.matrix, self.ctx, self._h = matrix, matrix.ctx, handle
        self._gids = None
        self._lazy_gids = None
        self._order = None

    @property
    def global_ids(self):
        if self._gids is None and self._lazy_gids is not None:
            self._gids = self._lazy_gids.get()
        return self._gids

    @global_ids.setter
    def global_ids(self, value):
        self._gids = value

    def close(self):
        if getattr(self, "_h", None):
            self.ctx._L.dvs_select_destroy(self._h)
            self._h = None

    def __del__(self):
        try:
            self.close()
        except Exception:
            pass

    def summary(self) -> _lib.SelectSummary:
        s = _lib.SelectSummary()
        self.ctx.check(self.ctx._L.dvs_select_get_summary(self.ctx._h, self._h, C.byref(s)))
        return s

    def members(self, with_freqs: bool = True) -> Members:
        n = self.summary().size
        pos = np.zeros(n, dtype=np.uint64)
        lab = np.zeros(n, dtype=np.uint32)
        dl = np.zeros(n, dtype=np.float64)
        en = np.zeros(n, dtype=np.float64)
        fr = np.zeros((n, self.matrix.nbins), dtype=np.float64) if with_freqs else None
        self.ctx.check(self.ctx._L.dvs_select_get_members(
            self.ctx._h, self._h, _lib.ptr(pos, C.c_uint64), _lib.ptr(lab, C.c_uint32),
            _lib.ptr(dl, C.c_double), _lib.ptr(en, C.c_double), _lib.ptr(fr, C.c_double)))
        return Members(pos, lab, dl, en, fr)

    def gather_members(self, rows_ptr: int, meta_ptr: int, cap_rows: int):
        self.ctx.check(self.ctx._L.dvs_select_gather_members(self.ctx._h, self._h, C.c_void_p(rows_ptr),
                                                             C.c_void_p(meta_ptr), cap_rows))

    def bench_scan(self, repeats: int = 5) -> tuple[float, int]:
        ms, rows = C.c_double(), C.c_uint64()
        self.ctx.check(self.ctx._L.dvs_select_bench_scan(self.ctx._h, self._h, repeats, C.byref(ms),
                                                         C.byref(rows)))
        return ms.value, rows.value

    def delta_jsd(self, queries: CountMatrix, qlabels=None) -> np.ndarray:
        out = np.zeros(queries.nrows, dtype=np.float64)
        ql = None if qlabels is None else np.ascontiguousarray(qlabels, dtype=np.uint32)
        self.ctx.check(self.ctx._L.dvs_select_delta_jsd(self.ctx._h, self._h, queries._h,
                                                        _lib.ptr(ql, C.c_uint32),
                                                        _lib.ptr(out, C.c_double)))
        return out

    def member_rows(self) -> np.ndarray:
        pos = self.members(with_freqs=False).positions.astype(np.int64)
        return pos if self._order is None else self._order[pos].astype(np.int64)

    def assign(self, n_nearest: int = 1, mode: str = "jsd"):
        from . import distance

        return distance.matrix_nearest(self.matrix, self.matrix, n_nearest, mode, r_rows=self.member_rows())

    def diversify(self, n_select: int | None, mode: str = "jsd", min_distance: float | None = None):
        from . import distance

        return distance.matrix_maxmin(self.matrix, n_select, mode=mode, seeds=self.member_rows(), min_distance=min_distance)


_default_ctx: Context | None = None


def default_context() -> Context:
    global _default_ctx
    if _default_ctx is None:
        _default_ctx = Context()
    return _default_ctx
```

### include/dvs_hip.h

```cpp
#ifndef DVS_HIP_H
#define DVS_HIP_H

#include <stddef.h>
#include <stdint.h>

#ifdef __cplusplus
extern "C" {
#endif

#define DVS_ABI_VERSION 4

#define DVS_OK 0
#define DVS_ERR_VALUE 1
#define DVS_ERR_RUNTIME 2
#define DVS_ERR_NOMEM 3
#define DVS_ERR_UNSUPPORTED 4
#define DVS_ERR_ZERODIV 5

typedef struct dvs_ctx dvs_ctx;
typedef struct dvs_matrix dvs_matrix;
typedef struct dvs_select dvs_select;

int dvs_abi_version(void);
int dvs_ctx_create(int device, void *stream, dvs_ctx **out);
void dvs_ctx_destroy(dvs_ctx *ctx);
const char *dvs_last_error(const dvs_ctx *ctx);
int dvs_ctx_sync(dvs_ctx *ctx);
int dvs_ctx_trim(dvs_ctx *ctx);
int dvs_ctx_device_info(dvs_ctx *ctx, char *name, size_t name_len, int *n_cu,
                        uint64_t *hbm_bytes);

int dvs_matrix_build(dvs_ctx *ctx, const uint8_t *seqs, int seqs_on_device,
                     const uint64_t *offsets, uint32_t nseq, uint32_t k,
                     uint32_t num_states, dvs_matrix **out);
int dvs_matrix_from_freqs(dvs_ctx *ctx, const double *freqs, uint32_t nrows,
                          uint64_t nbins, dvs_matrix **out);
int dvs_matrix_from_device_freqs(dvs_ctx *ctx, const double *d_freqs, const double *d_meta,
                                 uint32_t nrows, uint64_t nbins, dvs_matrix **out);
int dvs_matrix_get_source_rows(dvs_ctx *ctx, const dvs_matrix *m, uint32_t *out);
void dvs_matrix_destroy(dvs_matrix *m);
uint32_t dvs_matrix_nrows(const dvs_matrix *m);
uint64_t dvs_matrix_nbins(const dvs_matrix *m);
const void *dvs_matrix_dev_counts(const dvs_matrix *m);
uint32_t dvs_matrix_count_bytes(const dvs_matrix *m);
const void *dvs_matrix_dev_totals(const dvs_matrix *m);
const void *dvs_matrix_dev_entropy(const dvs_matrix *m);
int dvs_matrix_get_counts(dvs_ctx *ctx, const dvs_matrix *m, uint32_t row0,
                          uint32_t nrows, uint32_t *out);
int dvs_matrix_get_totals(dvs_ctx *ctx, const dvs_matrix *m, uint32_t *out);
int dvs_matrix_get_entropy(dvs_ctx *ctx, const dvs_matrix *m, double *out);
int dvs_kmer_counts(dvs_ctx *ctx, const uint8_t *seqs, const uint64_t *offsets,
                    uint32_t nseq, uint32_t k, uint32_t num_states,
                    uint32_t *counts_out, uint32_t *totals_out, double *entropy_out);

int dvs_canonical_bins(uint32_t k, uint32_t *reps_out, uint64_t *n_out);
int dvs_matrix_fold_canonical(dvs_ctx *ctx, const dvs_matrix *m, dvs_matrix **out);
uint32_t dvs_matrix_is_canonical(const dvs_matrix *m);

typedef struct dvs_packed dvs_packed;
int dvs_pack_sequences(dvs_ctx *ctx, const uint8_t *seqs, int seqs_on_device, uint64_t nbases,
                       dvs_packed **out);
void dvs_packed_destroy(dvs_packed *p);
int dvs_packed_info(const dvs_packed *p, uint64_t *nbases, uint64_t *nwords);
const void *dvs_packed_dev_codes(const dvs_packed *p);
const void *dvs_packed_dev_mask(const dvs_packed *p);
int dvs_packed_get(dvs_ctx *ctx, const dvs_packed *p, uint32_t *codes_out, uint16_t *mask_out);
int dvs_matrix_build_packed(dvs_ctx *ctx, const dvs_packed *p, const uint64_t *offsets, uint32_t nseq,
                            uint32_t k, dvs_matrix **out);

typedef struct dvs_seqbatch dvs_seqbatch;
void dvs_default_alphabet_lut(int rna, uint8_t lut[256]);
int dvs_seqbatch_from_fasta(dvs_ctx *ctx, const uint8_t *raw, int raw_on_device, uint64_t nbytes,
                            const uint8_t *lut256, int join_records, dvs_seqbatch **out);
void dvs_seqbatch_destroy(dvs_seqbatch *b);
int dvs_seqbatch_info(const dvs_seqbatch *b, uint32_t *nseq, uint64_t *total_bases, uint32_t *nrecords);
int dvs_seqbatch_offsets(const dvs_seqbatch *b, uint64_t *offsets_out);
int dvs_seqbatch_header_positions(const dvs_seqbatch *b, uint64_t *pos_out);
const void *dvs_seqbatch_dev_codes(const dvs_seqbatch *b);
int dvs_seqbatch_get_codes(dvs_ctx *ctx, const dvs_seqbatch *b, uint8_t *codes_out);
int dvs_matrix_build_from_seqbatch(dvs_ctx *ctx, const dvs_seqbatch *b, uint32_t k, uint32_t num_states,
                                   dvs_matrix **out);
int dvs_seqbatch_pack(dvs_ctx *ctx, dvs_seqbatch *b);
const dvs_packed *dvs_seqbatch_packed(const dvs_seqbatch *b);

#define DVS_MODE_NMOST 0
#define DVS_MODE_MAX 1
#define DVS_MODE_SET 2
#define DVS_STAT_STDEV 0
#define DVS_STAT_COV 1

typedef struct dvs_select_params {
    uint32_t mode;
    uint32_t n_seed;
    uint32_t max_size;
    uint32_t stat;
    uint32_t window;
    uint32_t flags;
} dvs_select_params;
#define DVS_SELECT_NO_ARBITER 1u
#define DVS_SELECT_STEPWISE 2u
#define DVS_ROW_REMOTE 0xFFFFFFFFu

typedef struct dvs_select_summary {
    uint32_t size;
    uint32_t lowest_index;
    double total_jsd, mean_delta_jsd, std_delta_jsd, cov_delta_jsd, summed_entropies;
    uint64_t rows_scored;
    uint64_t rows_rechecked;
    uint32_t n_windows, n_events, n_accepts, n_arbitrated;
    double scan_ms;
    uint64_t scan_launches;
    uint32_t engine;
    uint32_t rows_coarse_passed;
    double scan_ms_last;
    uint64_t rows_scored_last;
    double arbiter_ms;
} dvs_select_summary;

int dvs_select_run(dvs_ctx *ctx, const dvs_matrix *m, const uint32_t *order,
                   const uint32_t *labels, uint64_t npos,
                   const dvs_select_params *params, dvs_select **out);
void dvs_select_destroy(dvs_select *s);
int dvs_select_get_summary(dvs_ctx *ctx, const dvs_select *s, dvs_select_summary *out);
int dvs_select_get_members(dvs_ctx *ctx, const dvs_select *s, uint64_t *positions,
                           uint32_t *labels, double *delta_jsd, double *entropy,
                           double *freqs);
int dvs_select_gather_members(dvs_ctx *ctx, const dvs_select *s, double *d_rows, double *d_meta,
                              uint32_t cap_rows);
int dvs_select_delta_jsd(dvs_ctx *ctx, const dvs_select *s, const dvs_matrix *queries,
                         const uint32_t *qlabels, double *out);
int dvs_select_step_pack(dvs_ctx *ctx, dvs_select *s, double *d_slot);
int dvs_select_step_apply(dvs_ctx *ctx, dvs_select *s, const double *d_all, uint32_t world);
int dvs_select_step_poll(dvs_ctx *ctx, dvs_select *s, uint32_t *status, uint64_t *cursor);
int dvs_select_step_peek(dvs_ctx *ctx, dvs_select *s, uint32_t lag, uint32_t *status, int *must_poll);

int dvs_ctx_set_timing(dvs_ctx *ctx, int on);
int dvs_ctx_refresh_knobs(dvs_ctx *ctx);
int dvs_select_bench_scan(dvs_ctx *ctx, const dvs_select *s, int repeats, double *ms_out,
                          uint64_t *rows_out);
int dvs_selftest_fast_log2(dvs_ctx *ctx, double *max_abs_err);
int dvs_selftest_log2_acc(dvs_ctx *ctx, double *max_rel_err);
int dvs_selftest_log2_f32(dvs_ctx *ctx, double *max_ulps);
int dvs_selftest_exact_div(dvs_ctx *ctx, uint64_t *mismatches);
int dvs_selftest_handover(dvs_ctx *ctx, uint32_t rounds, uint64_t *failures);

int dvs_mash_sketch(dvs_ctx *ctx, const uint8_t *seqs, int seqs_on_device,
                    const uint64_t *offsets, uint32_t nseq, uint32_t k,
                    uint32_t sketch_size, uint32_t num_states, int mash_canonical,
                    uint32_t *sketches_out, uint32_t *lens_out);
int dvs_mash_distances(dvs_ctx *ctx, const uint32_t *sketches, uint32_t sketch_stride,
                       const uint32_t *lens, uint32_t nseq, uint32_t k, uint32_t sketch_size,
                       uint32_t row_start, uint32_t row_stride, int symmetric,
                       double *dist);
typedef struct dvs_sketches dvs_sketches;
int dvs_sketches_build(dvs_ctx *ctx, const uint8_t *seqs, int seqs_on_device, const uint64_t *offsets,
                       uint32_t nseq, uint32_t k, uint32_t sketch_size, uint32_t num_states,
                       int mash_canonical, dvs_sketches **out);
int dvs_sketches_build_packed(dvs_ctx *ctx, const dvs_packed *p, const uint64_t *offsets, uint32_t nseq,
                              uint32_t k, uint32_t sketch_size, int mash_canonical, dvs_sketches **out);
int dvs_sketches_build_from_seqbatch(dvs_ctx *ctx, const dvs_seqbatch *b, uint32_t k, uint32_t sketch_size,
                                     uint32_t num_states, int mash_canonical, dvs_sketches **out);
void dvs_sketches_destroy(dvs_sketches *sk);
int dvs_sketches_get(dvs_ctx *ctx, const dvs_sketches *sk, uint32_t *sketches_out, uint32_t *lens_out);
const void *dvs_sketches_dev(const dvs_sketches *sk);
const void *dvs_sketches_dev_lens(const dvs_sketches *sk);
int dvs_sketches_distances(dvs_ctx *ctx, const dvs_sketches *sk, uint32_t k, uint32_t sketch_size,
                           uint32_t row_start, uint32_t row_stride, int symmetric, double *dist);
int dvs_sketches_from_device(dvs_ctx *ctx, const uint32_t *d_sketches, const uint32_t *d_lens, uint32_t nseq,
                             uint32_t stride, dvs_sketches **out);
int dvs_sketches_copy_to_device(dvs_ctx *ctx, const dvs_sketches *sk, uint32_t *d_dst, uint32_t dst_stride,
                                uint32_t *d_dst_lens);
int dvs_sketches_distances_device(dvs_ctx *ctx, const dvs_sketches *sk, uint32_t k, uint32_t sketch_size,
                                  uint32_t row_start, uint32_t row_stride, int symmetric, double *d_dist,
                                  uint32_t *d_zerodiv);

enum { DVS_SRC_MASH = 0, DVS_SRC_EUCLIDEAN = 1, DVS_SRC_JSD = 2, DVS_SRC_GIVEN = 3 };
typedef struct dvs_source {
    uint32_t kind;
    void *handle;
    const uint32_t *rows;
    uint32_t n;
    uint32_t k, sketch_size;
    int on_device;
} dvs_source;
int dvs_distances(dvs_ctx *ctx, const dvs_source *src, double *dist);

#define DVS_LINKAGE_SINGLE 0
#define DVS_LINKAGE_COMPLETE 1
#define DVS_LINKAGE_AVERAGE 2
#define DVS_LINKAGE_WARD 5
#define DVS_LINKAGE_WEIGHTED 6
int dvs_linkage(dvs_ctx *ctx, const dvs_source *src, int method, uint32_t *pairs, double *heights, uint32_t *sizes);


int dvs_cross_distances(dvs_ctx *ctx, const dvs_source *q, const dvs_source *r, double *dist);
int dvs_nearest(dvs_ctx *ctx, const dvs_source *q, const dvs_source *r, uint32_t kk, uint32_t *idx, double *dist);

#define DVS_CUT_HEIGHT 0
#define DVS_CUT_NCLUSTERS 1
int dvs_linkage_cut(dvs_ctx *ctx, uint32_t n, const uint32_t *pairs, const double *heights, int criterion, double value,
                    uint32_t *labels_out, uint32_t *n_clusters_out);
int dvs_cluster_scores(dvs_ctx *ctx, const dvs_source *src, const uint32_t *labels, uint32_t n_clusters, double *within,
                       double *a, double *b, uint32_t *neighbour, double *silhouette, uint32_t *medoids);

typedef struct dvs_pairs dvs_pairs;
#define DVS_WITHIN_SKIP_SELF 1u
// ... 23 lines not shown
```

Measured before the change: 70.20 million.

## Add saturating 8-bit count plane for the coarse f32 scan of unsaturated rows

During the k=6 histogram build, each row's 16-bit counts are also written as a saturated 8-bit plane, swizzled so one wave reads it in four 16-byte loads per lane, plus a per-row flag set when any count exceeds 255. The persistent select scan reads this plane for the coarse f32 score on unflagged rows, halving the bytes fetched per row versus the 16-bit counts. This adds memory and build-time writes, a byte load per row for the flag, and an atomic counter per row scored from the plane. Accessors for the plane and the plane-row count are added.

```diff
diff --git a/diverseseq_amd/_lib.py b/diverseseq_amd/_lib.py
--- a/diverseseq_amd/_lib.py
+++ b/diverseseq_amd/_lib.py
@@ -40,6 +40,7 @@
     "dvs_linkage_cut", "dvs_linkage_cophenet", "dvs_nj_patristic", "dvs_pairs_destroy", "dvs_pairs_info", "dvs_pairs_get",
     "dvs_distances", "dvs_linkage", "dvs_nj", "dvs_maxmin", "dvs_cross_distances", "dvs_nearest", "dvs_within",
     "dvs_cluster_scores", "dvs_cophenet", "dvs_threshold_clusters",
+    "dvs_matrix_get_coarse8", "dvs_select_get_coarse8_rows",
 )
 WITHIN_SKIP_SELF = 1
 SRC_MASH, SRC_EUCLIDEAN, SRC_JSD, SRC_GIVEN = range(4)
@@ -137,6 +138,8 @@
             getattr(L, n).argtypes = [vp]
             getattr(L, n).restype = vp
         L.dvs_matrix_get_counts.argtypes = [vp, vp, C.c_uint32, C.c_uint32, u32p]
+        L.dvs_matrix_get_coarse8.argtypes = [vp, vp, C.c_uint32, C.c_uint32, u8p, u8p]
+        L.dvs_select_get_coarse8_rows.argtypes = [vp, vp, u64p]
         L.dvs_matrix_get_totals.argtypes = [vp, vp, u32p]
         L.dvs_matrix_get_entropy.argtypes = [vp, vp, f64p]
         L.dvs_matrix_get_source_rows.argtypes = [vp, vp, u32p]
diff --git a/diverseseq_amd/csrc/api.cpp b/diverseseq_amd/csrc/api.cpp
--- a/diverseseq_amd/csrc/api.cpp
+++ b/diverseseq_amd/csrc/api.cpp
@@ -125,6 +125,7 @@
     k->counts_u32 = on("DVS_COUNTS_U32");
     k->build_wait = on("DVS_BUILD_WAIT");
     k->no_packed_upload = on("DVS_NO_PACKED_UPLOAD");
+    k->no_coarse8 = on("DVS_NO_COARSE8");
     k->cu_mask_set = on("HSA_CU_MASK") || on("ROC_GLOBAL_CU_MASK");
     k->no_persist = on("DVS_NO_PERSIST");
     k->no_fast_step = on("DVS_NO_FAST_STEP");
@@ -367,6 +368,16 @@
     m->num_states = num_states;
     m->device = ctx->device;
     int rc = matrix_alloc(ctx, m);
+    if (!rc && m->kind == 2 && B == 4096 && !ctx->knobs.no_coarse8) {
+        if (dvs_dev_alloc(ctx, (void **)&m->d_coarse8, size_t(nseq) * B, "matrix counts (8-bit plane)") ||
+            dvs_dev_alloc(ctx, (void **)&m->d_coarse8_sat, nseq, "8-bit plane row flags")) {
+            (void)hipGetLastError();
+            dvs_dev_free(ctx, m->d_coarse8);
+            dvs_dev_free(ctx, m->d_coarse8_sat);
+            m->d_coarse8 = m->d_coarse8_sat = nullptr;
+            ctx->err.clear();
+        }
+    }
     if (!rc && nseq) rc = dvs_matrix_fill_counts(ctx, m, sv, offsets, no_wait);
     if (rc) {
         dvs_matrix_free_fields(m);
@@ -569,6 +580,25 @@
     return DVS_OK;
 }
 
+int dvs_matrix_get_coarse8(dvs_ctx *ctx, const dvs_matrix *m, uint32_t row0, uint32_t nrows, uint8_t *out_bytes,
+                           uint8_t *out_sat) {
+    if (!ctx || !m) return dvs_set_error(ctx, DVS_ERR_VALUE, "null argument");
+    if (!m->d_coarse8 || !m->d_coarse8_sat) return dvs_set_error(ctx, DVS_ERR_UNSUPPORTED, "the matrix has no 8-bit plane");
+    if (uint64_t(row0) + nrows > m->nrows) return dvs_set_error(ctx, DVS_ERR_VALUE, "row range out of bounds");
+    if (!nrows) return DVS_OK;
+    const uint64_t B = m->nbins;
+    std::vector<uint8_t> tmp(out_bytes ? size_t(nrows) * B : 0);
+    if (out_bytes)
+        DVS_HIP(ctx, hipMemcpyAsync(tmp.data(), m->d_coarse8 + uint64_t(row0) * B, tmp.size(), hipMemcpyDeviceToHost, ctx->stream));
+    if (out_sat) DVS_HIP(ctx, hipMemcpyAsync(out_sat, m->d_coarse8_sat + row0, nrows, hipMemcpyDeviceToHost, ctx->stream));
+    DVS_HIP(ctx, hipStreamSynchronize(ctx->stream));
+    for (size_t i = 0; i < tmp.size(); i++) {
+        const size_t at = i & 1023;
+        out_bytes[(i - at) + 256 * ((at >> 2) & 3) + 4 * (at >> 4) + (at & 3)] = tmp[i];
+    }
+    return DVS_OK;
+}
+
 int dvs_matrix_get_totals(dvs_ctx *ctx, const dvs_matrix *m, uint32_t *out) {
     if (!ctx || !m || !out) return dvs_set_error(ctx, DVS_ERR_VALUE, "null argument");
     if (!m->nrows) return DVS_OK;
diff --git a/diverseseq_amd/csrc/dvs_internal.h b/diverseseq_amd/csrc/dvs_internal.h
--- a/diverseseq_amd/csrc/dvs_internal.h
+++ b/diverseseq_amd/csrc/dvs_internal.h
@@ -21,6 +21,7 @@
     bool counts_u32 = false;
     bool build_wait = false;
     bool no_packed_upload = false;
+    bool no_coarse8 = false;
     bool cu_mask_set = false;
     bool no_fast_step = false;
     bool no_persist = false;
@@ -123,6 +124,7 @@
 struct dvs_matrix {
     int kind = 0;
     uint16_t *d_counts16 = nullptr;
+    uint8_t *d_coarse8 = nullptr, *d_coarse8_sat = nullptr;
     uint32_t nrows = 0;
     uint64_t nbins = 0;
     uint32_t k = 0, num_states = 0;
diff --git a/diverseseq_amd/csrc/kmer_hist.hip b/diverseseq_amd/csrc/kmer_hist.hip
--- a/diverseseq_amd/csrc/kmer_hist.hip
+++ b/diverseseq_amd/csrc/kmer_hist.hip
@@ -51,7 +51,8 @@
     const uint64_t *__restrict__ offsets,
     const KTile *__restrict__ tiles, uint32_t *__restrict__ counts, uint32_t *__restrict__ totals,
     double *__restrict__ entropy, const double *__restrict__ clog_tbl, uint32_t k, uint32_t ns,
-    uint64_t B, uint32_t hot_rows, uint32_t row0, uint64_t uni_base, uint64_t uni_stride) {
+    uint64_t B, uint32_t hot_rows, uint32_t row0, uint64_t uni_base, uint64_t uni_stride,
+    uint8_t *__restrict__ coarse8, uint8_t *__restrict__ coarse8_sat) {
     extern __shared__ __attribute__((aligned(16))) unsigned char smem[];
     KTile t;
     if (tiles) {
@@ -223,9 +224,30 @@
                 if (((w.x | w.y) & 0xFF00FF00u) == 0) sv[half] += ((tbl[v.x] + tbl[v.y]) + tbl[v.z]) + tbl[v.w];
                 else sv[half] += clog2c(v.x, tbl) + clog2c(v.y, tbl) + clog2c(v.z, tbl) + clog2c(v.w, tbl);
             }
+        [[maybe_unused]] bool sat = false;
+        if constexpr (OUT16) {
+            if (coarse8) {
+                uint4 *pl = reinterpret_cast<uint4 *>(coarse8 + uint64_t(t.row) * B);
+                for (uint32_t s = uint32_t(tid); s < uint32_t(B / 16); s += uint32_t(nthreads)) {
+                    const uint32_t u0 = (s >> 6) * 256u + (s & 63u);
+                    uint32_t o[4], any = 0;
+#pragma unroll
+                    for (int q = 0; q < 4; q++) {
+                        const uint2 w = h2[u0 + 64u * q];
+                        any |= w.x | w.y;
+                        o[q] = min(w.x & 0xFFFFu, 255u) | (min(w.x >> 16, 255u) << 8) | (min(w.y & 0xFFFFu, 255u) << 16) |
+                               (min(w.y >> 16, 255u) << 24);
+                    }
+                    sat = sat || (any & 0xFF00FF00u) != 0;
+                    if (t.row < hot_rows) pl[s] = make_uint4(o[0], o[1], o[2], o[3]);
+                    else __builtin_nontemporal_store((u32x4){o[0], o[1], o[2], o[3]}, reinterpret_cast<u32x4 *>(pl + s));
+                }
+            }
+        }
         tv[0] = double(nvalid);
         const int lane = tid & 63, wave = tid >> 6;
         double sums[2];
+        [[maybe_unused]] const bool wave_sat = __ballot(sat) != 0ull;
 #pragma unroll
         for (int q = 0; q < 2; q++) {
             const double a = dvs_wave_sum(q ? tv[0] : sv[0]), b = dvs_wave_sum(q ? tv[1] : sv[1]);
@@ -233,6 +255,7 @@
             if (lane == 0) {
                 scratch[wave] = a;
                 scratch[wave + 2] = b;
+                if constexpr (OUT16) scratch[wave + 4] = wave_sat ? 1.0 : 0.0;
             }
             __syncthreads();
             double acc = 0.0;
@@ -242,6 +265,8 @@
         if (tid == 0) {
             totals[t.row] = uint32_t(sums[1]);
             entropy[t.row] = sums[1] > 0.0 ? log2(sums[1]) - sums[0] / sums[1] : 0.0;
+            if constexpr (OUT16)
+                if (coarse8) coarse8_sat[t.row] = (scratch[4] != 0.0 || scratch[5] != 0.0) ? 1 : 0;
         }
     } else if (t.single) {
         double s = 0.0, tot = 0.0;
@@ -410,6 +435,9 @@
     dvs_dev_free(m->ctx, m->d_counts);
     dvs_dev_free(m->ctx, m->d_counts16);
     m->d_counts16 = nullptr;
+    dvs_dev_free(m->ctx, m->d_coarse8);
+    dvs_dev_free(m->ctx, m->d_coarse8_sat);
+    m->d_coarse8 = m->d_coarse8_sat = nullptr;
     dvs_dev_free(m->ctx, m->d_freqs);
     dvs_dev_free(m->ctx, m->d_totals);
     dvs_dev_free(m->ctx, m->d_entropy);
@@ -586,6 +614,7 @@
     uint32_t *d_rows = static_cast<uint32_t *>(oc.d_rows);
     KTile *d_tiles = static_cast<KTile *>(oc.d_tiles);
     const size_t n_long = oc.n_long, n_tiles = oc.n_tiles;
+    uint8_t *const no_c8 = nullptr;
     auto cleanup = [&]() {};
     int rc = DVS_OK;
     hipError_t e = hipSuccess;
@@ -612,7 +641,7 @@
         if (!rc)                                                                                 \
             hipLaunchKernelGGL((kmer_hist_kernel<NS4, LH, false, false, PKD>), dim3(GRID), dim3(NTHR), lds,  \
                                ctx->stream, d_seqs, d_pmask, nbytes, d_off, TILES, m->d_counts,  \
-                               m->d_totals, m->d_entropy, ctx->d_clog_tbl, k, ns, B, HOT, 0u, uni_base, uni_stride);   \
+                               m->d_totals, m->d_entropy, ctx->d_clog_tbl, k, ns, B, HOT, 0u, uni_base, uni_stride, no_c8, no_c8);   \
     } while (0)
 #define DVS_LAUNCH_HIST_ANY(GRID, TILES, NTHR, HOT)                            \
     do {                                                                  \
@@ -641,19 +670,19 @@
                 if (!rc)
                     hipLaunchKernelGGL((kmer_hist_kernel<true, true, true, true, true>), dim3(count), dim3(128), lds16, on,
                                        d_seqs, d_pmask, nbytes, d_off, static_cast<const KTile *>(nullptr), out16,
-                                       m->d_totals, m->d_entropy, ctx->d_clog_tbl, k, ns, B, hot_end, row0, uni_base, uni_stride);
+                                       m->d_totals, m->d_entropy, ctx->d_clog_tbl, k, ns, B, hot_end, row0, uni_base, uni_stride, m->d_coarse8, m->d_coarse8_sat);
             } else if (ns4) {
                 rc = set_dyn_lds(ctx, kmer_hist_kernel<true, true, true, true>, lds16);
                 if (!rc)
                     hipLaunchKernelGGL((kmer_hist_kernel<true, true, true, true>), dim3(count), dim3(128), lds16, on,
                                        d_seqs, d_pmask, nbytes, d_off, static_cast<const KTile *>(nullptr), out16,
-                                       m->d_totals, m->d_entropy, ctx->d_clog_tbl, k, ns, B, hot_end, row0, uni_base, uni_stride);
+                                       m->d_totals, m->d_entropy, ctx->d_clog_tbl, k, ns, B, hot_end, row0, uni_base, uni_stride, m->d_coarse8, m->d_coarse8_sat);
             } else {
                 rc = set_dyn_lds(ctx, kmer_hist_kernel<false, true, true, true>, lds16);
                 if (!rc)
                     hipLaunchKernelGGL((kmer_hist_kernel<false, true, true, true>), dim3(count), dim3(128), lds16, on,
                                        d_seqs, d_pmask, nbytes, d_off, static_cast<const KTile *>(nullptr), out16,
-                                       m->d_totals, m->d_entropy, ctx->d_clog_tbl, k, ns, B, hot_end, row0, uni_base, uni_stride);
+                                       m->d_totals, m->d_entropy, ctx->d_clog_tbl, k, ns, B, hot_end, row0, uni_base, uni_stride, m->d_coarse8, m->d_coarse8_sat);
             }
         };
         if (head_rows) {
@@ -707,19 +736,19 @@
             if (!rc)
                 hipLaunchKernelGGL((kmer_hist_kernel<true, true, true, false, true>), dim3(nseq), dim3(128), lds16, ctx->stream,
                                    d_seqs, d_pmask, nbytes, d_off, static_cast<const KTile *>(nullptr), m->d_counts,
-                                   m->d_totals, m->d_entropy, ctx->d_clog_tbl, k, ns, B, hot_rows, 0u, uni_base, uni_stride);
+                                   m->d_totals, m->d_entropy, ctx->d_clog_tbl, k, ns, B, hot_rows, 0u, uni_base, uni_stride, no_c8, no_c8);
         } else if (ns4) {
             rc = set_dyn_lds(ctx, kmer_hist_kernel<true, true, true>, lds16);
             if (!rc)
                 hipLaunchKernelGGL((kmer_hist_kernel<true, true, true>), dim3(nseq), dim3(128), lds16, ctx->stream,
                                    d_seqs, d_pmask, nbytes, d_off, static_cast<const KTile *>(nullptr), m->d_counts,
-                                   m->d_totals, m->d_entropy, ctx->d_clog_tbl, k, ns, B, hot_rows, 0u, uni_base, uni_stride);
+                                   m->d_totals, m->d_entropy, ctx->d_clog_tbl, k, ns, B, hot_rows, 0u, uni_base, uni_stride, no_c8, no_c8);
         } else {
             rc = set_dyn_lds(ctx, kmer_hist_kernel<false, true, true>, lds16);
             if (!rc)
                 hipLaunchKernelGGL((kmer_hist_kernel<false, true, true>), dim3(nseq), dim3(128), lds16, ctx->stream,
                                    d_seqs, d_pmask, nbytes, d_off, static_cast<const KTile *>(nullptr), m->d_counts,
-                                   m->d_totals, m->d_entropy, ctx->d_clog_tbl, k, ns, B, hot_rows, 0u, uni_base, uni_stride);
+                                   m->d_totals, m->d_entropy, ctx->d_clog_tbl, k, ns, B, hot_rows, 0u, uni_base, uni_stride, no_c8, no_c8);
         }
     } else
         DVS_LAUNCH_HIST_ANY(nseq, static_cast<const KTile *>(nullptr), nthreads, hot_rows);
diff --git a/diverseseq_amd/csrc/persist.hip b/diverseseq_amd/csrc/persist.hip
--- a/diverseseq_amd/csrc/persist.hip
+++ b/diverseseq_amd/csrc/persist.hip
@@ -263,7 +263,8 @@
                                             uint64_t first, uint64_t stride, uint64_t nrows,
                                             uint32_t lane, uint32_t &nread,
                                             uint32_t &nprecise, uint32_t &nmid, bool coarse_on,
-                                            bool burst_drop = true) {
+                                            bool burst_drop = true, const uint8_t *__restrict__ c8 = nullptr,
+                                            const uint8_t *__restrict__ c8_sat = nullptr, uint32_t *c8_count = nullptr) {
     const double dn = double(st.n), rn = 1.0 / dn;
     const double thr_lo = st.thr - st.band;
     const double thr_fast = thr_lo - FAST_BAND, thr_sure = st.thr + st.band + FAST_BAND;
@@ -277,6 +278,8 @@
         const uint64_t ev = p_hint_pos(win);
         const uint32_t tot = totals[p];
         const double hrow = rowH[p];
+        [[maybe_unused]] bool from_plane = false;
+        if constexpr (COARSE && sizeof(T) == 2) from_plane = c8 != nullptr && c8_sat[p] == 0;
         if (ev < p) break;
         if (tot == 0) continue;
         const double rt = 1.0 / double(tot);
@@ -289,7 +292,20 @@
                 double c0 = 0.0, c1 = 0.0;
                 bool done16 = false;
                 if constexpr (sizeof(T) == 2) {
-                    if (B == 4096) {
+                    if (B == 4096 && from_plane) {
+                        const uint4 *pp = reinterpret_cast<const uint4 *>(c8 + p * 4096) + lane;
+                        uint4 raw4[4];
+#pragma unroll
+                        for (int j = 0; j < 4; j++) raw4[j] = pp[j * 64];
+                        __builtin_amdgcn_sched_barrier(0);
+#pragma unroll
+                        for (int j = 0; j < 4; j++) {
+                            asm volatile("" : "+v"(raw4[j].x), "+v"(raw4[j].y), "+v"(raw4[j].z), "+v"(raw4[j].w));
+                            coarse16(raw4[j], slf + j * 1024 + lane * 4, r2, c0, c1);
+                        }
+                        if (lane == 0) atomicAdd(c8_count, 1u);
+                        done16 = true;
+                    } else if (B == 4096) {
                         uint4 raw8[8];
 #pragma unroll
                         for (int j = 0; j < 8; j++) raw8[j] = *reinterpret_cast<const uint4 *>(rp + j * 512 + lane * 8);
@@ -724,6 +740,8 @@
     uint32_t *s_slot = reinterpret_cast<uint32_t *>(s_pos + maxn);
     unsigned long long *s_win = reinterpret_cast<unsigned long long *>(s_slot + maxn + (maxn & 1));
     int *s_flag = reinterpret_cast<int *>(s_win + P_WINWORDS);
+    uint32_t *s_c8 = reinterpret_cast<uint32_t *>(s_flag + 3);
+    static_assert(P_MAXG <= SEL_C8_SLOTS, "one word of SelDev::c8_rows per workgroup");
     static_assert(maxn % 4 == 0 && P_WINWORDS % 2 == 0, "s_ltab below must sit on a 16-byte boundary");
     double2 *s_ltab = reinterpret_cast<double2 *>(s_win + P_WINWORDS + 2);
     unsigned long long *s_prev = reinterpret_cast<unsigned long long *>(s_ltab + 128);
@@ -737,6 +755,7 @@
     [[maybe_unused]] double *s_bpart = s_bev + 12 * P_BATCH;
     if (threadIdx.x < 128) log2_tab_fill(s_ltab, threadIdx.x);
     for (uint32_t i = threadIdx.x; i < (maxn + 1) * 2; i += P_THREADS) s_prev[i] = 0ull;
+    if (threadIdx.x == 0) *s_c8 = 0u;
     SelCtl *ctl = d.ctl;
     const int tid0 = threadIdx.x;
     const int tid = tid0;
@@ -1183,7 +1202,7 @@
             else
                 p_scan_rows<T, COARSE>(mat, d.totals, d.rowH, sl, slf, B, st, st.sumH - s_mH[st.li], win,
                                        uint64_t(blockIdx.x) * wpb + wave, nwaves, nrows, lane, nread, nprecise, nmid, coarse_on,
-                                       true);
+                                       true, d.c8, d.c8_sat, s_c8);
         }
         double fr[P_J];
         [[maybe_unused]] T craw[P_J];
@@ -2683,6 +2702,8 @@
         if (nprecise) atomicAdd(&ctl->rows_rechecked, (unsigned long long)nprecise);
         if (nmid) atomicAdd(&ctl->rows_coarse_passed, (unsigned long long)nmid);
     }
+    __syncthreads();
+    if (tid == 0 && *s_c8) atomicAdd(&d.c8_rows[blockIdx.x], *s_c8);
     if (lead && tid == 0) {
         ctl->cursor = st.cursor;
         ctl->window = st.window < ctl->window_max ? st.window : ctl->window_max;
diff --git a/diverseseq_amd/csrc/select.h b/diverseseq_amd/csrc/select.h
--- a/diverseseq_amd/csrc/select.h
+++ b/diverseseq_amd/csrc/select.h
@@ -4,6 +4,7 @@
 
 #define SEL_NONE 0xFFFFFFFFFFFFFFFFull
 #define SEL_SEEDS_AT 512
+#define SEL_C8_SLOTS 256
 
 enum : uint32_t { SEL_RUN = 0, SEL_DONE = 1, SEL_ARBITER = 2, SEL_ERROR = 3,
                   SEL_NEED_SETUP = 4 };
@@ -62,6 +63,8 @@
     uint32_t *ord = nullptr;
     uint8_t *inset = nullptr;
     uint32_t *wg_rows = nullptr;
+    const uint8_t *c8 = nullptr, *c8_sat = nullptr;
+    uint32_t *c8_rows = nullptr;
     unsigned long long *evlog_pos = nullptr;
     uint32_t *evlog_kind = nullptr;
     const double *gather_all = nullptr;
diff --git a/diverseseq_amd/csrc/select.hip b/diverseseq_amd/csrc/select.hip
--- a/diverseseq_amd/csrc/select.hip
+++ b/diverseseq_amd/csrc/select.hip
@@ -2194,7 +2194,7 @@
         {(void **)&d.mPos, size_t(cap) * 8, "d.mPos"},
         {(void **)&d.ord, size_t(cap) * 4, "d.ord"},
         {(void **)&d.inset, std::max<size_t>(nlabels, 1), "d.inset"},
-        {(void **)&d.wg_rows, size_t(s->scan_grid) * 8, "d.wg_rows"},
+        {(void **)&d.wg_rows, size_t(s->scan_grid) * 8 + SEL_C8_SLOTS * 4, "d.wg_rows"},
         {(void **)&d.evlog_pos, nlog * 8, "d.evlog_pos"},
         {(void **)&d.evlog_kind, nlog * 4, "d.evlog_kind"},
     };
@@ -2247,7 +2247,8 @@
     if (s->setup_side) s->used_side_streams = true;
     DVS_HIP(ctx, hipMemsetAsync(d.inset, 0, std::max<size_t>(nlabels, 1), s->setup_side ? s->setup_side : ctx->stream));
     s->inset_clean = true;
-    DVS_HIP(ctx, hipMemsetAsync(d.wg_rows, 0, size_t(s->scan_grid) * 8, s->setup_side ? s->setup_side : ctx->stream));
+    d.c8_rows = d.wg_rows + size_t(s->scan_grid) * 2;
+    DVS_HIP(ctx, hipMemsetAsync(d.wg_rows, 0, size_t(s->scan_grid) * 8 + SEL_C8_SLOTS * 4, s->setup_side ? s->setup_side : ctx->stream));
     s->seeded_start = s->persist && s->params.mode == DVS_MODE_NMOST && d.B <= 4096 && !order && !labels &&
                       !(s->params.flags & DVS_SELECT_STEPWISE) && n_seed >= 2 && n_seed <= 32 && !ctx->knobs.persist_no_seeded;
     s->persist_seeded = s->seeded_start;
@@ -2338,6 +2339,10 @@
     s->dev.nlabels = a.nlabels;
     s->dev.totals = m->d_totals;
     s->dev.rowH = m->d_entropy;
+    if (m->d_coarse8 && m->d_coarse8_sat && !ctx->knobs.no_coarse8) {
+        s->dev.c8 = m->d_coarse8;
+        s->dev.c8_sat = m->d_coarse8_sat;
+    }
     if ((rc = sel_geometry(ctx, s.get(), order, labels)) || (rc = sel_alloc(ctx, s.get(), order, labels)) ||
         (rc = sel_prepare_engine(ctx, s.get(), order, labels)) || (rc = sel_read_seeds(ctx, s.get(), order)))
         return rc;
@@ -2376,6 +2381,16 @@
     return DVS_OK;
 }
 
+extern "C" int dvs_select_get_coarse8_rows(dvs_ctx *ctx, const dvs_select *s, uint64_t *n) {
+    if (!s || !n) return dvs_set_error(ctx, DVS_ERR_VALUE, "null argument");
+    *n = 0;
+    if (!s->dev.c8_rows) return DVS_OK;
+    uint32_t per_wg[SEL_C8_SLOTS];
+    DVS_HIP(ctx, hipMemcpy(per_wg, s->dev.c8_rows, sizeof per_wg, hipMemcpyDeviceToHost));
+    for (uint32_t v : per_wg) *n += v;
+    return DVS_OK;
+}
+
 extern "C" int dvs_select_get_members(dvs_ctx *ctx, const dvs_select *s, uint64_t *positions,
                                       uint32_t *labels, double *delta_jsd, double *entropy,
                                       double *freqs) {
diff --git a/diverseseq_amd/csrc/select_dev.h b/diverseseq_amd/csrc/select_dev.h
--- a/diverseseq_amd/csrc/select_dev.h
+++ b/diverseseq_amd/csrc/select_dev.h
@@ -110,6 +110,22 @@
 __device__ __forceinline__ void coarse8(const uint4 c, const float *b, const dvs_f2 r2, double &a0, double &a1) {
     a0 += double(coarse4(make_uint2(c.x, c.y), *reinterpret_cast<const float4 *>(b), r2));
     a1 += double(coarse4(make_uint2(c.z, c.w), *reinterpret_cast<const float4 *>(b + 4), r2));
+}
+
+__device__ __forceinline__ float coarse4(const uint32_t c, const float4 b, const dvs_f2 r2) {
+    const dvs_f2 c01 = {float(c & 0xFFu), float((c >> 8) & 0xFFu)}, c23 = {float((c >> 16) & 0xFFu), float(c >> 24)};
+    const dvs_f2 y01 = __builtin_elementwise_fma(c01, r2, (dvs_f2){b.x, b.y});
+    const dvs_f2 y23 = __builtin_elementwise_fma(c23, r2, (dvs_f2){b.z, b.w});
+    const dvs_f2 l01 = {__builtin_amdgcn_logf(y01.x), __builtin_amdgcn_logf(y01.y)};
+    const dvs_f2 l23 = {__builtin_amdgcn_logf(y23.x), __builtin_amdgcn_logf(y23.y)};
+    const dvs_f2 s = y01 * l01 + y23 * l23;
+    return s.x + s.y;
+}
+__device__ __forceinline__ void coarse16(const uint4 c, const float *b, const dvs_f2 r2, double &a0, double &a1) {
+    a0 += double(coarse4(c.x, *reinterpret_cast<const float4 *>(b), r2));
+    a1 += double(coarse4(c.y, *reinterpret_cast<const float4 *>(b + 256), r2));
+    a0 += double(coarse4(c.z, *reinterpret_cast<const float4 *>(b + 512), r2));
+    a1 += double(coarse4(c.w, *reinterpret_cast<const float4 *>(b + 768), r2));
 }
 
 template <typename T> struct Raw4;
diff --git a/diverseseq_amd/engine.py b/diverseseq_amd/engine.py
--- a/diverseseq_amd/engine.py
+++ b/diverseseq_amd/engine.py
@@ -356,6 +356,14 @@
                                                          _lib.ptr(out, C.c_uint32)))
         return out
 
+    def coarse8(self, row0: int = 0, nrows: int | None = None) -> tuple[np.ndarray, np.ndarray]:
+        nrows = self.nrows - row0 if nrows is None else nrows
+        out = np.zeros((nrows, self.nbins), dtype=np.uint8)
+        sat = np.zeros(nrows, dtype=np.uint8)
+        self.ctx.check(self.ctx._L.dvs_matrix_get_coarse8(self.ctx._h, self._h, row0, nrows, _lib.ptr(out, C.c_uint8),
+                                                          _lib.ptr(sat, C.c_uint8)))
+        return out, sat
+
     def totals(self) -> np.ndarray:
         out = np.zeros(self.nrows, dtype=np.uint32)
         self.ctx.check(self.ctx._L.dvs_matrix_get_totals(self.ctx._h, self._h,
@@ -508,6 +516,12 @@
 _default_ctx: Context | None = None
 
 
+def coarse8_rows(sel: "Selection") -> int:
+    n = C.c_uint64(0)
+    sel.ctx.check(sel.ctx._L.dvs_select_get_coarse8_rows(sel.ctx._h, sel._h, C.byref(n)))
+    return int(n.value)
+
+
 def default_context() -> Context:
     global _default_ctx
     if _default_ctx is None:
diff --git a/include/dvs_hip.h b/include/dvs_hip.h
--- a/include/dvs_hip.h
+++ b/include/dvs_hip.h
@@ -47,6 +47,8 @@
 const void *dvs_matrix_dev_entropy(const dvs_matrix *m);
 int dvs_matrix_get_counts(dvs_ctx *ctx, const dvs_matrix *m, uint32_t row0,
                           uint32_t nrows, uint32_t *out);
+int dvs_matrix_get_coarse8(dvs_ctx *ctx, const dvs_matrix *m, uint32_t row0, uint32_t nrows, uint8_t *out_bytes,
+                           uint8_t *out_sat);
 int dvs_matrix_get_totals(dvs_ctx *ctx, const dvs_matrix *m, uint32_t *out);
 int dvs_matrix_get_entropy(dvs_ctx *ctx, const dvs_matrix *m, double *out);
 int dvs_kmer_counts(dvs_ctx *ctx, const uint8_t *seqs, const uint64_t *offsets,
@@ -122,6 +124,7 @@
                    const dvs_select_params *params, dvs_select **out);
 void dvs_select_destroy(dvs_select *s);
 int dvs_select_get_summary(dvs_ctx *ctx, const dvs_select *s, dvs_select_summary *out);
+int dvs_select_get_coarse8_rows(dvs_ctx *ctx, const dvs_select *s, uint64_t *n);
 int dvs_select_get_members(dvs_ctx *ctx, const dvs_select *s, uint64_t *positions,
                            uint32_t *labels, double *delta_jsd, double *entropy,
                            double *freqs);
```

Measured after the change: 71.69 million (median of 6 runs). +2.1%, better.
